# kaiwenShen/Do-You-Really-Need-to-Pay-2-20-Hedge-Fund-Strategy-Replication-via-Machine-Learning

Measured on AMD Instinct MI355X. Metric: seq/sec/node MTSS-WGAN-GP train (24x32 windows) at 1/2/4/8 GPUs; W-dist parity, higher is better.
Workload: dtype fp32; 1 GPU; global_batch=262144, batch_per_gpu=262144, seq_len=24, features=32, parallelism=dp1

## Files before the change

### do-you-really-need-to-pay-2-20-hedge-fund-strategy-replication-via-machine-learning_amd/csrc/bindings.cpp

```cpp
#include <torch/extension.h>
#include <torch/library.h>
#include <ATen/hip/impl/HIPGuardImplMasqueradingAsCUDA.h>
#include <ATen/hip/impl/HIPStreamMasqueradingAsCUDA.h>

#include "kernels.h"
#include "poison.h"

#include <atomic>
#include <cmath>
#include <cstdlib>
#include <cstring>

std::atomic<bool>& hfrep::poison_flag() {
  static std::atomic<bool> f{[] {
    const char* e = getenv("HFREP_POISON");
    return e && e[0] == '1';
  }()};
  return f;
}

namespace {

using at::Tensor;
using c10::optional;
// ... 162 lines not shown
  }
  Tensor ws = out_empty({(int64_t)hfrep::lstm_wgrad2_workspace_floats(M, K, Hd, N)}, x.options().dtype(at::kFloat));
  hfrep::launch_lstm_wgrad2(x.data_ptr(), hs.data_ptr(), dZ.data_ptr(), tangent ? xd->data_ptr() : nullptr,
                            tangent ? hds->data_ptr() : nullptr, tangent ? dZd->data_ptr() : nullptr,
                            gW.data_ptr<float>(), gU.data_ptr<float>(), gb.has_value() ? gb->data_ptr<float>() : nullptr,
                            M, K, Hd, N, Tn, ws.data_ptr<float>(), cur_stream(x));
}

Tensor act_fwd(Tensor x, int64_t act) {
  CHECK_GPU(x); GUARD(x);
  Tensor y = out_empty_like(x);
  hfrep::launch_act_fwd(dt_of(x), x.data_ptr(), y.data_ptr(), x.numel(), (int)act, cur_stream(x));
  return y;
}
Tensor act_bwd(Tensor dy, Tensor y, int64_t act) {
  CHECK_GPU(dy); CHECK_GPU(y); same_dt(dy, y);
  TORCH_CHECK(dy.numel() == y.numel(), "act_bwd: size");
  GUARD(dy);
  Tensor dx = out_empty_like(dy);
  hfrep::launch_act_bwd(dt_of(dy), dy.data_ptr(), y.data_ptr(), dx.data_ptr(), dy.numel(), (int)act, cur_stream(dy));
  return dx;
}
Tensor act_tangent_bwd(Tensor dyd, Tensor y, Tensor zd, int64_t act) {
  CHECK_GPU(dyd); CHECK_GPU(y); CHECK_GPU(zd); same_dt(dyd, y); same_dt(dyd, zd);
  TORCH_CHECK(dyd.numel() == y.numel() && y.numel() == zd.numel(), "act_tangent_bwd: size");
  GUARD(dyd);
  Tensor out = out_empty_like(dyd);
  hfrep::launch_act_tangent_bwd(dt_of(dyd), dyd.data_ptr(), y.data_ptr(), zd.data_ptr(), out.data_ptr(), dyd.numel(),
                                (int)act, cur_stream(dyd));
  return out;
}

void check_lstm_U(const Tensor& U, int64_t H) {
  CHECK_F32(U);
  TORCH_CHECK(U.dim() == 2 && U.size(0) == H && U.size(1) == 4 * H, "recurrent kernel must be (H, 4H)");
}

std::tuple<Tensor, Tensor, Tensor> lstm_fwd(Tensor zx, Tensor U, int64_t act, bool save) {
  CHECK_GPU(zx);
  TORCH_CHECK(zx.dim() == 3 && zx.size(2) % 4 == 0, "zx must be (B, T, 4H)");
  const int B = zx.size(0), Tn = zx.size(1), H = zx.size(2) / 4;
  check_lstm_U(U, H);
  GUARD(zx);
  Tensor hs = out_empty({B, Tn, H}, zx.options());
  Tensor gates = save ? out_empty({B, Tn, 4 * H}, zx.options()) : out_empty({0}, zx.options());
  Tensor cs = save ? out_empty({B, Tn, H}, zx.options()) : out_empty({0}, zx.options());
  const bool ok = hfrep::launch_lstm_fwd(dt_of(zx), zx.data_ptr(), U.data_ptr<float>(), hs.data_ptr(),
                                         save ? gates.data_ptr() : nullptr, save ? cs.data_ptr() : nullptr, B, Tn, H,
                                         (int)act, cur_stream(zx));
  TORCH_CHECK(ok, "lstm_fwd: hidden size ", H, " not instantiated (supported: 100, 64, 32)");
  return {hs, gates, cs};
}

Tensor lstm_bwd(Tensor dH, Tensor gates, Tensor cs, Tensor U, int64_t act) {
  CHECK_GPU(dH); CHECK_GPU(gates); CHECK_GPU(cs); same_dt(dH, gates); same_dt(dH, cs);
  const int B = gates.size(0), Tn = gates.size(1), H = gates.size(2) / 4;
  TORCH_CHECK(dH.sizes() == cs.sizes() && cs.size(2) == H, "lstm_bwd: shapes");
  check_lstm_U(U, H);
  GUARD(dH);
  Tensor dZ = out_empty_like(gates);
  const bool ok = hfrep::launch_lstm_bwd(dt_of(dH), dH.data_ptr(), gates.data_ptr(), cs.data_ptr(),
                                         U.data_ptr<float>(), dZ.data_ptr(), B, Tn, H, (int)act, cur_stream(dH));
  TORCH_CHECK(ok, "lstm_bwd: hidden size ", H, " not instantiated");
  return dZ;
}

std::tuple<Tensor, Tensor, Tensor> lstm_tfwd(Tensor dzx, Tensor gates, Tensor cs, Tensor U, int64_t act) {
  CHECK_GPU(dzx); CHECK_GPU(gates); CHECK_GPU(cs); same_dt(dzx, gates); same_dt(dzx, cs);
  TORCH_CHECK(dzx.sizes() == gates.sizes(), "lstm_tfwd: shapes");
  const int B = gates.size(0), Tn = gates.size(1), H = gates.size(2) / 4;
  check_lstm_U(U, H);
  GUARD(dzx);
  Tensor hds = out_empty({B, Tn, H}, dzx.options());
  Tensor zds = out_empty_like(gates);
  Tensor cds = out_empty({B, Tn, H}, dzx.options());
  const bool ok = hfrep::launch_lstm_tfwd(dt_of(dzx), dzx.data_ptr(), gates.data_ptr(), cs.data_ptr(),
                                          U.data_ptr<float>(), hds.data_ptr(), zds.data_ptr(), cds.data_ptr(), B, Tn,
                                          H, (int)act, cur_stream(dzx));
  TORCH_CHECK(ok, "lstm_tfwd: hidden size ", H, " not instantiated");
  return {hds, zds, cds};
}

std::tuple<Tensor, Tensor> lstm_tbwd(optional<Tensor> dH, Tensor dHd, Tensor gates, Tensor cs, Tensor zds, Tensor cds,
                                     Tensor U, int64_t act) {
  CHECK_GPU(dHd); CHECK_GPU(gates); CHECK_GPU(cs); CHECK_GPU(zds); CHECK_GPU(cds);
  same_dt(dHd, gates); same_dt(dHd, zds); same_dt(dHd, cds);
  if (dH.has_value()) { CHECK_GPU(*dH); same_dt(*dH, dHd); }
  const int B = gates.size(0), Tn = gates.size(1), H = gates.size(2) / 4;
  check_lstm_U(U, H);
  GUARD(dHd);
  Tensor dZ = out_empty_like(gates), dZd = out_empty_like(gates);
  const bool ok = hfrep::launch_lstm_tbwd(dt_of(dHd), ptr_or_null(dH), dHd.data_ptr(), gates.data_ptr(),
                                          cs.data_ptr(), zds.data_ptr(), cds.data_ptr(), U.data_ptr<float>(),
                                          dZ.data_ptr(), dZd.data_ptr(), B, Tn, H, (int)act, cur_stream(dHd));
  TORCH_CHECK(ok, "lstm_tbwd: hidden size ", H, " not instantiated");
  return {dZ, dZd};
}

bool lstmf_supported(int64_t H, int64_t K, int64_t act) { return hfrep::lstmf_supported((int)H, (int)K, (int)act); }
bool narrowf_supported(int64_t K, int64_t N) { return hfrep::narrowf_supported((int)K, (int)N); }
int64_t set_lstmf_fwd_impl(int64_t v) { return hfrep::set_lstmf_fwd_impl((int)v); }
int64_t set_lstmf_fwd100_impl(int64_t v) { return hfrep::set_lstmf_fwd100_impl((int)v); }
int64_t set_lstmf_bwd_impl(int64_t v) { return hfrep::set_lstmf_bwd_impl((int)v); }

std::tuple<Tensor, Tensor> lstmf_fwd(Tensor x, Tensor W, optional<Tensor> b, Tensor U, int64_t act, bool save) {
  CHECK_F32(x); CHECK_F32(W);
  TORCH_CHECK(x.dim() == 3, "x must be (B, T, K)");
  const int B = x.size(0), Tn = x.size(1), K = x.size(2), H = U.size(0);
  check_lstm_U(U, H);
  TORCH_CHECK(W.size(0) == K && W.size(1) == 4 * H, "W must be (K, 4H)");
  if (b.has_value()) { CHECK_F32(*b); TORCH_CHECK(b->numel() == 4 * H, "bias size"); }
  TORCH_CHECK(hfrep::lstmf_supported(H, K, (int)act), "lstmf_fwd: unsupported H/K/act");
  GUARD(x);
  Tensor hs = out_empty({B, Tn, H}, x.options());
  Tensor tape = at::empty({save ? (int64_t)hfrep::lstmf_tape_elems(B, Tn) : 0}, x.options());
  const bool ok = hfrep::launch_lstmf_fwd(x.data_ptr<float>(), W.data_ptr<float>(),
                                          b.has_value() ? b->data_ptr<float>() : nullptr, U.data_ptr<float>(),
                                          hs.data_ptr<float>(), save ? tape.data_ptr<float>() : nullptr, B, Tn, K, H,
                                          (int)act, cur_stream(x));
  TORCH_CHECK(ok, "lstmf_fwd: launch failed");
  return {hs, tape};
}

std::tuple<Tensor, Tensor> lstmf_tfwd(Tensor xd, Tensor W, Tensor U, Tensor tape, int64_t act) {
  CHECK_F32(xd); CHECK_F32(W); CHECK_F32(tape);
  TORCH_CHECK(xd.dim() == 3, "xd must be (B, T, K)");
  const int B = xd.size(0), Tn = xd.size(1), K = xd.size(2), H = U.size(0);
  check_lstm_U(U, H);
  TORCH_CHECK(W.size(0) == K && W.size(1) == 4 * H, "W must be (K, 4H)");
  TORCH_CHECK(tape.numel() == (int64_t)hfrep::lstmf_tape_elems(B, Tn), "lstmf_tfwd: tape size");
  TORCH_CHECK(hfrep::lstmf_supported(H, K, (int)act), "lstmf_tfwd: unsupported H/K/act");
  GUARD(xd);
  Tensor hds = out_empty({B, Tn, H}, xd.options());
  Tensor ttape = at::empty_like(tape);
  const bool ok = hfrep::launch_lstmf_tfwd(xd.data_ptr<float>(), W.data_ptr<float>(), U.data_ptr<float>(),
                                           tape.data_ptr<float>(), hds.data_ptr<float>(), ttape.data_ptr<float>(), B, Tn,
                                           K, H, (int)act, cur_stream(xd));
  TORCH_CHECK(ok, "lstmf_tfwd: launch failed");
  return {hds, ttape};
}

static void check_head(const optional<Tensor>& d, const optional<Tensor>& w, const Tensor& like, int64_t B, int64_t n) {
  if (d.has_value()) {
    CHECK_F32(*d);
    TORCH_CHECK(d->numel() == B && d->device() == like.device(), "head adjoint factor: B fp32 values");
  }
  if (w.has_value()) {
    CHECK_F32(*w);
    TORCH_CHECK(w->numel() == n && w->device() == like.device(), "head weight: Tn H fp32 values");
  }
}

bool lstmf_ahd_supported() { return hfrep::lstmf_ahd_supported(); }

Tensor lstmf_bwd(optional<Tensor> dH, Tensor tape, Tensor U, int64_t act, int64_t B, int64_t Tn, optional<Tensor> hd,
                 optional<Tensor> hw, optional<Tensor> ah_out) {
  CHECK_F32(tape);
  const int H = U.size(0);
  check_lstm_U(U, H);
  TORCH_CHECK(tape.numel() == (int64_t)hfrep::lstmf_tape_elems(B, Tn), "lstmf_bwd: tape size");
  if (dH.has_value()) { CHECK_F32(*dH); TORCH_CHECK(dH->numel() == B * Tn * H, "lstmf_bwd: dH shape"); }
  TORCH_CHECK(hd.has_value() == hw.has_value() && !(hd.has_value() && dH.has_value()),
              "lstmf_bwd: dH or the head factors (hd, hw)");
  check_head(hd, hw, tape, B, Tn * H);
  if (ah_out.has_value()) {
    CHECK_F32(*ah_out);
    TORCH_CHECK(ah_out->numel() == B * Tn * H && ah_out->is_contiguous() && ah_out->device() == tape.device(),
                "lstmf_bwd: ah_out must be a contiguous (B, T, H) fp32 tensor on the tape's device");
    TORCH_CHECK(hfrep::lstmf_ahd_supported(), "lstmf_bwd: ah_out needs the split-recurrent BPTT (lstmf_ahd_supported)");
  }
  GUARD(tape);
  Tensor dZ = out_empty({B, Tn, 4 * H}, tape.options());
  Tensor dHm;
  if (hd.has_value() && !hfrep::lstmf_head_supported()) {
    dHm = out_empty({B, Tn * H}, tape.options());
    hfrep::launch_skinny_dgrad(hfrep::DT_F32, hd->data_ptr<float>(), hw->data_ptr<float>(), dHm.data_ptr(), B,
                               (int)(Tn * H), 1, cur_stream(tape));
  }
  const bool head = hd.has_value() && !dHm.defined();
  const float* dhp = dHm.defined() ? dHm.data_ptr<float>() : dH.has_value() ? dH->data_ptr<float>() : nullptr;
  const bool ok = hfrep::launch_lstmf_bwd(dhp, tape.data_ptr<float>(), U.data_ptr<float>(), dZ.data_ptr<float>(), B, Tn,
                                          H, (int)act, cur_stream(tape), head ? hd->data_ptr<float>() : nullptr,
                                          head ? hw->data_ptr<float>() : nullptr,
                                          ah_out.has_value() ? ah_out->data_ptr<float>() : nullptr);
  TORCH_CHECK(ok, "lstmf_bwd: unsupported H / act");
  return dZ;
}

Tensor lstmf_tbwd1(optional<Tensor> dH, Tensor aH, Tensor tape, Tensor ttape, Tensor U, int64_t act, int64_t B,
                   int64_t Tn, optional<Tensor> hd, optional<Tensor> hw) {
  CHECK_F32(tape); CHECK_F32(ttape); CHECK_F32(aH);
  const int H = U.size(0);
  check_lstm_U(U, H);
  TORCH_CHECK(tape.numel() == (int64_t)hfrep::lstmf_tape_elems(B, Tn) && ttape.numel() == tape.numel(), "tape size");
  TORCH_CHECK(aH.numel() == B * Tn * H && aH.is_contiguous() && aH.device() == tape.device(),
              "lstmf_tbwd1: aH must be a contiguous (B, T, H) fp32 tensor on the tape's device");
  if (dH.has_value()) {
    CHECK_F32(*dH);
    TORCH_CHECK(dH->numel() == B * Tn * H && dH->is_contiguous() && dH->device() == tape.device(),
                "lstmf_tbwd1: adjoint shape");
  }
  const bool head = hw.has_value();
  TORCH_CHECK(!head || !dH.has_value(), "lstmf_tbwd1: the adjoint dH or head factors, not both");
  TORCH_CHECK(head || !hd.has_value(), "lstmf_tbwd1: hd needs hw");
  check_head(hd, hw, tape, B, Tn * H);
  GUARD(tape);
  Tensor dZ = out_empty({B, Tn, 4 * H}, tape.options());
  const bool ok = hfrep::launch_lstmf_tbwd1(dH.has_value() ? dH->data_ptr<float>() : nullptr, aH.data_ptr<float>(),
                                            tape.data_ptr<float>(), ttape.data_ptr<float>(), U.data_ptr<float>(),
                                            dZ.data_ptr<float>(), B, Tn, H, (int)act, cur_stream(tape),
                                            head && hd.has_value() ? hd->data_ptr<float>() : nullptr,
                                            head ? hw->data_ptr<float>() : nullptr);
  TORCH_CHECK(ok, "lstmf_tbwd1: unsupported H / act");
  return dZ;
}

std::tuple<Tensor, Tensor> lstmf_tbwd(optional<Tensor> dH, optional<Tensor> dHd, Tensor tape, Tensor ttape, Tensor U,
                                      int64_t act, int64_t B, int64_t Tn, optional<Tensor> hd, optional<Tensor> hdd,
                                      optional<Tensor> hw) {
  CHECK_F32(tape); CHECK_F32(ttape);
  const int H = U.size(0);
  check_lstm_U(U, H);
  TORCH_CHECK(tape.numel() == (int64_t)hfrep::lstmf_tape_elems(B, Tn) && ttape.numel() == tape.numel(), "tape size");
  for (const auto* d : {&dH, &dHd})
    if (d->has_value()) { CHECK_F32(**d); TORCH_CHECK((*d)->numel() == B * Tn * H, "lstmf_tbwd: adjoint shape"); }
  const bool head = hw.has_value();
  TORCH_CHECK(!head || (!dH.has_value() && !dHd.has_value()), "lstmf_tbwd: adjoints (dH, dHd) or head factors, not both");
  check_head(hd, hw, tape, B, Tn * H);
  check_head(hdd, {}, tape, B, Tn * H);
  GUARD(tape);
  Tensor dZ = out_empty({B, Tn, 4 * H}, tape.options()), dZd = out_empty({B, Tn, 4 * H}, tape.options());
  const bool ok = hfrep::launch_lstmf_tbwd(dH.has_value() ? dH->data_ptr<float>() : nullptr,
                                           dHd.has_value() ? dHd->data_ptr<float>() : nullptr, tape.data_ptr<float>(),
                                           ttape.data_ptr<float>(), U.data_ptr<float>(), dZ.data_ptr<float>(),
                                           dZd.data_ptr<float>(), B, Tn, H, (int)act, cur_stream(tape),
                                           head && hd.has_value() ? hd->data_ptr<float>() : nullptr,
                                           head && hdd.has_value() ? hdd->data_ptr<float>() : nullptr,
                                           head ? hw->data_ptr<float>() : nullptr);
  TORCH_CHECK(ok, "lstmf_tbwd: unsupported H / act");
  return {dZ, dZd};
}

Tensor lstmf_dgrad(Tensor dz, Tensor W, int64_t impl) {
  CHECK_F32(dz); CHECK_F32(W);
  TORCH_CHECK(dz.dim() == 2 && dz.is_contiguous() && W.dim() == 2 && W.is_contiguous() && W.size(1) == dz.size(1),
              "lstmf_dgrad: dz (M, N) and W (KO, N), contiguous");
  TORCH_CHECK(hfrep::lstmf_dgrad_supported(dz.size(1), W.size(0)), "lstmf_dgrad: N must be 400 and KO <= 112");
  GUARD(dz);
  Tensor x = out_empty({dz.size(0), W.size(0)}, dz.options());
  if (dz.size(0) == 0) return x;
  const bool ok = hfrep::launch_lstmf_dgrad(dz.data_ptr<float>(), W.data_ptr<float>(), x.data_ptr<float>(), dz.size(0),
                                            dz.size(1), W.size(0), cur_stream(dz), (int)impl);
  TORCH_CHECK(ok, "lstmf_dgrad: launch failed");
  return x;
}

void check_lstm2(const Tensor& x, const Tensor& U, int64_t H) {
  TORCH_CHECK(x.scalar_type() == at::kBFloat16, "lstm2 kernels are bf16-only");
  check_lstm_U(U, H);
  TORCH_CHECK(hfrep::lstm2_supported((int)H, (int)x.size(2)), "lstm2: unsupported H/K (H must be 100, K <= 128)");
}

std::tuple<Tensor, Tensor> lstm2_fwd(Tensor x, Tensor W, optional<Tensor> b, Tensor U, int64_t act, bool save) {
  CHECK_GPU(x); CHECK_F32(W);
  TORCH_CHECK(x.dim() == 3, "x must be (B, T, K)");
  const int B = x.size(0), Tn = x.size(1), K = x.size(2), H = U.size(0);
  check_lstm2(x, U, H);
  TORCH_CHECK(W.size(0) == K && W.size(1) == 4 * H, "W must be (K, 4H)");
  if (b.has_value()) { CHECK_F32(*b); TORCH_CHECK(b->numel() == 4 * H, "bias size"); }
  GUARD(x);
  Tensor hs = out_empty({B, Tn, H}, x.options());
  Tensor tape = at::empty({save ? (int64_t)hfrep::lstm2_tape_elems(B, Tn) : 0}, x.options());
  hfrep::launch_lstm2_fwd(x.data_ptr(), W.data_ptr<float>(), b.has_value() ? b->data_ptr<float>() : nullptr,
                          U.data_ptr<float>(), hs.data_ptr(), save ? tape.data_ptr() : nullptr, B, Tn, K, H, (int)act,
                          cur_stream(x));
  return {hs, tape};
}


static int check_dx_W(const optional<Tensor>& W, int H) {
  if (!W.has_value()) return 0;
  CHECK_F32(*W);
  TORCH_CHECK(W->dim() == 2 && W->size(1) == 4 * H && W->size(0) >= 1 && W->size(0) <= 112,
              "fused dX: W must be (K <= 112, 4H)");
  return (int)W->size(0);
}

static void check_head(const optional<Tensor>& d, const Tensor& w, const Tensor& like, int64_t B, int64_t Tn, int64_t H) {
  if (!d.has_value()) return;
  CHECK_GPU(*d); same_dt(*d, like);
  TORCH_CHECK(d->numel() == B && d->is_contiguous(), "head adjoint: d must be (B, 1) contiguous");
  CHECK_F32(w);
  TORCH_CHECK(w.numel() == Tn * H && w.is_contiguous(), "head adjoint: w must hold T * H floats");
}

std::tuple<Tensor, Tensor> lstm2_bwd(optional<Tensor> dH_, Tensor tape, Tensor U, int64_t act, optional<Tensor> W,
                                     bool need_dz, optional<Tensor> head_d, optional<Tensor> head_w) {
  CHECK_GPU(tape);
  const int H = U.size(0);
  TORCH_CHECK(dH_.has_value() != (head_d.has_value() && head_w.has_value()), "lstm2_bwd: dH xor (head_d, head_w)");
  const int B = dH_ ? dH_->size(0) : head_d->size(0);
  const int Tn = dH_ ? dH_->size(1) : head_w->numel() / H;
  check_lstm_U(U, H);
  if (dH_) { CHECK_GPU(*dH_); same_dt(*dH_, tape); TORCH_CHECK(dH_->size(2) == H, "dH shape"); }
  else check_head(head_d, *head_w, tape, B, Tn, H);
  TORCH_CHECK(tape.numel() == (int64_t)hfrep::lstm2_tape_elems(B, Tn), "lstm2_bwd: tape size");
  const int K = check_dx_W(W, H);
  GUARD(tape);
  TORCH_CHECK(need_dz || K, "lstm2_bwd: nothing to compute (need_dz=False without W)");
  const bool gen = !dH_;
  Tensor dZ = out_empty({need_dz ? B : 0, Tn, 4 * H}, tape.options());
  Tensor dX = out_empty({K ? B : 0, Tn, K}, tape.options());
  hfrep::launch_lstm2_bwd(gen ? nullptr : dH_->data_ptr(), tape.data_ptr(), U.data_ptr<float>(),
                          need_dz ? dZ.data_ptr() : nullptr, K ? W->data_ptr<float>() : nullptr,
                          K ? dX.data_ptr() : nullptr, K, B, Tn, H, (int)act, cur_stream(tape),
                          gen ? head_d->data_ptr() : nullptr, gen ? head_w->data_ptr<float>() : nullptr);
  return {dZ, dX};
}

std::tuple<Tensor, Tensor> lstm2_tfwd(Tensor xd, Tensor W, Tensor U, Tensor tape, int64_t act) {
  CHECK_GPU(xd); CHECK_F32(W); CHECK_GPU(tape); same_dt(xd, tape);
  const int B = xd.size(0), Tn = xd.size(1), K = xd.size(2), H = U.size(0);
  check_lstm2(xd, U, H);
  TORCH_CHECK(W.size(0) == K && W.size(1) == 4 * H, "W must be (K, 4H)");
  TORCH_CHECK(tape.numel() == (int64_t)hfrep::lstm2_tape_elems(B, Tn), "lstm2_tfwd: tape size");
  GUARD(xd);
  Tensor hds = out_empty({B, Tn, H}, xd.options());
  Tensor ttape = at::empty_like(tape);
  hfrep::launch_lstm2_tfwd(xd.data_ptr(), W.data_ptr<float>(), U.data_ptr<float>(), tape.data_ptr(), hds.data_ptr(),
                           ttape.data_ptr(), B, Tn, K, H, (int)act, cur_stream(xd));
  return {hds, ttape};
}

std::tuple<Tensor, Tensor, Tensor, Tensor> lstm2_tbwd(optional<Tensor> dH, optional<Tensor> dHd_, Tensor tape,
                                                      Tensor ttape, Tensor U, int64_t act, optional<Tensor> W,
                                                      optional<Tensor> head_d, optional<Tensor> head_dd,
                                                      optional<Tensor> head_w) {
  CHECK_GPU(tape); CHECK_GPU(ttape); same_dt(tape, ttape);
  const int H = U.size(0);
  const bool head = head_w.has_value();
  TORCH_CHECK(head ? (!dH && !dHd_ && (head_d || head_dd)) : (dHd_.has_value() && !head_d && !head_dd),
              "lstm2_tbwd: (dH?, dHd) tensors xor (head_d?, head_dd?, head_w)");
  const int B = head ? (head_d ? head_d->size(0) : head_dd->size(0)) : dHd_->size(0);
  const int Tn = head ? head_w->numel() / H : dHd_->size(1);
  check_lstm_U(U, H);
  if (!head) {
    CHECK_GPU(*dHd_); same_dt(*dHd_, tape);
    if (dH.has_value()) { CHECK_GPU(*dH); same_dt(*dH, *dHd_); TORCH_CHECK(dH->sizes() == dHd_->sizes(), "dH shape"); }
  } else {
    check_head(head_d, *head_w, tape, B, Tn, H);
    check_head(head_dd, *head_w, tape, B, Tn, H);
  }
  TORCH_CHECK(tape.numel() == (int64_t)hfrep::lstm2_tape_elems(B, Tn) && ttape.numel() == tape.numel(), "tape size");
  GUARD(tape);
  const int K = check_dx_W(W, H);
  const bool gen = head;
  Tensor dZ = out_empty({B, Tn, 4 * H}, tape.options()), dZd = out_empty({B, Tn, 4 * H}, tape.options());
  Tensor dX = out_empty({K ? B : 0, Tn, K}, tape.options()), dXd = out_empty({K ? B : 0, Tn, K}, tape.options());
  hfrep::launch_lstm2_tbwd(gen ? nullptr : ptr_or_null(dH), gen ? nullptr : dHd_->data_ptr(), tape.data_ptr(),
                           ttape.data_ptr(), U.data_ptr<float>(), dZ.data_ptr(), dZd.data_ptr(),
                           K ? W->data_ptr<float>() : nullptr, K ? dX.data_ptr() : nullptr, K ? dXd.data_ptr() : nullptr,
                           K, B, Tn, H, (int)act, cur_stream(tape), gen ? ptr_or_null(head_d) : nullptr,
                           gen ? ptr_or_null(head_dd) : nullptr, gen ? head_w->data_ptr<float>() : nullptr);
  return {dZ, dZd, dX, dXd};
}
// ... 400 lines not shown
  CHECK_F32(x); CHECK_F32(ref_sorted);
  TORCH_CHECK(x.dim() == 2, "ks_stat: x must be (n, F)");
  const int64_t n = x.size(0), F = x.size(1);
  TORCH_CHECK(n >= 1 && n <= (int64_t(1) << 24), "ks_stat: 1 <= n <= 2^24, got n = ", n);
  TORCH_CHECK(F >= 1 && F <= 1024, "ks_stat: 1 <= F <= 1024, got F = ", F);
  TORCH_CHECK(ref_sorted.device() == x.device() && ref_sorted.dim() == 2 && ref_sorted.size(0) == F &&
                  ref_sorted.size(1) == n,
              "ks_stat: ref_sorted must be (F, n) = (", F, ", ", n, ") fp32 on x's device");
  GUARD(x);
  const auto f64 = x.options().dtype(at::kDouble);
  Tensor out = out_empty({F}, f64);
  Tensor ws = out_empty({F, n}, x.options());
  Tensor ws2 = out_empty({n > 16384 ? F : 0, n}, x.options());
  Tensor slab = out_empty({F, 2, (int64_t)hfrep::ks_blocks((int)n)}, f64);
  hfrep::launch_ks_stat(x.data_ptr<float>(), ref_sorted.data_ptr<float>(), reinterpret_cast<uint32_t*>(ws.data_ptr()),
                        reinterpret_cast<uint32_t*>(ws2.data_ptr()), slab.data_ptr<double>(), out.data_ptr<double>(), (int)n, (int)F, cur_stream(x));
  return out;
}

Tensor acf_mean(Tensor x, int64_t nlags) {
  CHECK_F32(x);
  TORCH_CHECK(x.dim() == 3 && x.size(0) >= 1 && x.size(1) >= 1 && x.size(2) >= 1, "acf_mean: x must be (N, T, F)");
  const int64_t N = x.size(0), T = x.size(1), F = x.size(2);
  TORCH_CHECK(N <= INT32_MAX && nlags >= 0 && nlags <= 4096 && T <= 65536 && F <= 65536 &&
                  hfrep::acf_supported((int)T, (int)F, (int)nlags),
              "acf_mean: the (T, F) window and the (nlags + 1) F accumulators must fit 160 KB of LDS, got T = ", T,
              ", F = ", F, ", nlags = ", nlags);
  GUARD(x);
  const auto f64 = x.options().dtype(at::kDouble);
  Tensor out = out_empty({F, nlags + 1}, f64);
  Tensor slab = out_empty({(int64_t)hfrep::acf_blocks((int)N), (nlags + 1) * F}, f64);
  hfrep::launch_acf_mean(x.data_ptr<float>(), slab.data_ptr<double>(), out.data_ptr<double>(), (int)N, (int)T, (int)F,
                         (int)nlags, cur_stream(x));
  return out;
}

Tensor nb_divergences(Tensor real, Tensor fake, Tensor theta, Tensor var, Tensor log_prior) {
  CHECK_F32(real); CHECK_F32(fake);
  TORCH_CHECK(real.dim() == 3 && real.size(0) >= 1 && real.sizes() == fake.sizes() && fake.device() == real.device(),
              "nb_divergences: real and fake must be (N, T, F) on one device");
  const int64_t N = real.size(0), T = real.size(1), F = real.size(2);
  TORCH_CHECK(N <= INT32_MAX && T <= 168 && F <= 64 && hfrep::nb_supported((int)T, (int)F),
              "nb_divergences: F <= 64 and T <= 168, got T = ", T,
              ", F = ", F);
  for (const Tensor* t : {&theta, &var, &log_prior})
    TORCH_CHECK(t->is_cuda() && t->device() == real.device() && t->scalar_type() == at::kDouble && t->is_contiguous(),
                "nb_divergences: theta, var and log_prior must be contiguous float64 tensors on real's device");
  TORCH_CHECK(theta.dim() == 2 && theta.size(0) == F && theta.size(1) == T && var.sizes() == theta.sizes() &&
                  log_prior.dim() == 1 && log_prior.size(0) == F,
              "nb_divergences: theta, var (F, T) and log_prior (F,)");
  GUARD(real);
  const auto f64 = real.options().dtype(at::kDouble);
  Tensor out = out_empty({4}, f64);
  Tensor slab = out_empty({(int64_t)hfrep::nb_slab_rows((int)N), 4}, f64);
  hfrep::launch_nb_divergences(real.data_ptr<float>(), fake.data_ptr<float>(), theta.data_ptr<double>(),
                               var.data_ptr<double>(), log_prior.data_ptr<double>(), slab.data_ptr<double>(),
                               out.data_ptr<double>(), (int)N, (int)T, (int)F, cur_stream(real));
  return out;
}

Tensor lp_cols(Tensor a, Tensor b) {
  CHECK_F32(a); CHECK_F32(b);
  TORCH_CHECK(a.dim() == 2 && a.sizes() == b.sizes() && a.device() == b.device(),
              "lp_cols: a and b must be (n, F) on one device");
  const int64_t n = a.size(0), F = a.size(1);
  TORCH_CHECK(n >= 1 && n <= INT32_MAX && F >= 1 && F <= (1 << 20), "lp_cols: 1 <= n < 2^31, 1 <= F <= 2^20");
  GUARD(a);
  const auto f64 = a.options().dtype(at::kDouble);
  Tensor out = out_empty({3, F}, f64);
  Tensor slab = out_empty({(int64_t)hfrep::lp_blocks(n), 3, F}, f64);
  hfrep::launch_lp_cols(a.data_ptr<float>(), b.data_ptr<float>(), slab.data_ptr<double>(), out.data_ptr<double>(), n,
                        (int)F, cur_stream(a));
  return out;
}

Tensor p2p_buffer(int64_t cap, int64_t device) {
  TORCH_CHECK(cap > 0, "p2p_buffer: cap must be positive");
  bool fine = false;
  void* p = hfrep::p2p_alloc(cap, (int)device, &fine);
  auto opts = at::TensorOptions().dtype(at::kByte).device(at::Device(at::kCUDA, (int)device));
  return torch::from_blob(p, {(int64_t)hfrep::p2p_buffer_bytes(cap)}, [](void* q) { hfrep::p2p_free(q); }, opts);
}

std::vector<int64_t> p2p_handle(Tensor buf) {
  TORCH_CHECK(buf.is_cuda() && buf.scalar_type() == at::kByte, "p2p_handle: a p2p_buffer tensor");
  uint8_t h[64];
  hfrep::p2p_ipc_handle(buf.data_ptr(), h);
  return std::vector<int64_t>(h, h + 64);
}

int64_t p2p_open(std::vector<int64_t> handle, int64_t device) {
  TORCH_CHECK(handle.size() == 64, "p2p_open: a 64-byte IPC handle");
  uint8_t h[64];
  for (int i = 0; i < 64; ++i) h[i] = (uint8_t)handle[i];
  return (int64_t)reinterpret_cast<intptr_t>(hfrep::p2p_ipc_open(h, (int)device));
}

void p2p_close(int64_t ptr) { hfrep::p2p_ipc_close(reinterpret_cast<void*>((intptr_t)ptr)); }

void p2p_allreduce_(Tensor x, Tensor buf, std::vector<int64_t> peers, int64_t rank, int64_t cap, double scale,
                    double timeout_s) {
  CHECK_F32(x);
  TORCH_CHECK(buf.is_cuda() && buf.scalar_type() == at::kByte && buf.device() == x.device(),
              "p2p_allreduce_: buf must be this device's p2p_buffer");
  const int world = (int)peers.size();
  TORCH_CHECK(world >= 1 && world <= hfrep::kP2PMaxRanks && rank >= 0 && rank < world, "p2p_allreduce_: 1 <= world <= 8");
  TORCH_CHECK(x.numel() <= cap && buf.numel() >= (int64_t)hfrep::p2p_buffer_bytes(cap), "p2p_allreduce_: x exceeds cap");
  TORCH_CHECK(peers[rank] == (int64_t)reinterpret_cast<intptr_t>(buf.data_ptr()), "p2p_allreduce_: peers[rank] must be buf");
  hfrep::P2PPeers pp{};
  for (int r = 0; r < world; ++r) pp.base[r] = reinterpret_cast<char*>((intptr_t)peers[r]);
  TORCH_CHECK(timeout_s > 0, "p2p_allreduce_: timeout_s must be positive");
  GUARD(x);
  static thread_local int s_dev = -1;
  static thread_local double s_sec = -1;
  static thread_local uint64_t s_ticks = 0;
  if (s_dev != x.get_device() || s_sec != timeout_s) {
    s_ticks = hfrep::p2p_timeout_ticks(timeout_s, x.get_device());
    s_dev = x.get_device();
    s_sec = timeout_s;
  }
  hfrep::launch_p2p_allreduce(x.data_ptr<float>(), x.numel(), pp, (int)rank, world, cap, (float)scale, s_ticks,
                              cur_stream(x));
}

int64_t p2p_error(Tensor buf) {
  TORCH_CHECK(buf.is_cuda() && buf.scalar_type() == at::kByte, "p2p_error: a p2p_buffer tensor");
  GUARD(buf);
  return hfrep::p2p_read_error(buf.data_ptr());
}

}

TORCH_LIBRARY(hfrep, m) {
  m.def("linear(Tensor x, Tensor W, Tensor? b, int act, Tensor(a!)? out=None) -> Tensor");
  m.def("linear_dgrad(Tensor dz, Tensor W) -> Tensor");
  m.def("linear_wgrad_(Tensor x, Tensor dz, Tensor(a!) gW, Tensor(b!)? gb, int shiftT=0) -> ()");
  m.def("lstm_wgrad_(Tensor x, Tensor hs, Tensor dZ, Tensor(a!) gW, Tensor(b!) gU, Tensor(c!)? gb, Tensor? xd=None, Tensor? hds=None, Tensor? dZd=None, int impl=0) -> ()");
  m.def("act_fwd(Tensor x, int act) -> Tensor");
  m.def("act_bwd(Tensor dy, Tensor y, int act) -> Tensor");
  m.def("act_tangent_bwd(Tensor dyd, Tensor y, Tensor zd, int act) -> Tensor");
  m.def("lstm_fwd(Tensor zx, Tensor U, int act, bool save) -> (Tensor, Tensor, Tensor)");
  m.def("lstm_bwd(Tensor dH, Tensor gates, Tensor cs, Tensor U, int act) -> Tensor");
  m.def("lstm_tfwd(Tensor dzx, Tensor gates, Tensor cs, Tensor U, int act) -> (Tensor, Tensor, Tensor)");
  m.def("lstm_tbwd(Tensor? dH, Tensor dHd, Tensor gates, Tensor cs, Tensor zds, Tensor cds, Tensor U, int act) -> (Tensor, Tensor)");
  m.def("lstmf_supported(int H, int K, int act) -> bool", &lstmf_supported);
  m.def("narrowf_supported(int K, int N) -> bool", &narrowf_supported);
  m.def("set_lstmf_fwd_impl(int v) -> int", &set_lstmf_fwd_impl);
  m.def("set_lstmf_fwd100_impl(int v) -> int", &set_lstmf_fwd100_impl);
  m.def("set_lstmf_bwd_impl(int v) -> int", &set_lstmf_bwd_impl);
  m.def("lstmf_fwd(Tensor x, Tensor W, Tensor? b, Tensor U, int act, bool save) -> (Tensor, Tensor)");
  m.def("linear_head_cs(Tensor x, Tensor W, Tensor? b, int split, float wa, float wb, Tensor(a!) gW, Tensor(b!)? gb) -> Tensor");
  m.def("linear_head_cs_supported(int K) -> bool", &linear_head_cs_supported);
  m.def("lstmf_bwd(Tensor? dH, Tensor tape, Tensor U, int act, int B, int T, Tensor? hd=None, Tensor? hw=None, "
        "Tensor(a!)? ah_out=None) -> Tensor");
  m.def("lstmf_ahd_supported() -> bool", &lstmf_ahd_supported);
  m.def("lstmf_tbwd1(Tensor? dH, Tensor aH, Tensor tape, Tensor ttape, Tensor U, int act, int B, int T, Tensor? hd=None, "
        "Tensor? hw=None) -> Tensor");
  m.def("lstmf_tbwd(Tensor? dH, Tensor? dHd, Tensor tape, Tensor ttape, Tensor U, int act, int B, int T, Tensor? hd=None, "
        "Tensor? hdd=None, Tensor? hw=None) -> (Tensor, Tensor)");
  m.def("lstmf_tfwd(Tensor xd, Tensor W, Tensor U, Tensor tape, int act) -> (Tensor, Tensor)");
  m.def("lstmf_dgrad(Tensor dz, Tensor W, int impl=0) -> Tensor");
  m.def("lstm2_fwd(Tensor x, Tensor W, Tensor? b, Tensor U, int act, bool save) -> (Tensor, Tensor)");
  m.def("lstm2_bwd(Tensor? dH, Tensor tape, Tensor U, int act, Tensor? W=None, bool need_dz=True, Tensor? head_d=None, "
        "Tensor? head_w=None) -> (Tensor, Tensor)");
  m.def("lstm2_tfwd(Tensor xd, Tensor W, Tensor U, Tensor tape, int act) -> (Tensor, Tensor)");
  m.def("lstm2_tbwd(Tensor? dH, Tensor? dHd, Tensor tape, Tensor ttape, Tensor U, int act, Tensor? W=None, "
        "Tensor? head_d=None, Tensor? head_dd=None, Tensor? head_w=None) -> (Tensor, Tensor, Tensor, Tensor)");
  m.def("set_debug_poison(bool on) -> bool", &set_debug_poison);
  m.def("layernorm_fwd(Tensor x, Tensor gamma, Tensor beta, float eps, bool save=True, float pre_lrelu=-1.0) -> "
        "(Tensor, Tensor, Tensor)");
  m.def("layernorm_bwd_(Tensor dy, Tensor xhat, Tensor rstd, Tensor gamma, Tensor(a!)? ggamma, Tensor(b!)? gbeta) -> Tensor");
  m.def("layernorm_tfwd(Tensor xd, Tensor xhat, Tensor rstd, Tensor gamma) -> Tensor");
  m.def("layernorm_tbwd_(Tensor? dy, Tensor dyd, Tensor xd, Tensor xhat, Tensor rstd, Tensor gamma, "
        "Tensor(a!) ggamma, Tensor(b!) gbeta, bool need_dx) -> (Tensor, Tensor)");
  m.def("gp_coef(Tensor g, float weight) -> (Tensor, Tensor)");
  m.def("gp_coef_pack(Tensor g, float weight, Tensor w) -> (Tensor, Tensor)");
  m.def("gp_pack(Tensor pen, float weight, Tensor w) -> Tensor");
  m.def("gan_loss(Tensor p, int split, float la, float lb, int kind) -> (Tensor, Tensor)");
  m.def("im2col_causal(Tensor x, int k, int dil) -> Tensor");
  m.def("col2im_causal(Tensor dcols, int k, int dil, int C) -> Tensor");
  m.def("interpolate(Tensor real, Tensor fake, Tensor alpha) -> Tensor");
  m.def("philox_fill_(Tensor(a!) out, int seed, Tensor(b!) ctr, int dist) -> ()");
  m.def("sample_windows(Tensor data, int batch, int seed, Tensor(a!) ctr, ScalarType out_dtype, Tensor(b!)? dst=None) -> Tensor");
  m.def("ae_fit_supported(int A, int k, int batch) -> bool", &ae_fit_supported);
  m.def("ae_fit(Tensor[] Xt, Tensor[] Xv, Tensor[] order, Tensor(a!)[] We, Tensor(b!)[] Wd, Tensor(c!)[] mWe, "
        "Tensor(d!)[] vWe, Tensor(e!)[] mWd, Tensor(f!)[] vWd, Tensor(g!)[] step, Tensor(h!)[] m_cache, int[] patience, "
        "float lr, float b1, float b2, float eps, int batch, bool bf16) -> (Tensor, Tensor)");
  m.def("ae_window_table(Tensor x, Tensor ends, bool refit) -> (Tensor, Tensor, Tensor)");
  m.def("ae_recon_metrics(Tensor[] x, Tensor[] ends, Tensor[] scale, Tensor[] mn, Tensor[] sstot, Tensor[] We, Tensor[] Wd, "
        "Tensor work, bool bf16) -> (Tensor, Tensor)");
  m.def("rmsprop_(Tensor(a!) p, Tensor g, Tensor(b!) ms, float lr, float rho, float eps, float clip, float gscale) -> ()");
  m.def("adam_(Tensor(a!) p, Tensor g, Tensor(b!) m, Tensor(c!) v, Tensor step, float lr, float b1, float b2, float eps, float clip, float gscale) -> ()");
  m.def("nadam_(Tensor(a!) p, Tensor g, Tensor(b!) m, Tensor(c!) v, Tensor step, Tensor m_cache, float lr, float b1, float b2, float eps, float gscale) -> ()");
  m.def("step_advance_(Tensor(a!) step, Tensor(b!)? m_cache, float b1) -> ()");
  m.def("clip_(Tensor(a!) p, float c) -> ()");
  m.def("wdist_sorted(Tensor x, Tensor ref_sorted) -> Tensor");
  m.def("ks_stat(Tensor x, Tensor ref_sorted) -> Tensor");
  m.def("acf_mean(Tensor x, int nlags) -> Tensor");
  m.def("nb_divergences(Tensor real, Tensor fake, Tensor theta, Tensor var, Tensor log_prior) -> Tensor");
  m.def("lp_cols(Tensor a, Tensor b) -> Tensor");
  m.def("p2p_buffer(int cap, int device) -> Tensor", &p2p_buffer);
  m.def("p2p_handle(Tensor buf) -> int[]");
  m.def("p2p_open(int[] handle, int device) -> int", &p2p_open);
  m.def("p2p_close(int ptr) -> ()", &p2p_close);
  m.def("p2p_allreduce_(Tensor(a!) x, Tensor buf, int[] peers, int rank, int cap, float scale, float timeout_s) -> ()");
  m.def("p2p_error(Tensor buf) -> int");
}

TORCH_LIBRARY_IMPL(hfrep, CUDA, m) {
  m.impl("linear", &linear);
  m.impl("p2p_handle", &p2p_handle);
  m.impl("p2p_allreduce_", &p2p_allreduce_);
  m.impl("p2p_error", &p2p_error);
  m.impl("linear_dgrad", &linear_dgrad);
  m.impl("linear_wgrad_", &linear_wgrad_);
  m.impl("lstm_wgrad_", &lstm_wgrad_);
  m.impl("act_fwd", &act_fwd);
  m.impl("act_bwd", &act_bwd);
  m.impl("act_tangent_bwd", &act_tangent_bwd);
  m.impl("lstm_fwd", &lstm_fwd);
  m.impl("lstmf_fwd", &lstmf_fwd);
  m.impl("lstmf_tfwd", &lstmf_tfwd);
  m.impl("linear_head_cs", &linear_head_cs);
  m.impl("lstmf_bwd", &lstmf_bwd);
  m.impl("lstmf_tbwd", &lstmf_tbwd);
  m.impl("lstmf_tbwd1", &lstmf_tbwd1);
  m.impl("lstmf_dgrad", &lstmf_dgrad);
  m.impl("lstm_bwd", &lstm_bwd);
  m.impl("lstm_tfwd", &lstm_tfwd);
  m.impl("lstm_tbwd", &lstm_tbwd);
  m.impl("lstm2_fwd", &lstm2_fwd);
  m.impl("lstm2_bwd", &lstm2_bwd);
  m.impl("lstm2_tfwd", &lstm2_tfwd);
  m.impl("lstm2_tbwd", &lstm2_tbwd);
  m.impl("layernorm_fwd", &layernorm_fwd);
  m.impl("layernorm_bwd_", &layernorm_bwd_);
  m.impl("layernorm_tfwd", &layernorm_tfwd);
  m.impl("layernorm_tbwd_", &layernorm_tbwd_);
  m.impl("gp_coef", &gp_coef);
  m.impl("gp_coef_pack", &gp_coef_pack);
  m.impl("gp_pack", &gp_pack);
  m.impl("gan_loss", &gan_loss);
  m.impl("im2col_causal", &im2col_causal);
  m.impl("col2im_causal", &col2im_causal);
  m.impl("interpolate", &interpolate);
  m.impl("philox_fill_", &philox_fill_);
  m.impl("sample_windows", &sample_windows);
  m.impl("ae_fit", &ae_fit);
  m.impl("ae_window_table", &ae_window_table);
  m.impl("ae_recon_metrics", &ae_recon_metrics);
  m.impl("rmsprop_", &rmsprop_);
  m.impl("adam_", &adam_);
  m.impl("nadam_", &nadam_);
  m.impl("step_advance_", &step_advance_);
  m.impl("clip_", &clip_);
  m.impl("wdist_sorted", &wdist_sorted);
  m.impl("ks_stat", &ks_stat);
  m.impl("acf_mean", &acf_mean);
  m.impl("nb_divergences", &nb_divergences);
  m.impl("lp_cols", &lp_cols);
}
```

### do-you-really-need-to-pay-2-20-hedge-fund-strategy-replication-via-machine-learning_amd/csrc/kernels.h

```cpp
#pragma once
#include <hip/hip_runtime.h>
#include <stdint.h>

namespace hfrep {

enum DType : int { DT_F32 = 0, DT_BF16 = 1 };

bool launch_lstm_fwd(int dt, const void* zx, const float* U, void* hs, void* gates, void* cs, int B, int Tn, int H,
                     int act, hipStream_t s);
bool launch_lstm_bwd(int dt, const void* dH, const void* gates, const void* cs, const float* U, void* dZ, int B,
                     int Tn, int H, int act, hipStream_t s);
bool launch_lstm_tfwd(int dt, const void* dzx, const void* gates, const void* cs, const float* U, void* hds,
                      void* zds, void* cds, int B, int Tn, int H, int act, hipStream_t s);
bool launch_lstm_tbwd(int dt, const void* dH, const void* dHd, const void* gates, const void* cs, const void* zds,
                      const void* cds, const float* U, void* dZ, void* dZd, int B, int Tn, int H, int act,
                      hipStream_t s);

size_t lstm2_tape_elems(int B, int Tn);
bool lstm2_supported(int H, int K);
void launch_lstm2_fwd(const void* x, const float* W, const float* b, const float* U, void* hs, void* tape, int B, int Tn,
                      int K, int H, int act, hipStream_t s);
void launch_lstm2_tfwd(const void* xd, const float* W, const float* U, const void* tape, void* hds, void* ttape, int B,
                       int Tn, int K, int H, int act, hipStream_t s);
void launch_lstm2_bwd(const void* dH, const void* tape, const float* U, void* dZ, const float* W, void* dX, int K,
                      int B, int Tn, int H, int act, hipStream_t s, const void* head_d = nullptr,
                      const float* hw = nullptr);
void launch_lstm2_tbwd(const void* dH, const void* dHd, const void* tape, const void* ttape, const float* U, void* dZ,
                       void* dZd, const float* W, void* dX, void* dXd, int K, int B, int Tn, int H, int act,
                       hipStream_t s, const void* head_d = nullptr, const void* head_dd = nullptr,
                       const float* hw = nullptr);

bool lstmf_supported(int H, int K, int act);
size_t lstmf_tape_elems(int B, int Tn);
bool launch_lstmf_fwd(const float* x, const float* W, const float* b, const float* U, float* hs, float* tape, int B,
                      int Tn, int K, int H, int act, hipStream_t s);
bool launch_lstmf_tfwd(const float* xd, const float* W, const float* U, const float* tape, float* hds, float* ttape,
                       int B, int Tn, int K, int H, int act, hipStream_t s);
bool launch_lstmf_bwd(const float* dH, const float* tape, const float* U, float* dZ, int B, int Tn, int H, int act,
                      hipStream_t s, const float* hd = nullptr, const float* hw = nullptr, float* aH = nullptr);
bool lstmf_head_supported();
bool lstmf_ahd_supported();
bool launch_lstmf_tbwd1(const float* dH, const float* aH, const float* tape, const float* ttape, const float* U, float* dZ,
                        int B, int Tn, int H, int act, hipStream_t s, const float* hd = nullptr,
                        const float* hw = nullptr);
bool launch_lstmf_tbwd(const float* dH, const float* dHd, const float* tape, const float* ttape, const float* U, float* dZ,
                       float* dZd, int B, int Tn, int H, int act, hipStream_t s, const float* hd = nullptr,
                       const float* hdd = nullptr, const float* hw = nullptr);
int set_lstmf_fwd_impl(int v);
int set_lstmf_fwd100_impl(int v);
int set_lstmf_bwd_impl(int v);

bool lstmf_wgrad_supported(int K, int H, int N);
size_t lstmf_wgrad_workspace_floats(int M, int K, int impl = 0);
bool launch_lstmf_wgrad(const float* X, const float* Hs, const float* D, const float* Xd, const float* Hds, const float* Dd,
                        float* gW, float* gU, float* gb, int M, int K, int Tn, float* ws, hipStream_t s, int impl = 0);
bool lstmf_dgrad_supported(int N, int KO);
bool launch_lstmf_dgrad(const float* D, const float* W, float* X, int M, int N, int KO, hipStream_t s, int impl = 0);

bool ae_fit_supported(int A, int k, int batch);
struct AeFitJob {
  const float* Xt;
  const float* Xv;
  const int* order;
  float *We, *Wd, *mWe, *vWe, *mWd, *vWd, *step, *m_cache;
  double* hist;
  int* nep;
  int nt, nv, epochs, patience, k, pad_;
};
void launch_ae_fit(bool bf16, const AeFitJob* jobs, int njobs, int batch, float lr, float b1, float b2, float eps, int A,
                   hipStream_t s);

void launch_ae_window_table(const double* X, const int* ends, double* scale, double* mn, double* sstot, int A, int n,
                            int W, bool refit, hipStream_t s);
struct AeEvalJob {
  const double* X;
  const int* ends;
  const double *scale, *mn, *sstot;
  const float *We, *Wd;
  double *r2, *rmse;
  int n, W, k, pad_;
};
void launch_ae_recon_metrics(bool bf16, const AeEvalJob* jobs, int njobs, const int* work, int nwork, int A,
                             hipStream_t s);

void launch_linear(int dt, const void* A, const float* W, const float* bias, void* C, int M, int N, int K,
                   int w_trans, int act, hipStream_t s);
bool fp32_exact_mode();
size_t wgrad_workspace_floats(int M, int K, int N);
void launch_wgrad(int dt, const void* X, const void* D, float* gW, float* gb, int M, int K, int N, int shiftT,
                  float* ws, hipStream_t s);

size_t lstm_wgrad2_workspace_floats(int M, int K, int Hd, int N);
void launch_lstm_wgrad2(const void* X0, const void* H0, const void* D0, const void* X1, const void* H1, const void* D1,
                        float* gW, float* gU, float* gb, int M, int K, int Hd, int N, int Tn, float* ws, hipStream_t s);
void launch_lstm_wgrad2_reduce(const float* ws, float* gW, float* gU, float* gb, int splits, int K, int Hd, int N,
                               hipStream_t s, int Ks = 0);
void launch_linear2(const void* A, const float* W, const float* bias, void* C, int M, int N, int K, int w_trans, int act,
                    hipStream_t s);

bool lstm_wgrad3_supported(int M, int K, int Hd, int N);
size_t lstm_wgrad3_workspace_floats(int K, int Hd, int N);
bool launch_lstm_wgrad3(const void* X0, const void* H0, const void* D0, const void* X1, const void* H1, const void* D1,
                        float* gW, float* gU, float* gb, int M, int K, int Hd, int N, int Tn, float* ws, hipStream_t s);

bool skinny_supported(int K, int N);
bool narrow_supported(int K, int N);
void launch_narrow_fwd(const void* x, const float* W, const float* b, void* y, int M, int K, int N, int act,
                       hipStream_t s);
bool narrowf_supported(int K, int N);
bool widef_supported(int K, int N);
void launch_widef(const float* x, const float* B, int sk, int sn, const float* b, float* y, int M, int K, int N,
                  int act, hipStream_t s);
void launch_narrowf(const float* x, const float* B, int sk, int sn, const float* b, float* y, int M, int K, int N,
                    int act, hipStream_t s);
void launch_skinny_fwd(int dt, const void* x, const float* W, const float* b, void* y, int M, int K, int N, int act,
                       hipStream_t s);
size_t skinny_wgrad_workspace_floats(int M, int K, int N);
void launch_skinny_wgrad(int dt, const void* x, const void* d, float* gW, float* gb, int M, int K, int N, float* ws,
                         hipStream_t s);
void launch_skinny_dgrad(int dt, const void* d, const float* W, void* dx, int M, int K, int N, hipStream_t s);
bool skinny_fwd_cs_supported(int K);
size_t skinny_fwd_cs_workspace_floats(int M, int K);
void launch_skinny_fwd_cs(int dt, const void* x, const float* W, const float* b, void* y, int M, int K, int split,
                          float wa, float wb, float* gW, float* gb, float* ws, hipStream_t s);
void launch_split_reduce(const float* slab, float* a, float* b, int splits, int na, int nb, hipStream_t s);

int device_cu_count();
void launch_im2col_causal(int dt, const void* x, void* cols, int B, int Tn, int C, int k, int dil, hipStream_t s);
void launch_col2im_causal(int dt, const void* dcols, void* dx, int B, int Tn, int C, int k, int dil, hipStream_t s);
void launch_act_fwd(int dt, const void* x, void* y, int64_t n, int act, hipStream_t s);
void launch_act_bwd(int dt, const void* dy, const void* y, void* dx, int64_t n, int act, hipStream_t s);
void launch_act_tangent_bwd(int dt, const void* dyd, const void* y, const void* zd, void* out, int64_t n, int act,
                            hipStream_t s);
void launch_layernorm_fwd(int dt, const void* x, const float* gamma, const float* beta, void* y, void* xhat,
                          float* rstd, int64_t rows, int D, float eps, float pre_alpha, hipStream_t s);
int layernorm_bwd_splits(int64_t rows);
void launch_layernorm_bwd(int dt, const void* dy, const void* xhat, const float* rstd, const float* gamma,
                          void* dx, float* ggamma, float* gbeta, float* ws, int64_t rows, int D, hipStream_t s);
void launch_layernorm_tfwd(int dt, const void* xd, const void* xhat, const float* rstd, const float* gamma, void* yd,
                           int64_t rows, int D, hipStream_t s);
void launch_layernorm_tbwd(int dt, const void* dy, const void* dyd, const void* xd, const void* xhat,
                           const float* rstd, const float* gamma, void* dx, void* dxd, float* ggamma, float* gbeta,
                           float* ws, int64_t rows, int D, hipStream_t s);
void launch_gan_loss(int dt, const void* p, int64_t n, int64_t split, float la, float lb, int kind, void* grad,
                     float* partial, float* out, hipStream_t s);
int gan_loss_partials();
void launch_gp_pack(const float* pen, const float* w, float weight, float* pack, hipStream_t s);
void launch_gp_coef(int dt, const void* g, void* v, float* pen, float* rowpen, int B, int64_t D, float weight,
                    hipStream_t s, const float* w = nullptr, float* pack = nullptr);
void launch_interpolate(int dt, const void* real, const void* fake, const float* alpha, void* out, int B,
                        int64_t D, hipStream_t s);
void launch_philox_fill(int dt, void* out, int64_t n, uint64_t seed, int64_t* ctr, int dist, hipStream_t s);
void launch_sample_windows(int dt, const float* data, int64_t N, int64_t D, void* out, int B, uint64_t seed,
                           int64_t* ctr, hipStream_t s);
void launch_cast(int dt_in, const void* in, int dt_out, void* out, int64_t n, hipStream_t s);

void launch_rmsprop(float* p, const float* g, float* ms, int64_t n, float lr, float rho, float eps, float clip,
                    float gscale, hipStream_t s);
void launch_adam(float* p, const float* g, float* m, float* v, int64_t n, const float* step, float lr, float b1,
                 float b2, float eps, float clip, float gscale, hipStream_t s);
void launch_nadam(float* p, const float* g, float* m, float* v, int64_t n, const float* step, const float* m_cache,
                  float lr, float b1, float b2, float eps, float gscale, hipStream_t s);
void launch_step_advance(float* step, float* m_cache, float b1, hipStream_t s);
void launch_clip(float* p, int64_t n, float c, hipStream_t s);

int wdist_blocks(int n);
void launch_wdist_sorted(int dt, const void* x, const float* ref_sorted, uint32_t* ws, double* slab, double* out, int n,
                         int F, hipStream_t s);

int ks_blocks(int n);
void launch_ks_stat(const float* x, const float* ref_sorted, uint32_t* ws, uint32_t* ws2, double* slab, double* out,
                    int n, int F, hipStream_t s);
bool acf_supported(int T, int F, int nlags);
int acf_blocks(int N);
void launch_acf_mean(const float* x, double* slab, double* out, int N, int T, int F, int nlags, hipStream_t s);
bool nb_supported(int T, int F);
int nb_slab_rows(int N);
void launch_nb_divergences(const float* real, const float* fake, const double* theta, const double* var,
                           const double* log_prior, double* slab, double* out, int N, int T, int F, hipStream_t s);
int lp_blocks(int64_t n);
void launch_lp_cols(const float* a, const float* b, double* slab, double* out, int64_t n, int F, hipStream_t s);

constexpr int kP2PMaxRanks = 8, kP2PMaxBlocks = 256;
constexpr int kP2PCtr = 0, kP2PDone = 128, kP2PErr = 256, kP2PFlags = 4096, kP2PData = 16384;
struct P2PPeers { char* base[kP2PMaxRanks]; };
size_t p2p_buffer_bytes(int64_t cap);
void* p2p_alloc(int64_t cap, int device, bool* fine_grained);
void p2p_free(void* p);
void p2p_ipc_handle(void* p, uint8_t out[64]);
void* p2p_ipc_open(const uint8_t h[64], int device);
void p2p_ipc_close(void* p);
int p2p_read_error(void* own);
uint64_t p2p_timeout_ticks(double seconds, int device);
int p2p_blocks(int64_t n);
void launch_p2p_allreduce(float* x, int64_t n, const P2PPeers& peers, int rank, int world, int64_t cap, float scale,
                          uint64_t timeout_ticks, hipStream_t s);

// ... 2 lines not shown
```

### do-you-really-need-to-pay-2-20-hedge-fund-strategy-replication-via-machine-learning_amd/csrc/lstm_f32.hip

```cpp
#include "lstmf_dev.h"

#include <atomic>
#include <cstdlib>
#include <type_traits>
#include <stdexcept>

namespace hfrep {

namespace {

__device__ __forceinline__ rsrc_t ftile_rsrc(const float* base, int row0, int B, int Tn, int W) {
  row0 = __builtin_amdgcn_readfirstlane(row0);
  const int nr = base ? max(0, min(32, B - row0)) : 0;
  return make_rsrc(base + (nr ? (size_t)row0 * Tn * W : 0), nr * Tn * W * 4);
}

template <int K>
struct FGeo {
  static_assert(K >= 1 && K <= 112, "fp32 LSTM: K <= 112");
  static constexpr int KS = (K + 3) / 4;
  static constexpr int KQ = KS <= 12 ? 12 : 28;
  static constexpr int LR = KS <= 12 ? 56 : 120;
  static constexpr int NJ = (KS + 3) / 4;
};
template <int K>
constexpr int f_nwr() { return FGeo<K>::KS <= 12 ? FGeo<K>::KS : 12; }
template <int K>
constexpr int f_nwl() { return FGeo<K>::KS - f_nwr<K>(); }

__device__ __forceinline__ float qswap2(float v) {
  return __builtin_bit_cast(float, __builtin_amdgcn_mov_dpp(__builtin_bit_cast(int, v), 0x4E, 0xF, 0xF, true));
}
__device__ __forceinline__ float qswap1(float v) {
  return __builtin_bit_cast(float, __builtin_amdgcn_mov_dpp(__builtin_bit_cast(int, v), 0xB1, 0xF, 0xF, true));
}
__device__ __forceinline__ void quad_transpose(float (&a)[4], int q) {
  const float p0 = qswap2(a[0]), p1 = qswap2(a[1]), p2 = qswap2(a[2]), p3 = qswap2(a[3]);
  const bool lo = q < 2;
  const float b0 = lo ? a[0] : p2, b1 = lo ? a[1] : p3, b2 = lo ? p0 : a[2], b3 = lo ? p1 : a[3];
  const float r0 = qswap1(b0), r1 = qswap1(b1), r2 = qswap1(b2), r3 = qswap1(b3);
  const bool ev = !(q & 1);
  a[0] = ev ? b0 : r1;
  a[1] = ev ? r0 : b1;
  a[2] = ev ? b2 : r3;
  a[3] = ev ? r2 : b3;
}

template <int K>
struct FXPart {
  static constexpr bool VEC = K % 4 == 0;
  static constexpr int PER = VEC ? K / 4 : K;
  static constexpr int NJ = (32 * PER + 255) / 256;
  float v[VEC ? 4 * NJ : NJ];
  int goff[NJ], lpos[NJ];
  __device__ __forceinline__ void set(int Tn, int tid) {
    using GX = FGeo<K>;
#pragma unroll
    for (int j = 0; j < NJ; ++j) {
      const int e = tid + 256 * j, r = e / PER, c = e - r * PER;
      const bool ok = r < 32;
      if constexpr (VEC) {
        goff[j] = ok ? (r * Tn * K + 4 * c) * 4 : kOOB;
        lpos[j] = ok ? r * GX::LR + c : -1;
      } else {
        goff[j] = ok ? (r * Tn * K + c) * 4 : kOOB;
        lpos[j] = ok ? r * GX::LR + (c & 3) * GX::KQ + (c >> 2) : -1;
      }
    }
  }
  __device__ __forceinline__ void load(rsrc_t rx, int Tn, int t, bool on) {
#pragma unroll
    for (int j = 0; j < NJ; ++j) {
      const int vo = on ? goff[j] : kOOB;
      if constexpr (VEC) {
        const f32x4 d = __builtin_bit_cast(f32x4, __builtin_amdgcn_raw_buffer_load_b128(rx, vo, t * K * 4, 0));
        v[4 * j] = d[0]; v[4 * j + 1] = d[1]; v[4 * j + 2] = d[2]; v[4 * j + 3] = d[3];
      } else {
        v[j] = ld1(rx, vo, t * K * 4);
      }
    }
  }
  __device__ __forceinline__ void to_lds(float* xb, float* trash) const {
    using GX = FGeo<K>;
#pragma unroll
    for (int j = 0; j < NJ; ++j) {
      float* d = lpos[j] >= 0 ? xb + lpos[j] : trash;
      if constexpr (VEC) {
        const int s = lpos[j] >= 0 ? GX::KQ : 0;
        d[0] = v[4 * j]; d[s] = v[4 * j + 1]; d[2 * s] = v[4 * j + 2]; d[3 * s] = v[4 * j + 3];
      } else {
        d[0] = v[j];
      }
    }
  }
};

constexpr int FT_MN = 2 * FNT, FT_SLOT = 64 * 5, FT_STEP = 4 * FT_MN * FT_SLOT;
__device__ __forceinline__ rsrc_t ftape_rsrc(const float* tape, int rb, int nrb, int Tn) {
  rb = __builtin_amdgcn_readfirstlane(rb);
  const bool on = tape && rb < nrb;
  return make_rsrc(tape + (on ? (size_t)rb * Tn * FT_STEP : 0), on ? Tn * FT_STEP * 4 : 0);
}
__device__ __forceinline__ int ftape_lane(int w, int lane) { return (w * FT_MN * FT_SLOT) * 4 + lane * 16; }
__device__ __forceinline__ int ftape_cell(int w, int lane) { return (w * FT_MN * FT_SLOT + 256 + lane) * 4; }
__device__ __forceinline__ constexpr int ftape_slot(int m, int n) { return (m * FNT + n) * FT_SLOT * 4; }

}

template <int ACT, int KX, bool TAPE, bool TAN>
__global__ void __launch_bounds__(256, 1)
lstmf_fwd_kernel(const float* __restrict__ x, const float* __restrict__ W, const float* __restrict__ bias,
                 const float* __restrict__ U, const float* __restrict__ ptape, float* __restrict__ hs,
                 float* __restrict__ tape, int B, int Tn) {
  using GX = FGeo<KX>;
  using GH = FGeo<FH>;
  constexpr int NWR = f_nwr<KX>(), NWL = f_nwl<KX>();
  extern __shared__ __attribute__((aligned(16))) float fsm[];
  float* xb = fsm;
  float* hb = xb + 2 * 32 * GX::LR;
  float* wl = hb + 2 * 32 * GH::LR;
  float* trash = wl + NWL * 4 * FNT * 64;
  const int tid = threadIdx.x, lane = tid & 63;
  const int w = __builtin_amdgcn_readfirstlane(tid >> 6);
  const int q = lane & 3, g = lane >> 4, j4 = (lane & 15) >> 2;
  const int ub = FUW * w + j4;
  const int nrb = (B + 31) / 32;

  for (int i = tid; i < 2 * 32 * (GX::LR + GH::LR); i += 256) fsm[i] = 0.f;

  constexpr float GSC = ACT == ACT_TANH ? -2.f * kLog2e : ACT == ACT_SIGMOID ? -kLog2e : 1.f;
  const float sc = TAN ? 1.f : (q == 2 ? GSC : -kLog2e);
  float uf[GH::KS][FNT];
  float wf[NWR][FNT];
  float bq[FNT];
#pragma unroll
  for (int n = 0; n < FNT; ++n) {
    const int u = ub + 4 * n;
    const bool ok = u < FH;
    const int cl = q * FH + (ok ? u : FH - 1);
#pragma unroll
    for (int ks = 0; ks < GH::KS; ++ks) {
      const float v = U[(4 * ks + g) * FG + cl];
      uf[ks][n] = ok ? v * sc : 0.f;
      asm volatile("" : "+a"(uf[ks][n]));
    }
#pragma unroll
    for (int ks = 0; ks < GX::KS; ++ks) {
      const int k = 4 * ks + g;
      const float v = W[min(k, KX - 1) * FG + cl];
      const float wv = (ok && k < KX) ? v * sc : 0.f;
      if (ks < NWR) {
        wf[ks < NWR ? ks : 0][n] = wv;
        if (ks >= 8) asm volatile("" : "+a"(wf[ks < NWR ? ks : 0][n]));
      }
      else wl[(((ks - NWR) * 4 + w) * FNT + n) * 64 + lane] = wv;
    }
    const float bv = bias ? bias[cl] : 0.f;
    bq[n] = (!TAN && ok) ? bv * sc : 0.f;
  }
  const bool glin = !TAN && ACT == ACT_LINEAR && q == 2;
  const float am = (ACT == ACT_TANH && q == 2) ? 2.f : 1.f, bm = (ACT == ACT_TANH && q == 2) ? -1.f : 0.f;
  const int ax = (lane & 15) * GX::LR + g * GX::KQ, ah = (lane & 15) * GH::LR + g * GH::KQ;
  const int hw = (4 * g + q) * GH::LR + j4 * GH::KQ + 7 * w;

  for (int rb = blockIdx.x; rb < nrb; rb += gridDim.x) {
    const int row0 = rb * 32;
    const rsrc_t rx = ftile_rsrc(x, row0, B, Tn, KX);
    const rsrc_t rh = ftile_rsrc(hs, row0, B, Tn, FH);
    const rsrc_t rt = ftape_rsrc(TAPE ? tape : nullptr, rb, nrb, Tn);
    const rsrc_t rp = ftape_rsrc(TAN ? ptape : nullptr, rb, nrb, Tn);
    int vp1[2];
#pragma unroll
    for (int m = 0; m < 2; ++m) vp1[m] = ((16 * m + 4 * g + q) * Tn * FH + ub) * 4;
    const int tl = ftape_lane(w, lane), tcl = ftape_cell(w, lane);
    float cprev[TAN ? 2 : 1][FNT];
    if constexpr (TAN) {
#pragma unroll
      for (int m = 0; m < 2; ++m)
#pragma unroll
        for (int n = 0; n < FNT; ++n) cprev[m][n] = 0.f;
    }
    float cst[2][FNT];
#pragma unroll
    for (int m = 0; m < 2; ++m)
#pragma unroll
      for (int n = 0; n < FNT; ++n) cst[m][n] = 0.f;
    FXPart<KX> xp;
    xp.set(Tn, tid);
    xp.load(rx, Tn, 0, true);
    for (int i = tid; i < 32 * GH::LR; i += 256) hb[i] = 0.f;
    xp.to_lds(xb, trash);
    __syncthreads();
    for (int t = 0; t < Tn; ++t) {
      const float* xcur = xb + (t & 1) * 32 * GX::LR;
      const float* hcur = hb + (t & 1) * 32 * GH::LR;
      float* hnext = hb + ((t + 1) & 1) * 32 * GH::LR;
      xp.load(rx, Tn, t + 1, t + 1 < Tn);
#pragma unroll
      for (int m = 0; m < 2; ++m) {
        f32x4 pg[TAN ? FNT : 1];
        float pc[TAN ? FNT : 1];
        const int p1 = vp1[m] + t * FH * 4, tb = t * FT_STEP * 4;
        if constexpr (TAN) {
#pragma unroll
          for (int n = 0; n < FNT; ++n) {
            const bool tok = !(w == 3 && n >= 4);
            pg[n] = ld4(rp, tok ? tl + tb + ftape_slot(m, n) : kOOB);
            pc[n] = ld1(rp, tok ? tcl + tb + ftape_slot(m, n) : kOOB, 0);
          }
        }
        f32x4 acc[FNT];
#pragma unroll
        for (int n = 0; n < FNT; ++n) acc[n] = f32x4{0.f, 0.f, 0.f, 0.f};
#pragma unroll
        for (int j = 0; j < GX::NJ; ++j) {
          const f32x4 a4 = *reinterpret_cast<const f32x4*>(xcur + ax + 16 * m * GX::LR + 4 * j);
#pragma unroll
          for (int s = 0; s < 4; ++s) {
            const int ks = 4 * j + s;
            if (ks >= GX::KS) break;
#pragma unroll
            for (int n = 0; n < FNT; ++n) {
              const float bw = ks < NWR ? wf[ks < NWR ? ks : 0][n] : wl[(((ks - NWR) * 4 + w) * FNT + n) * 64 + lane];
              acc[n] = mma4(a4[s], bw, acc[n]);
            }
          }
          __builtin_amdgcn_sched_barrier(0);
        }
#pragma unroll
        for (int j = 0; j < GH::NJ; ++j) {
          const f32x4 a4 = *reinterpret_cast<const f32x4*>(hcur + ah + 16 * m * GH::LR + 4 * j);
#pragma unroll
          for (int s = 0; s < 4; ++s) {
            const int ks = 4 * j + s;
            if (ks >= GH::KS) break;
#pragma unroll
            for (int n = 0; n < FNT; ++n) acc[n] = mma4(a4[s], uf[ks][n], acc[n]);
          }
          __builtin_amdgcn_sched_barrier(0);
        }
#pragma unroll
        for (int n = 0; n < FNT; ++n) {
          const bool tok = !(w == 3 && n >= 4);
          const int v1 = tok ? p1 + 16 * n : kOOB;
          float hv;
          if constexpr (!TAN) {
            float y[4];
#pragma unroll
            for (int i = 0; i < 4; ++i) {
              const float s = acc[n][i] + bq[n];
              const float e = am * __builtin_amdgcn_rcpf(1.f + __builtin_amdgcn_exp2f(s)) + bm;
              y[i] = glin ? s : e;
            }
            quad_transpose(y, q);
            const float cn = y[1] * cst[m][n] + y[0] * y[2];
            float ca;
            if constexpr (ACT == ACT_TANH) ca = 2.f * __builtin_amdgcn_rcpf(1.f + __builtin_amdgcn_exp2f(GSC * cn)) - 1.f;
            else if constexpr (ACT == ACT_SIGMOID) ca = __builtin_amdgcn_rcpf(1.f + __builtin_amdgcn_exp2f(GSC * cn));
// ... 263 lines not shown
        }
      for (int i = tid; i < 32 * BZ_LR; i += 512) zt[i] = 0.f;
      for (int i = tid; i < 32 * BH_LR; i += 512) ht[i] = 0.f;
      __syncthreads();
      auto half_b = [&](auto M_, int t) {
        constexpr int m = decltype(M_)::value;
#pragma unroll
        for (int n = 0; n < FNT; ++n) {
          const bool tok = unit_ok(w, n);
          f32x4 z4;
          bptt_cell<ACT>(z4, dc[m][n], tg[m][n], tc[m][n], tcp[m][n], tdh[m][n], ht[hr + 16 * m * BH_LR + 4 * n], tok,
                         zt + zw + 16 * m * BZ_LR + 4 * n, trash);
          tc[m][n] = tcp[m][n];
          const int tp = t > 0 ? t - 1 : 0;
          bwdf_tape_load(tg[m][n], tcp[m][n], tdh[m][n], rt, rdh, tl + tp * FT_STEP * 4 + ftape_slot(m, n),
                         tcl + (tp - 1) * FT_STEP * 4 + ftape_slot(m, n), vp1[m] + tp * FH * 4 + 16 * n,
                         tok && t > 0, tp > 0);
        }
      };
      for (int t = Tn - 1; t >= 0; --t) {
        if (t < Tn - 1) st.half<1, false>(zt, rz, Tn, t + 1, nr);
        half_b(I0{}, t);
        lds_barrier();
        st.half<0, false>(zt, rz, Tn, t, nr);
        half_b(I1{}, t);
        lds_barrier();
      }
      st.half<1, false>(zt, rz, Tn, 0, nr);
      __syncthreads();
    }
  }
}

constexpr int kTanCellGroup = 2;
template <int ACT, bool HEAD = false>
__global__ void __launch_bounds__(512, 1)
lstmf_tbwdp_kernel(const float* __restrict__ dH, const float* __restrict__ dHd, const float* __restrict__ tape,
                   const float* __restrict__ ttape, const float* __restrict__ U, float* __restrict__ dZ,
                   float* __restrict__ dZd, int B, int Tn, const float* __restrict__ hd, const float* __restrict__ hdd,
                   const float* __restrict__ hw) {
  extern __shared__ __attribute__((aligned(16))) float fsm[];
  float* zt = fsm;
  float* zdt = zt + 32 * BZ_LR;
  float* ht = zdt + 32 * BZ_LR;
  float* hdt = ht + 32 * BH_LR;
  float* trash = hdt + 32 * BH_LR;
  const int tid = threadIdx.x, lane = tid & 63;
  const int wv = __builtin_amdgcn_readfirstlane(tid >> 6);
  const int w = wv & 3;
  const int q = lane & 3, g = lane >> 4, j4 = (lane & 15) >> 2, c16 = lane & 15;
  const int nrb = (B + 31) / 32;
  if (wv < 4) {
    float ut[2][FH];
    rev_ut_load(ut, U, w, c16, g);
    auto half_a = [&](auto M_) {
      constexpr int M = decltype(M_)::value;
      rev_half_a<M, 2>(zt, ht, ut, w, c16, g);
      rev_half_a<M, 2>(zdt, hdt, ut, w, c16, g);
    };
    const RevStore st(tid, Tn);
    for (int rb = blockIdx.x; rb < nrb; rb += gridDim.x) {
      const int row0 = rb * 32;
      const rsrc_t rz = ftile_rsrc(dZ, row0, B, Tn, FG), rzd = ftile_rsrc(dZd, row0, B, Tn, FG);
      const int nr = min(32, B - row0);
      auto store_half = [&](auto M_, int ts) {
        constexpr int M = decltype(M_)::value;
        st.half<M, true>(zt, rz, Tn, ts, nr);
        st.half<M, true>(zdt, rzd, Tn, ts, nr);
      };
      for (int i = tid; i < 2 * 32 * (BZ_LR + BH_LR); i += 512) zt[i] = 0.f;
      __syncthreads();
      for (int t = Tn - 1; t >= 0; --t) {
        if (t < Tn - 1) store_half(I1{}, t + 1);
        half_a(I1{});
        lds_barrier();
        store_half(I0{}, t);
        half_a(I0{});
        lds_barrier();
      }
      store_half(I1{}, 0);
      __syncthreads();
    }
  } else {
    const int ub = FUW * w + j4;
    const int hr = (4 * g + q) * BH_LR + ub, zw = (4 * g + q) * BZ_LR + ub;
    const int tl = ftape_lane(w, lane), tcl = ftape_cell(w, lane);
    for (int rb = blockIdx.x; rb < nrb; rb += gridDim.x) {
      const int row0 = rb * 32;
      const rsrc_t rdh = ftile_rsrc(dH, row0, B, Tn, FH), rdhd = ftile_rsrc(dHd, row0, B, Tn, FH);
      const rsrc_t rt = ftape_rsrc(tape, rb, nrb, Tn), rtt = ftape_rsrc(ttape, rb, nrb, Tn);
      int vp1[2];
#pragma unroll
      for (int m = 0; m < 2; ++m) vp1[m] = ((16 * m + 4 * g + q) * Tn * FH + ub) * 4;
      float hdv[2], hddv[2];
      head_rows<HEAD>(hdv, hd, hd != nullptr, row0, B, g, q);
      head_rows<HEAD>(hddv, hdd, hdd != nullptr, row0, B, g, q);
      const rsrc_t rhw = head_rsrc<HEAD>(hw, Tn);
      const int hvo = ub * 4;
      float tc[2][FNT], tcd[2][FNT], acn[2][FNT], acdn[2][FNT];
      f32x4 tg[FNT], tz[FNT];
      float tcp[FNT], tcdp[FNT], tdh[FNT], tdhd[FNT];
      auto load_half = [&](auto M_, int tt, bool on) {
        constexpr int m = decltype(M_)::value;
#pragma unroll
        for (int n = 0; n < FNT; ++n) {
          const bool tok = on && unit_ok(w, n);
          const float wn = tan_step_load<HEAD>(tg[n], tz[n], tcp[n], tcdp[n], tdh[n], rt, rtt, rdh, rhw, tl, tcl, vp1[m],
                                               hvo, hdv[m], m, n, tt, tok);
          if constexpr (HEAD) tdhd[n] = hddv[m] * wn;
          else tdhd[n] = ld1(rdhd, tok ? vp1[m] : kOOB, tt * FH * 4 + 16 * n);
        }
      };
#pragma unroll
      for (int m = 0; m < 2; ++m)
#pragma unroll
        for (int n = 0; n < FNT; ++n) {
          const bool tok = unit_ok(w, n);
          const int oc = tcl + (Tn - 1) * FT_STEP * 4 + ftape_slot(m, n);
          acn[m][n] = 0.f;
          acdn[m][n] = 0.f;
          tc[m][n] = ld1(rt, tok ? oc : kOOB, 0);
          tcd[m][n] = ld1(rtt, tok ? oc : kOOB, 0);
        }
      load_half(I0{}, Tn - 1, true);
      for (int i = tid; i < 2 * 32 * (BZ_LR + BH_LR); i += 512) zt[i] = 0.f;
      __syncthreads();
      auto half_b = [&](auto M_) {
        constexpr int m = decltype(M_)::value;
#pragma unroll
        for (int n = 0; n < FNT; ++n) {
          const int hi = hr + 16 * m * BH_LR + 4 * n, zo = zw + 16 * m * BZ_LR + 4 * n;
          tan_cell<ACT, true>(acn[m][n], acdn[m][n], tg[n], tz[n], tc[m][n], tcd[m][n], tcp[n], tcdp[n], tdh[n], ht + hi,
                              tdhd[n], hdt + hi, unit_ok(w, n), zt, zdt, zo, trash);
          tc[m][n] = tcp[n];
          tcd[m][n] = tcdp[n];
          if ((n + 1) % kTanCellGroup == 0 || n == FNT - 1) __builtin_amdgcn_sched_barrier(0);
        }
      };
      for (int t = Tn - 1; t >= 0; --t) {
        half_b(I0{});
        __builtin_amdgcn_sched_barrier(0);
        load_half(I1{}, t, true);
        lds_barrier();
        half_b(I1{});
        __builtin_amdgcn_sched_barrier(0);
        load_half(I0{}, t > 0 ? t - 1 : 0, t > 0);
        lds_barrier();
      }
      __syncthreads();
    }
  }
}

template <int ACT, bool HEAD = false>
__global__ void __launch_bounds__(512, 1)
lstmf_tbwd1_kernel(const float* __restrict__ dH, const float* __restrict__ aH, const float* __restrict__ tape,
                   const float* __restrict__ ttape, const float* __restrict__ U, float* __restrict__ dZ, int B, int Tn,
                   const float* __restrict__ hd, const float* __restrict__ hw) {
  extern __shared__ __attribute__((aligned(16))) float fsm[];
  float* zt = fsm;
  float* ht = zt + 32 * BZ_LR;
  float* trash = ht + 32 * BH_LR;
  const int tid = threadIdx.x, lane = tid & 63;
  const int wv = __builtin_amdgcn_readfirstlane(tid >> 6);
  const int w = wv & 3;
  const int q = lane & 3, g = lane >> 4, j4 = (lane & 15) >> 2, c16 = lane & 15;
  const int nrb = (B + 31) / 32;
  if (wv < 4) {
    float ut[2][FH];
    rev_ut_load(ut, U, w, c16, g);
    const RevStore st(tid, Tn);
    for (int rb = blockIdx.x; rb < nrb; rb += gridDim.x) {
      const int row0 = rb * 32;
      const rsrc_t rz = ftile_rsrc(dZ, row0, B, Tn, FG);
      const int nr = min(32, B - row0);
      for (int i = tid; i < 32 * (BZ_LR + BH_LR); i += 512) zt[i] = 0.f;
      __syncthreads();
      for (int t = Tn - 1; t >= 0; --t) {
        if (t < Tn - 1) st.half<1, true>(zt, rz, Tn, t + 1, nr);
        rev_half_a<1, 2>(zt, ht, ut, w, c16, g);
        lds_barrier();
        st.half<0, true>(zt, rz, Tn, t, nr);
        rev_half_a<0, 2>(zt, ht, ut, w, c16, g);
        lds_barrier();
      }
      st.half<1, true>(zt, rz, Tn, 0, nr);
      __syncthreads();
    }
  } else {
    const int ub = FUW * w + j4;
    const int hr = (4 * g + q) * BH_LR + ub, zw = (4 * g + q) * BZ_LR + ub;
    const int tl = ftape_lane(w, lane), tcl = ftape_cell(w, lane);
    for (int rb = blockIdx.x; rb < nrb; rb += gridDim.x) {
      const int row0 = rb * 32;
      const rsrc_t rdh = ftile_rsrc(dH, row0, B, Tn, FH), rah = ftile_rsrc(aH, row0, B, Tn, FH);
      const rsrc_t rt = ftape_rsrc(tape, rb, nrb, Tn), rtt = ftape_rsrc(ttape, rb, nrb, Tn);
      int vp1[2];
#pragma unroll
      for (int m = 0; m < 2; ++m) vp1[m] = ((16 * m + 4 * g + q) * Tn * FH + ub) * 4;
      float hdv[2];
      head_rows<HEAD>(hdv, hd, hd != nullptr, row0, B, g, q);
      const rsrc_t rhw = head_rsrc<HEAD>(hw, Tn);
      const int hvo = ub * 4;
      float tc[2][FNT], tcd[2][FNT], acn[2][FNT], acdn[2][FNT];
      f32x4 tg[FNT], tz[FNT];
      float tcp[FNT], tcdp[FNT], tdh[FNT], tah[FNT];
      auto load_cell = [&](auto M_, int n, int tt, bool on) {
        constexpr int m = decltype(M_)::value;
        const bool tok = on && unit_ok(w, n);
        tan_step_load<HEAD>(tg[n], tz[n], tcp[n], tcdp[n], tdh[n], rt, rtt, rdh, rhw, tl, tcl, vp1[m], hvo, hdv[m], m, n, tt,
                            tok);
        tah[n] = ld1(rah, tok ? vp1[m] : kOOB, tt * FH * 4 + 16 * n);
      };
      auto load_half = [&](auto M_, int tt, bool on) {
#pragma unroll
        for (int n = 0; n < FNT; ++n) load_cell(M_, n, tt, on);
      };
#pragma unroll
      for (int m = 0; m < 2; ++m)
#pragma unroll
        for (int n = 0; n < FNT; ++n) {
          const bool tok = unit_ok(w, n);
          const int oc = tcl + (Tn - 1) * FT_STEP * 4 + ftape_slot(m, n);
          acn[m][n] = 0.f;
          acdn[m][n] = 0.f;
          tc[m][n] = ld1(rt, tok ? oc : kOOB, 0);
          tcd[m][n] = ld1(rtt, tok ? oc : kOOB, 0);
        }
      load_half(I0{}, Tn - 1, true);
      for (int i = tid; i < 32 * (BZ_LR + BH_LR); i += 512) zt[i] = 0.f;
      __syncthreads();
      auto half_b = [&](auto M_, auto MN_, int tn, bool non) {
        constexpr int m = decltype(M_)::value;
#pragma unroll
        for (int n = 0; n < FNT; ++n) {
          const bool tok = unit_ok(w, n);
          const float i_ = tg[n][0], f_ = tg[n][1], g_ = tg[n][2], o_ = tg[n][3];
          const float zdi = tz[n][0], zdf = tz[n][1], zdg = tz[n][2], zdo = tz[n][3];
          const float c = tc[m][n], cd = tcd[m][n], cp = tcp[n], cdp = tcdp[n];
          const float si = i_ * (1.f - i_), sf = f_ * (1.f - f_), so = o_ * (1.f - o_), sg = act_dy(ACT, g_);
          const float idot = si * zdi, fdot = sf * zdf, gdot = sg * zdg, odot = so * zdo;
          const float ca = act_f(ACT, c), d1 = act_dy(ACT, ca), d2 = act_d2y(ACT, ca);
          const float a_h = tdh[n] + ht[hr + 16 * m * BH_LR + 4 * n], a_hd = tah[n];
          const float a_od = a_hd * ca;
          const float a_o = a_h * ca + a_hd * d1 * cd;
          const float a_cd = acdn[m][n] + a_hd * o_ * d1;
          const float a_c = acn[m][n] + a_h * o_ * d1 + a_hd * (odot * d1 + o_ * d2 * cd);
          const float a_fd = a_cd * cp, a_id = a_cd * g_, a_gd = a_cd * i_;
          const float a_f = a_c * cp + a_cd * cdp;
          const float a_i = a_c * g_ + a_cd * gdot;
          const float a_g = a_c * i_ + a_cd * idot;
          acn[m][n] = tok ? a_c * f_ + a_cd * fdot : 0.f;
          acdn[m][n] = tok ? a_cd * f_ : 0.f;
          const float s2i = si * (1.f - 2.f * i_), s2f = sf * (1.f - 2.f * f_), s2o = so * (1.f - 2.f * o_);
          const float s2g = act_d2y(ACT, g_);
          float z4[4];
          z4[0] = a_i * si + a_id * s2i * zdi;
          z4[1] = a_f * sf + a_fd * s2f * zdf;
          z4[2] = a_g * sg + a_gd * s2g * zdg;
          z4[3] = a_o * so + a_od * s2o * zdo;
          float* zp = tok ? zt + zw + 16 * m * BZ_LR + 4 * n : trash;
#pragma unroll
          for (int k = 0; k < 4; ++k) zp[k * BZ_KQ] = z4[k];
          tc[m][n] = cp;
          tcd[m][n] = cdp;
          load_cell(MN_, n, tn, non);
          if ((n + 1) % kTanCellGroup == 0 || n == FNT - 1) __builtin_amdgcn_sched_barrier(0);
        }
      };
      for (int t = Tn - 1; t >= 0; --t) {
        half_b(I0{}, I1{}, t, true);
        lds_barrier();
        half_b(I1{}, I0{}, t > 0 ? t - 1 : 0, t > 0);
        lds_barrier();
      }
      __syncthreads();
    }
  }
}

constexpr int FS_HR = 112;
constexpr int FS_HPL = 32 * FS_HR * 2;
constexpr int FS_HB = 3 * FS_HPL + 32 * 4 * 4;

template <int ACT, int KX, bool TAPE, bool TAN>
__global__ void __launch_bounds__(256, 1)
lstmf_fwds_kernel(const float* __restrict__ x, const float* __restrict__ W, const float* __restrict__ bias,
                  const float* __restrict__ U, const float* __restrict__ ptape, float* __restrict__ hs,
                  float* __restrict__ tape, int B, int Tn) {
  using GX = FGeo<KX>;
  static_assert(GX::KS <= 12, "split forward: K <= 48 (W^T in registers)");
  constexpr int NW = GX::KS;
  extern __shared__ __attribute__((aligned(16))) float fsm[];
  float* xb = fsm;
  float* trash = xb + 2 * 32 * GX::LR;
  lds_char* trashc = (lds_char*)trash;
  lds_char* hb = (lds_char*)(trash + 4);
  const int tid = threadIdx.x, lane = tid & 63;
  const int w = __builtin_amdgcn_readfirstlane(tid >> 6);
  const int q = lane & 3, g = lane >> 4, j4 = (lane & 15) >> 2;
  const int ub = FUW * w + j4;
  const int nrb = (B + 31) / 32;

  for (int i = tid; i < 2 * 32 * GX::LR; i += 256) xb[i] = 0.f;

  constexpr float GSC = ACT == ACT_TANH ? -2.f * kLog2e : ACT == ACT_SIGMOID ? -kLog2e : 1.f;
  const float sc = TAN ? 1.f : (q == 2 ? GSC : -kLog2e);
  bf16x8 up[3][FNT][3];
  float ut[FNT], wf[NW][FNT], bq[FNT];
#pragma unroll
  for (int n = 0; n < FNT; ++n) {
    const int u = ub + 4 * n;
    const bool ok = u < FH;
    const int cl = q * FH + (ok ? u : FH - 1);
#pragma unroll
    for (int ks = 0; ks < 3; ++ks) {
      uint32_t hh[8], mm[8], ll[8];
#pragma unroll
      for (int j = 0; j < 8; ++j) {
        const int k = 32 * ks + 8 * g + j;
        const float v = ok ? U[k * FG + cl] * sc : 0.f;
        const uint32_t h = trunc_hi(v);
        const float r1 = v - __builtin_bit_cast(float, h);
        const uint32_t m = trunc_hi(r1);
        const float r2 = r1 - __builtin_bit_cast(float, m);
        hh[j] = h; mm[j] = m; ll[j] = __builtin_bit_cast(uint32_t, r2);
      }
      uint4 ph, pm, pl;
      ph.x = __builtin_amdgcn_perm(hh[1], hh[0], 0x07060302u); ph.y = __builtin_amdgcn_perm(hh[3], hh[2], 0x07060302u);
      ph.z = __builtin_amdgcn_perm(hh[5], hh[4], 0x07060302u); ph.w = __builtin_amdgcn_perm(hh[7], hh[6], 0x07060302u);
      pm.x = __builtin_amdgcn_perm(mm[1], mm[0], 0x07060302u); pm.y = __builtin_amdgcn_perm(mm[3], mm[2], 0x07060302u);
      pm.z = __builtin_amdgcn_perm(mm[5], mm[4], 0x07060302u); pm.w = __builtin_amdgcn_perm(mm[7], mm[6], 0x07060302u);
      pl.x = __builtin_amdgcn_perm(ll[1], ll[0], 0x07060302u); pl.y = __builtin_amdgcn_perm(ll[3], ll[2], 0x07060302u);
      pl.z = __builtin_amdgcn_perm(ll[5], ll[4], 0x07060302u); pl.w = __builtin_amdgcn_perm(ll[7], ll[6], 0x07060302u);
      up[ks][n][0] = __builtin_bit_cast(bf16x8, ph);
      up[ks][n][1] = __builtin_bit_cast(bf16x8, pm);
      up[ks][n][2] = __builtin_bit_cast(bf16x8, pl);
#pragma unroll
      for (int p = 0; p < 3; ++p) asm volatile("" : "+a"(up[ks][n][p]));
    }
    ut[n] = ok ? U[(96 + g) * FG + cl] * sc : 0.f;
#pragma unroll
    for (int ks = 0; ks < NW; ++ks) {
      const int k = 4 * ks + g;
      const float v = W[min(k, KX - 1) * FG + cl];
      wf[ks][n] = (ok && k < KX) ? v * sc : 0.f;
    }
    const float bv = bias ? bias[cl] : 0.f;
    bq[n] = (!TAN && ok) ? bv * sc : 0.f;
  }
  const bool glin = !TAN && ACT == ACT_LINEAR && q == 2;
  const float am = (ACT == ACT_TANH && q == 2) ? 2.f : 1.f, bm = (ACT == ACT_TANH && q == 2) ? -1.f : 0.f;
  const int ax = (lane & 15) * GX::LR + g * GX::KQ;
  const int ahp = ((lane & 15) * FS_HR + 8 * g) * 2, aht = 3 * FS_HPL + ((lane & 15) * 4 + g) * 4;

  for (int rb = blockIdx.x; rb < nrb; rb += gridDim.x) {
    const int row0 = rb * 32;
    const rsrc_t rx = ftile_rsrc(x, row0, B, Tn, KX);
    const rsrc_t rh = ftile_rsrc(hs, row0, B, Tn, FH);
    const rsrc_t rt = ftape_rsrc(TAPE ? tape : nullptr, rb, nrb, Tn);
    const rsrc_t rp = ftape_rsrc(TAN ? ptape : nullptr, rb, nrb, Tn);
    int vp1[2];
#pragma unroll
    for (int m = 0; m < 2; ++m) vp1[m] = ((16 * m + 4 * g + q) * Tn * FH + ub) * 4;
    const int tl = ftape_lane(w, lane), tcl = ftape_cell(w, lane);
// ... 489 lines not shown
      for (int m = 0; m < 2; ++m)
#pragma unroll
        for (int n = 0; n < NT; ++n) cprev[m][n] = 0.f;
    }
    float cst[2][NT];
#pragma unroll
    for (int m = 0; m < 2; ++m)
#pragma unroll
      for (int n = 0; n < NT; ++n) cst[m][n] = 0.f;
    if constexpr (!BIG) {
      xp.set(Tn, xtid);
      if (!xld) {
#pragma unroll
        for (int j = 0; j < FXPart<KX>::NJ; ++j) { xp.goff[j] = kOOB; xp.lpos[j] = -1; }
      }
      xp.load(rx, Tn, 0, true);
    }
    for (int i = tid; i < 32 * GH::LR; i += 512) hb[i] = 0.f;
    if constexpr (!BIG) xp.to_lds(xb, trash);
    __syncthreads();
    for (int t = 0; t < Tn; ++t) {
      const float* xcur = xb + (t & 1) * 32 * GX::LR;
      const float* hcur = hb + (t & 1) * 32 * GH::LR;
      float* hnext = hb + ((t + 1) & 1) * 32 * GH::LR;
      if constexpr (!BIG) xp.load(rx, Tn, t + 1, t + 1 < Tn);
      auto half = [&](auto M_) {
        constexpr int m = decltype(M_)::value;
        constexpr int NH = (BIG && m == ROLE - 1) ? 4 : 3;
        f32x4 pg[TAN ? NH : 1];
        float pc[TAN ? NH : 1];
        const int p1 = vp0 + (16 * m * Tn + t) * FH * 4;
        const int tb = t * FT_STEP * 4 + ftape_slot(m, 0);
        if constexpr (TAN) {
#pragma unroll
          for (int n = 0; n < NH; ++n) {
            pg[n] = ld4(rp, lane * 16 + (tb + tsl[n]));
            pc[n] = ld1(rp, (256 + lane) * 4 + (tb + tsl[n]), 0);
          }
        }
        f32x4 acc[NH];
#pragma unroll
        for (int n = 0; n < NH; ++n) acc[n] = f32x4{0.f, 0.f, 0.f, 0.f};
        f32x4 w4[NH];
#pragma unroll
        for (int j = 0; j < GX::NJ; ++j) {
          const f32x4 a4 = *reinterpret_cast<const f32x4*>(xcur + ax + 16 * m * GX::LR + 4 * j);
#pragma unroll
          for (int s = 0; s < 4; ++s) {
            const int ks = 4 * j + s;
            if (ks >= GX::KS) break;
            if (ks >= NWR && (ks - NWR) % 4 == 0) {
#pragma unroll
              for (int n = 0; n < NH; ++n) w4[n] = wlw[(wrel(n) + (ks - NWR) / 4) * 64];
            }
#pragma unroll
            for (int n = 0; n < NH; ++n) {
              const float bw = ks < NWR ? wf[ks < NWR ? ks : 0][n] : w4[n][(ks >= NWR ? ks - NWR : 0) & 3];
              acc[n] = mma4(a4[s], bw, acc[n]);
            }
          }
          __builtin_amdgcn_sched_barrier(0);
        }
#pragma unroll
        for (int j = 0; j < GH::NJ; ++j) {
          const f32x4 a4 = *reinterpret_cast<const f32x4*>(hcur + ah + 16 * m * GH::LR + 4 * j);
#pragma unroll
          for (int s = 0; s < 4; ++s) {
            const int ks = 4 * j + s;
            if (ks >= GH::KS) break;
#pragma unroll
            for (int n = 0; n < NH; ++n) acc[n] = mma4(a4[s], uf[ks][n], acc[n]);
          }
          __builtin_amdgcn_sched_barrier(0);
        }
#pragma unroll
        for (int n = 0; n < NH; ++n) {
          const int v1 = p1 + 16 * f2_rel<ROLE>(n);
          const int tg = lane * 16 + (tb + tsl[n]), tc = (256 + lane) * 4 + (tb + tsl[n]);
          const f32x4 zs = acc[n];
          float hv;
          if constexpr (!TAN) {
            float y[4];
#pragma unroll
            for (int e4 = 0; e4 < 4; ++e4) {
              const float s_ = zs[e4] + bq[n];
              const float r_ = __builtin_amdgcn_rcpf(1.f + __builtin_amdgcn_exp2f(s_));
              float e = r_;
              if constexpr (ACT == ACT_TANH) e = __builtin_fmaf(am, r_, bm);
              y[e4] = glin ? s_ : e;
            }
            quad_transpose(y, q);
            const float cn = __builtin_fmaf(y[1], cst[m][n], y[0] * y[2]);
            float ca;
            if constexpr (ACT == ACT_TANH) ca = __builtin_fmaf(__builtin_amdgcn_rcpf(1.f + __builtin_amdgcn_exp2f(GSC * cn)), 2.f, -1.f);
            else if constexpr (ACT == ACT_SIGMOID) ca = __builtin_amdgcn_rcpf(1.f + __builtin_amdgcn_exp2f(GSC * cn));
            else ca = cn;
            hv = y[3] * ca;
            cst[m][n] = cn;
            if constexpr (TAPE) {
              st4(f32x4{y[0], y[1], y[2], y[3]}, rt, tg);
              st1(cn, rt, tc, 0);
            }
          } else {
            float zd[4] = {zs[0], zs[1], zs[2], zs[3]};
            quad_transpose(zd, q);
            const f32x4 y = pg[n];
            const float idot = y[0] * (1.f - y[0]) * zd[0], fdot = y[1] * (1.f - y[1]) * zd[1];
            const float dg = ACT == ACT_TANH ? __builtin_fmaf(-y[2], y[2], 1.f) : ACT == ACT_SIGMOID ? y[2] * (1.f - y[2]) : 1.f;
            const float gdot = dg * zd[2], odot = y[3] * (1.f - y[3]) * zd[3];
            const float c = pc[n];
            const float ca = act_f(ACT, c);
            const float dc = ACT == ACT_TANH ? __builtin_fmaf(-ca, ca, 1.f) : ACT == ACT_SIGMOID ? ca * (1.f - ca) : 1.f;
            const float yd = y[3] * dc;
            const float fc = __builtin_fmaf(fdot, cprev[m][n], y[1] * cst[m][n]);
            float cdn = __builtin_fmaf(y[0], gdot, __builtin_fmaf(idot, y[2], fc));
            if (m == 0 && (t0 + f2_rel<ROLE>(n)) % FNT == 4) {
              if constexpr (ACT == ACT_LINEAR) cdn = f2_rnd(y[0] * gdot) + (f2_rnd(idot * y[2]) + (f2_rnd(fdot * cprev[m][n]) + f2_rnd(y[1] * cst[m][n])));
              else cdn = __builtin_fmaf(y[0], gdot, f2_rnd(idot * y[2]) + fc);
            }
            hv = __builtin_fmaf(odot, ca, yd * cdn);
            cst[m][n] = cdn;
            cprev[m][n] = c;
            st4(f32x4{zd[0], zd[1], zd[2], zd[3]}, rt, tg);
            st1(cdn, rt, tc, 0);
          }
          hnext[hw + 16 * m * GH::LR + f2_rel<ROLE>(n)] = hv;
          st1(hv, rh, v1, 0);
        }
      };
      half(I0{});
      half(I1{});
      if constexpr (!BIG) xp.to_lds(xb + ((t + 1) & 1) * 32 * GX::LR, trash);
      lds_barrier();
    }
  }
}

template <int ACT, int KX, bool TAPE, bool TAN>
__global__ void __launch_bounds__(512, 1)
lstmf_fwd2_kernel(const float* __restrict__ x, const float* __restrict__ W, const float* __restrict__ bias,
                  const float* __restrict__ U, const float* __restrict__ ptape, float* __restrict__ hs,
                  float* __restrict__ tape, int B, int Tn) {
  static_assert(KX == 100, "the eight-wave exact forward is the K = 100 layer's");
  extern __shared__ __attribute__((aligned(16))) float fsm[];
  const int v = __builtin_amdgcn_readfirstlane(threadIdx.x >> 6);
  if (v == 0) fwd2_run<ACT, TAPE, TAN, 1>(x, W, bias, U, ptape, hs, tape, B, Tn, fsm, v);
  else if (v == 1) fwd2_run<ACT, TAPE, TAN, 2>(x, W, bias, U, ptape, hs, tape, B, Tn, fsm, v);
  else fwd2_run<ACT, TAPE, TAN, 0>(x, W, bias, U, ptape, hs, tape, B, Tn, fsm, v);
}

constexpr int BS_LZ = 432;
constexpr int BS_PL = 32 * BS_LZ * 2;

template <int ACT, bool HEAD = false, bool AHD = false>
__global__ void __launch_bounds__(256, 1)
lstmf_bwds_kernel(const float* __restrict__ dH, const float* __restrict__ tape, const float* __restrict__ U,
                  float* __restrict__ dZ, int B, int Tn, const float* __restrict__ hd, const float* __restrict__ hw,
                  float* __restrict__ aH) {
  extern __shared__ __attribute__((aligned(16))) float fsm[];
  float* zt = fsm;
  float* ht = zt + 32 * BZ_LR;
  float* trash = ht + 32 * BH_LR;
  lds_char* trashp = (lds_char*)(trash + 4 * BZ_KQ);
  lds_char* zp = (lds_char*)(trash + 4 * BZ_KQ + 4);
  const int tid = threadIdx.x, lane = tid & 63;
  const int w = __builtin_amdgcn_readfirstlane(tid >> 6);
  const int q = lane & 3, g = lane >> 4, j4 = (lane & 15) >> 2, c16 = lane & 15;
  const int nrb = (B + 31) / 32;
  bf16x8 up[2][DS_KS][3];
#pragma unroll
  for (int e = 0; e < 2; ++e) {
    const int col = 16 * (2 * w + e) + c16;
    const bool ok = col < FH;
#pragma unroll
    for (int ks = 0; ks < DS_KS; ++ks) {
      f32x4 v[2];
#pragma unroll
      for (int j = 0; j < 8; ++j) {
        const int k = min(32 * ks + 8 * g + j, FG - 1);
        const float x = U[(ok ? col : 0) * FG + (k & 3) * FH + (k >> 2)];
        v[j >> 2][j & 3] = (ok && 32 * ks + 8 * g + j < FG) ? x : 0.f;
      }
      uint32_t p0[3][2], p1[3][2];
      split3(v[0], p0);
      split3(v[1], p1);
#pragma unroll
      for (int p = 0; p < 3; ++p) {
        up[e][ks][p] = __builtin_bit_cast(bf16x8, make_uint4(p0[p][0], p0[p][1], p1[p][0], p1[p][1]));
        if (e == 1 || ks < 8) asm volatile("" : "+a"(up[e][ks][p]));
      }
    }
  }
  const int ub = FUW * w + j4;
  const int hr = (4 * g + q) * BH_LR + ub, zw = (4 * g + q) * BZ_LR + ub;
  const int zpw = ((4 * g + q) * BS_LZ + 4 * ub) * 2;
  const int ao = (c16 * BS_LZ + 8 * g) * 2;
  const RevStore st(tid, Tn);
  const int tl = ftape_lane(w, lane), tcl = ftape_cell(w, lane);
  for (int rb = blockIdx.x; rb < nrb; rb += gridDim.x) {
    const int row0 = rb * 32;
    const rsrc_t rdh = ftile_rsrc(dH, row0, B, Tn, FH), rt = ftape_rsrc(tape, rb, nrb, Tn);
    const rsrc_t rz = ftile_rsrc(dZ, row0, B, Tn, FG);
    const rsrc_t rah = ftile_rsrc(AHD ? aH : nullptr, row0, B, Tn, FH);
    const int nr = min(32, B - row0);
    int vp1[2];
#pragma unroll
    for (int m = 0; m < 2; ++m) vp1[m] = ((16 * m + 4 * g + q) * Tn * FH + ub) * 4;
    float hdv[2];
    head_rows<HEAD>(hdv, hd, true, row0, B, g, q);
    const rsrc_t rhw = head_rsrc<HEAD>(hw, Tn);
    const int hvo = ub * 4;
    float dc[2][FNT], tc[2][FNT];
    f32x4 tg[FNT];
    float tcp[FNT], tdh[FNT];
    const int T1 = Tn - 1;
#pragma unroll
    for (int n = 0; n < FNT; ++n) {
      const bool tok = unit_ok(w, n);
#pragma unroll
      for (int m = 0; m < 2; ++m) {
        dc[m][n] = 0.f;
        tc[m][n] = ld1(rt, tok ? tcl + T1 * FT_STEP * 4 + ftape_slot(m, n) : kOOB, 0);
      }
      bwdf_tape_load_u<HEAD>(tg[n], tcp[n], tdh[n], rt, rdh, tl, tcl, vp1[0], T1 * FT_STEP * 4 + ftape_slot(0, n),
                             max(T1 - 1, 0) * FT_STEP * 4 + ftape_slot(0, n), T1 * FH * 4 + 16 * n, tok, T1 > 0, hdv[0],
                             rhw, hvo);
    }
    for (int i = tid; i < 3 * BS_PL / 16; i += 256)
      reinterpret_cast<__attribute__((address_space(3))) u32x4_t*>(zp)[i] = u32x4_t{0, 0, 0, 0};
    for (int i = tid; i < 32 * BH_LR; i += 256) ht[i] = 0.f;
    __syncthreads();
    auto cell = [&](auto M_, int n, float hrec, int t) {
      constexpr int m = decltype(M_)::value;
      const bool tok = unit_ok(w, n);
      f32x4 z4;
      const float dht = bptt_cell<ACT>(z4, dc[m][n], tg[n], tc[m][n], tcp[n], tdh[n], hrec, tok,
                                       zt + zw + 16 * m * BZ_LR + 4 * n, trash);
      uint32_t p[3][2];
      split3(z4, p);
      planes_store(p, tok ? zp + zpw + 16 * m * BS_LZ * 2 + 32 * n : trashp, tok ? BS_PL : 0);
      tc[m][n] = tcp[n];
      if constexpr (m == 0) {
        bwdf_tape_load_u<HEAD>(tg[n], tcp[n], tdh[n], rt, rdh, tl, tcl, vp1[1], t * FT_STEP * 4 + ftape_slot(1, n),
                               max(t - 1, 0) * FT_STEP * 4 + ftape_slot(1, n), t * FH * 4 + 16 * n, tok, t > 0, hdv[1],
                               rhw, hvo);
      } else {
        const int tp = t > 0 ? t - 1 : 0;
        bwdf_tape_load_u<HEAD>(tg[n], tcp[n], tdh[n], rt, rdh, tl, tcl, vp1[0], tp * FT_STEP * 4 + ftape_slot(0, n),
                               max(tp - 1, 0) * FT_STEP * 4 + ftape_slot(0, n), tp * FH * 4 + 16 * n, tok && t > 0,
                               tp > 0, hdv[0], rhw, hvo);
      }
      if constexpr (AHD) st1(dht, rah, tok ? vp1[m] : kOOB, t * FH * 4 + 16 * n);
    };
    auto phase = [&](auto MA_, int t) {
      constexpr int MA = decltype(MA_)::value;
      if constexpr (MA == 1) {
        if (t < T1) st.half<1, false>(zt, rz, Tn, t + 1, nr);
      } else {
        st.half<0, false>(zt, rz, Tn, t, nr);
      }
      float hv[FNT];
#pragma unroll
      for (int n = 0; n < FNT; ++n) hv[n] = ht[hr + 16 * (1 - MA) * BH_LR + 4 * n];
      __builtin_amdgcn_sched_barrier(0);
      f32x4 acc[2] = {f32x4{0.f, 0.f, 0.f, 0.f}, f32x4{0.f, 0.f, 0.f, 0.f}};
      const lds_char* ar = zp + ao + 16 * MA * BS_LZ * 2;
      bf16x8 af[2][3];
#pragma unroll
      for (int p = 0; p < 3; ++p) af[0][p] = *reinterpret_cast<const __attribute__((address_space(3))) bf16x8*>(ar + p * BS_PL);
#pragma unroll
      for (int ks = 0; ks < DS_KS; ++ks) {
        if (ks + 1 < DS_KS) {
#pragma unroll
          for (int p = 0; p < 3; ++p)
            af[(ks + 1) & 1][p] = *reinterpret_cast<const __attribute__((address_space(3))) bf16x8*>(ar + p * BS_PL + 64 * (ks + 1));
        }
        const bf16x8(&a)[3] = af[ks & 1];
#pragma unroll
        for (int e = 0; e < 2; ++e) acc[e] = mma_split6(a, up[e][ks], acc[e]);
        if (ks < FNT) cell(std::integral_constant<int, 1 - MA>{}, ks, hv[ks], t);
      }
#pragma unroll
      for (int ks = 0; ks < DS_KS; ++ks) {
        __builtin_amdgcn_sched_group_barrier(0x100, 3, 0);
#pragma unroll
        for (int i = 0; i < 12; ++i) {
          __builtin_amdgcn_sched_group_barrier(0x008, 1, 0);
          __builtin_amdgcn_sched_group_barrier(0x002, 3, 0);
        }
      }
      __builtin_amdgcn_sched_barrier(0);
#pragma unroll
      for (int e = 0; e < 2; ++e) {
        const bool ok = 2 * w + e < 7;
        float* hd = ok ? ht + (16 * MA + 4 * g) * BH_LR + 16 * (2 * w + e) + c16 : trash;
        const int hs = ok ? BH_LR : 0;
#pragma unroll
        for (int i = 0; i < 4; ++i) hd[i * hs] = acc[e][i];
      }
      lds_barrier();
    };
    for (int t = T1; t >= 0; --t) {
      phase(I1{}, t);
      phase(I0{}, t);
    }
    st.half<1, false>(zt, rz, Tn, 0, nr);
    __syncthreads();
  }
}


struct RevStoreW {
  int lo[2], go[2];
  __device__ __forceinline__ RevStoreW(int lane, int Tn) {
#pragma unroll
    for (int j = 0; j < 2; ++j) {
      const bool ok = lane + 64 * j < 100;
      const int ch = ok ? lane + 64 * j : lane, qq = ch / 25, c = ch - 25 * qq;
      lo[j] = qq * BZ_KQ + 4 * c;
      go[j] = ok ? (qq * FH + 4 * c) * 4 : kOOB;
    }
  }
  template <int M>
  __device__ __forceinline__ void half(const float* tile, rsrc_t rz, int Tn, int ts, int nr) const {
#pragma unroll
    for (int r = 16 * M; r < 16 * M + 16; ++r) {
#pragma unroll
      for (int j = 0; j < 2; ++j) {
        const f32x4 v = *reinterpret_cast<const f32x4*>(tile + lo[j] + r * BZ_LR);
        st16(v, rz, r < nr, go[j], (r * Tn + ts) * FG * 4);
      }
    }
  }
};

#ifndef HFREP_BWDS2_NAF
#define HFREP_BWDS2_NAF 1
#endif
template <int ACT, bool HEAD, int NG, bool TILE, bool ST>
__device__ __forceinline__ void bwds2_run(const float* __restrict__ dH, const float* __restrict__ tape,
                                          const float* __restrict__ U, float* __restrict__ dZ, int B, int Tn,
                                          const float* __restrict__ hd, const float* __restrict__ hw, float* fsm,
                                          int v) {
  float* zt = fsm;
  float* ht = zt + 32 * BZ_LR;
  float* trash = ht + 32 * BH_LR;
  lds_char* zp = (lds_char*)(trash + 4 * BZ_KQ + 4);
  const int tid = threadIdx.x, lane = tid & 63;
  const int q = lane & 3, g = lane >> 4, j4 = (lane & 15) >> 2, c16 = lane & 15;
  const int nrb = (B + 31) / 32;
  const int g0 = 3 * v;
  bf16x8 up[TILE ? DS_KS : 1][3];
  if constexpr (TILE) {
    const int col = 16 * v + c16;
    const bool ok = col < FH;
#pragma unroll
    for (int ks = 0; ks < DS_KS; ++ks) {
      f32x4 uv[2];
#pragma unroll
      for (int j = 0; j < 8; ++j) {
        const int k = min(32 * ks + 8 * g + j, FG - 1);
        const float x = U[(ok ? col : 0) * FG + (k & 3) * FH + (k >> 2)];
        uv[j >> 2][j & 3] = (ok && 32 * ks + 8 * g + j < FG) ? x : 0.f;
      }
      uint32_t p0[3][2], p1[3][2];
      split3(uv[0], p0);
      split3(uv[1], p1);
#pragma unroll
      for (int p = 0; p < 3; ++p) {
        up[ks][p] = __builtin_bit_cast(bf16x8, make_uint4(p0[p][0], p0[p][1], p1[p][0], p1[p][1]));
        asm volatile("" : "+v"(up[ks][p]));
      }
    }
  }
  const int ub = 4 * g0 + j4;
  const int hr = (4 * g + q) * BH_LR + ub, zw = (4 * g + q) * BZ_LR + ub;
  const int zpw = ((4 * g + q) * BS_LZ + 4 * ub) * 2;
  const int ao = (c16 * BS_LZ + 8 * g) * 2;
  const RevStoreW st(lane, Tn);
  const int tl = lane * 16, tcl = (256 + lane) * 4;
  int tsl[NG];
#pragma unroll
  for (int k = 0; k < NG; ++k) tsl[k] = ftape_lane((g0 + k) / FNT, 0) + ftape_slot(0, (g0 + k) % FNT);
  for (int rb = blockIdx.x; rb < nrb; rb += gridDim.x) {
    const int row0 = rb * 32;
    const rsrc_t rdh = ftile_rsrc(dH, row0, B, Tn, FH), rt = ftape_rsrc(tape, rb, nrb, Tn);
    const rsrc_t rz = ftile_rsrc(dZ, row0, B, Tn, FG);
    const int nr = min(32, B - row0);
    int vp1[2];
#pragma unroll
    for (int m = 0; m < 2; ++m) vp1[m] = ((16 * m + 4 * g + q) * Tn * FH + ub) * 4;
    float hdv[2];
    head_rows<HEAD>(hdv, hd, true, row0, B, g, q);
    const rsrc_t rhw = head_rsrc<HEAD>(hw, Tn);
    const int hvo = ub * 4;
    float dc[2][NG], tc[2][NG];
    f32x4 tg[NG];
    float tcp[NG], tdh[NG];
    const int T1 = Tn - 1;
#pragma unroll
    for (int k = 0; k < NG; ++k) {
#pragma unroll
      for (int m = 0; m < 2; ++m) {
        dc[m][k] = 0.f;
        tc[m][k] = ld1(rt, tcl, T1 * FT_STEP * 4 + m * ftape_slot(1, 0) + tsl[k]);
      }
      bwdf_tape_load_u<HEAD>(tg[k], tcp[k], tdh[k], rt, rdh, tl, tcl, vp1[0], T1 * FT_STEP * 4 + tsl[k],
                             max(T1 - 1, 0) * FT_STEP * 4 + tsl[k], T1 * FH * 4 + 16 * k, true, T1 > 0, hdv[0], rhw, hvo);
    }
    for (int i = tid; i < 3 * BS_PL / 16; i += 512)
      reinterpret_cast<__attribute__((address_space(3))) u32x4_t*>(zp)[i] = u32x4_t{0, 0, 0, 0};
    for (int i = tid; i < 32 * BH_LR; i += 512) ht[i] = 0.f;
    __syncthreads();
    auto cell = [&](auto M_, int k, float hrec, int t) {
      constexpr int m = decltype(M_)::value;
      f32x4 z4;
      bptt_cell<ACT>(z4, dc[m][k], tg[k], tc[m][k], tcp[k], tdh[k], hrec, true, zt + zw + 16 * m * BZ_LR + 4 * k, trash);
      uint32_t p[3][2];
      split3(z4, p);
      planes_store(p, zp + zpw + 16 * m * BS_LZ * 2 + 32 * k, BS_PL);
      tc[m][k] = tcp[k];
      const int sl = (1 - m) * ftape_slot(1, 0) + tsl[k];
      if constexpr (m == 0) {
        bwdf_tape_load_u<HEAD>(tg[k], tcp[k], tdh[k], rt, rdh, tl, tcl, vp1[1], t * FT_STEP * 4 + sl,
                               max(t - 1, 0) * FT_STEP * 4 + sl, t * FH * 4 + 16 * k, true, t > 0, hdv[1], rhw, hvo);
      } else {
        const int tp = t > 0 ? t - 1 : 0;
        bwdf_tape_load_u<HEAD>(tg[k], tcp[k], tdh[k], rt, rdh, tl, tcl, vp1[0], tp * FT_STEP * 4 + sl,
                               max(tp - 1, 0) * FT_STEP * 4 + sl, tp * FH * 4 + 16 * k, t > 0, tp > 0, hdv[0], rhw, hvo);
      }
    };
    auto phase = [&](auto MA_, int t) {
      constexpr int MA = decltype(MA_)::value;
      if constexpr (ST) {
        if constexpr (MA == 1) {
          if (t < T1) st.half<1>(zt, rz, Tn, t + 1, nr);
        } else {
          st.half<0>(zt, rz, Tn, t, nr);
        }
      }
      float hv[NG];
#pragma unroll
      for (int k = 0; k < NG; ++k) hv[k] = ht[hr + 16 * (1 - MA) * BH_LR + 4 * k];
      if constexpr (TILE) {
        __builtin_amdgcn_sched_barrier(0);
        f32x4 acc = f32x4{0.f, 0.f, 0.f, 0.f};
        const lds_char* ar = zp + ao + 16 * MA * BS_LZ * 2;
        constexpr int NAF = HFREP_BWDS2_NAF;
        bf16x8 af[NAF][3];
        if constexpr (NAF == 2) {
#pragma unroll
          for (int p = 0; p < 3; ++p) af[0][p] = *reinterpret_cast<const __attribute__((address_space(3))) bf16x8*>(ar + p * BS_PL);
        }
#pragma unroll
        for (int ks = 0; ks < DS_KS; ++ks) {
          const int kr = NAF == 2 ? ks + 1 : ks;
          if (kr < DS_KS) {
#pragma unroll
            for (int p = 0; p < 3; ++p)
              af[kr % NAF][p] = *reinterpret_cast<const __attribute__((address_space(3))) bf16x8*>(ar + p * BS_PL + 64 * kr);
          }
          acc = mma_split6(af[ks % NAF], up[ks], acc);
          if (ks < NG) cell(std::integral_constant<int, 1 - MA>{}, ks, hv[ks], t);
        }
#pragma unroll
        for (int ks = 0; ks < DS_KS; ++ks) {
          __builtin_amdgcn_sched_group_barrier(0x100, 3, 0);
#pragma unroll
          for (int i = 0; i < 6; ++i) {
            __builtin_amdgcn_sched_group_barrier(0x008, 1, 0);
            __builtin_amdgcn_sched_group_barrier(0x002, 3, 0);
          }
        }
        __builtin_amdgcn_sched_barrier(0);
        float* hp = ht + (16 * MA + 4 * g) * BH_LR + 16 * v + c16;
#pragma unroll
        for (int i = 0; i < 4; ++i) hp[i * BH_LR] = acc[i];
      } else {
#pragma unroll
        for (int k = 0; k < NG; ++k) cell(std::integral_constant<int, 1 - MA>{}, k, hv[k], t);
      }
      lds_barrier();
    };
    for (int t = T1; t >= 0; --t) {
      phase(I1{}, t);
      phase(I0{}, t);
    }
    if constexpr (ST) st.half<1>(zt, rz, Tn, 0, nr);
    __syncthreads();
  }
}

template <int ACT, bool HEAD = false>
__global__ void __launch_bounds__(512, 1)
lstmf_bwds2_kernel(const float* __restrict__ dH, const float* __restrict__ tape, const float* __restrict__ U,
                   float* __restrict__ dZ, int B, int Tn, const float* __restrict__ hd, const float* __restrict__ hw) {
  extern __shared__ __attribute__((aligned(16))) float fsm[];
  const int v = __builtin_amdgcn_readfirstlane(threadIdx.x >> 6);
  if (v < 7) bwds2_run<ACT, HEAD, 3, true, false>(dH, tape, U, dZ, B, Tn, hd, hw, fsm, v);
  else bwds2_run<ACT, HEAD, 4, false, true>(dH, tape, U, dZ, B, Tn, hd, hw, fsm, v);
}

namespace {
template <int KX>
constexpr size_t fwdf_smem() {
  return (size_t)(2 * 32 * FGeo<KX>::LR + 2 * 32 * FGeo<FH>::LR + f_nwl<KX>() * 4 * FNT * 64 + 4) * 4;
}
static_assert(fwdf_smem<100>() <= F_LDS_MAX, "fp32 forward LDS");

template <int KX>
constexpr size_t fwds_smem() {
  return (size_t)(2 * 32 * FGeo<KX>::LR) * 4 + 2 * FS_HB + 16;
}
static_assert(fwds2_smem<32>() <= F_LDS_MAX, "two-wave split forward LDS");
static_assert(fwd2_smem() <= F_LDS_MAX, "eight-wave exact forward LDS");
static std::atomic<int>& fwdf_impl() {
  static std::atomic<int> v{fp32_exact() ? 1 : 3};
  return v;
}
static int fwdf_version() { return fwdf_impl().load(std::memory_order_relaxed); }
static std::atomic<int>& fwdf100_impl() {
  static std::atomic<int> v{2};
  return v;
}
template <int ACT, int KX, bool TAPE, bool TAN>
void fwd2_launch(const float* x, const float* W, const float* b, const float* U, const float* pt, float* hs, float* tp,
                 int B, int Tn, hipStream_t s) {
  const int nrb = (B + 31) / 32, cus = device_cu_count();
  auto k = lstmf_fwd2_kernel<ACT, KX, TAPE, TAN>;
  allow_lds(reinterpret_cast<const void*>(k));
  hipLaunchKernelGGL(k, dim3(nrb < cus ? nrb : cus), dim3(512), fwd2_smem(), s, x, W, b, U, pt, hs, tp, B, Tn);
}
template <int ACT, int KX, bool TAPE, bool TAN, int SKEW>
void fwds2_launch(const float* x, const float* W, const float* b, const float* U, const float* pt, float* hs, float* tp,
                  int B, int Tn, hipStream_t s) {
  const int nrb = (B + 31) / 32, cus = device_cu_count();
  auto k = lstmf_fwds2_kernel<ACT, KX, TAPE, TAN, SKEW>;
  allow_lds(reinterpret_cast<const void*>(k));
  hipLaunchKernelGGL(k, dim3(nrb < cus ? nrb : cus), dim3(512), fwds2_smem<KX>(), s, x, W, b, U, pt, hs, tp, B, Tn);
}
template <int ACT, int KX, bool TAPE, bool TAN>
void fwdf_launch(const float* x, const float* W, const float* b, const float* U, const float* pt, float* hs, float* tp,
                 int B, int Tn, hipStream_t s) {
  const int nrb = (B + 31) / 32, cus = device_cu_count();
  if constexpr (KX == 100) {
    if (fwdf100_impl().load(std::memory_order_relaxed) == 2)
      return fwd2_launch<ACT, KX, TAPE, TAN>(x, W, b, U, pt, hs, tp, B, Tn, s);
  }
  if constexpr (KX == 32) {
    const int ver = fwdf_version();
    if (ver == 3) return fwds2_launch<ACT, KX, TAPE, TAN, HFREP_FWDS2_SKEW>(x, W, b, U, pt, hs, tp, B, Tn, s);
#ifdef HFREP_FWDS2_AB
    if constexpr (ACT == ACT_TANH) {
      if (ver == 30) return fwds2_launch<ACT, KX, TAPE, TAN, 0>(x, W, b, U, pt, hs, tp, B, Tn, s);
      if (ver == 31) return fwds2_launch<ACT, KX, TAPE, TAN, 1>(x, W, b, U, pt, hs, tp, B, Tn, s);
      if (ver == 32) return fwds2_launch<ACT, KX, TAPE, TAN, 2>(x, W, b, U, pt, hs, tp, B, Tn, s);
      if (ver == 33) return fwds2_launch<ACT, KX, TAPE, TAN, 3>(x, W, b, U, pt, hs, tp, B, Tn, s);
    }
#endif
  }
  if constexpr (FGeo<KX>::KS <= 8 || (FGeo<KX>::KS <= 12 && !TAN)) {
    if (fwdf_version() >= 2) {
      auto k = lstmf_fwds_kernel<ACT, KX, TAPE, TAN>;
      allow_lds(reinterpret_cast<const void*>(k));
      hipLaunchKernelGGL(k, dim3(nrb < cus ? nrb : cus), dim3(256), fwds_smem<KX>(), s, x, W, b, U, pt, hs, tp, B, Tn);
      return;
    }
  }
  auto k = lstmf_fwd_kernel<ACT, KX, TAPE, TAN>;
  allow_lds(reinterpret_cast<const void*>(k));
  hipLaunchKernelGGL(k, dim3(nrb < cus ? nrb : cus), dim3(256), fwdf_smem<KX>(), s, x, W, b, U, pt, hs, tp, B, Tn);
}
template <int KX, bool TAPE, bool TAN>
void fwdf_act(int act, const float* x, const float* W, const float* b, const float* U, const float* pt, float* hs,
              float* tp, int B, int Tn, hipStream_t s) {
  switch (act) {
    case ACT_LINEAR: fwdf_launch<ACT_LINEAR, KX, TAPE, TAN>(x, W, b, U, pt, hs, tp, B, Tn, s); break;
    case ACT_SIGMOID: fwdf_launch<ACT_SIGMOID, KX, TAPE, TAN>(x, W, b, U, pt, hs, tp, B, Tn, s); break;
    default: fwdf_launch<ACT_TANH, KX, TAPE, TAN>(x, W, b, U, pt, hs, tp, B, Tn, s); break;
  }
}
template <bool TAPE, bool TAN>
bool fwdf_k(int K, int act, const float* x, const float* W, const float* b, const float* U, const float* pt, float* hs,
            float* tp, int B, int Tn, hipStream_t s) {
  switch (K) {
    case 32: fwdf_act<32, TAPE, TAN>(act, x, W, b, U, pt, hs, tp, B, Tn, s); return true;
    case 35: fwdf_act<35, TAPE, TAN>(act, x, W, b, U, pt, hs, tp, B, Tn, s); return true;
    case 36: fwdf_act<36, TAPE, TAN>(act, x, W, b, U, pt, hs, tp, B, Tn, s); return true;
    case 100: fwdf_act<100, TAPE, TAN>(act, x, W, b, U, pt, hs, tp, B, Tn, s); return true;
    default: return false;
  }
}
}

int set_lstmf_fwd_impl(int v) { return fwdf_impl().exchange(v); }
int set_lstmf_fwd100_impl(int v) { return fwdf100_impl().exchange(v); }

bool lstmf_supported(int H, int K, int act) {
  return H == FH && (K == 32 || K == 35 || K == 36 || K == 100) && (act == ACT_LINEAR || act == ACT_SIGMOID || act == ACT_TANH);
}

bool launch_lstmf_fwd(const float* x, const float* W, const float* b, const float* U, float* hs, float* tape, int B,
                      int Tn, int K, int H, int act, hipStream_t s) {
  if (!lstmf_supported(H, K, act) || B <= 0 || Tn <= 0) return false;
  if (tape) return fwdf_k<true, false>(K, act, x, W, b, U, nullptr, hs, tape, B, Tn, s);
  return fwdf_k<false, false>(K, act, x, W, b, U, nullptr, hs, nullptr, B, Tn, s);
}

bool launch_lstmf_tfwd(const float* xd, const float* W, const float* U, const float* tape, float* hds, float* ttape,
                       int B, int Tn, int K, int H, int act, hipStream_t s) {
  if (!lstmf_supported(H, K, act) || B <= 0 || Tn <= 0) return false;
  return fwdf_k<true, true>(K, act, xd, W, nullptr, U, tape, hds, ttape, B, Tn, s);
}

static std::atomic<int>& bwdf_impl() {
  static std::atomic<int> v{fp32_exact() ? 2 : 4};
  return v;
}
template <int ACT>
void bwdf_launch(const float* dH, const float* tape, const float* U, float* dZ, int B, int Tn, hipStream_t s,
                 const float* hd, const float* hw, float* aH) {
  const int ver = bwdf_impl().load(std::memory_order_relaxed);
  const int nrb = (B + 31) / 32, cus = device_cu_count();
  const size_t sm = (size_t)(32 * BZ_LR + 32 * BH_LR + 4 * BZ_KQ) * 4;
  if (ver == 4 && !aH) {
    auto go = [&](auto k) {
      allow_lds(reinterpret_cast<const void*>(k));
      hipLaunchKernelGGL(k, dim3(nrb < cus ? nrb : cus), dim3(512), sm + 16 + 3 * BS_PL, s, dH, tape, U, dZ, B, Tn, hd,
                         hw);
    };
    if (hd) go(lstmf_bwds2_kernel<ACT, true>);
    else go(lstmf_bwds2_kernel<ACT, false>);
    return;
  }
  if (ver != 2) {
    auto go = [&](auto k) {
      allow_lds(reinterpret_cast<const void*>(k));
      hipLaunchKernelGGL(k, dim3(nrb < cus ? nrb : cus), dim3(256), sm + 16 + 3 * BS_PL, s, dH, tape, U, dZ, B, Tn, hd,
                         hw, aH);
    };
    if (aH) {
      if (hd) go(lstmf_bwds_kernel<ACT, true, true>);
      else go(lstmf_bwds_kernel<ACT, false, true>);
    } else {
      if (hd) go(lstmf_bwds_kernel<ACT, true>);
      else go(lstmf_bwds_kernel<ACT, false>);
    }
    return;
  }
  if (aH) throw std::runtime_error("lstmf_bwd: the exact-fp32 BPTT does not store the h adjoints (lstmf_ahd_supported)");
  if (hd) throw std::runtime_error("lstmf_bwd: the exact-fp32 BPTT takes a materialised dH (lstmf_head_supported)");
  auto k = lstmf_bwdp_kernel<ACT>;
  allow_lds(reinterpret_cast<const void*>(k));
  hipLaunchKernelGGL(k, dim3(nrb < cus ? nrb : cus), dim3(512), sm, s, dH, tape, U, dZ, B, Tn);
}
static_assert((32 * BZ_LR + 32 * BH_LR + 4 * BZ_KQ) * 4 + 16 + 3 * BS_PL <= F_LDS_MAX, "split BPTT LDS");
int set_lstmf_bwd_impl(int v) { return bwdf_impl().exchange(v); }
bool lstmf_head_supported() { return bwdf_impl().load(std::memory_order_relaxed) != 2; }
bool lstmf_ahd_supported() { return bwdf_impl().load(std::memory_order_relaxed) != 2; }
bool launch_lstmf_bwd(const float* dH, const float* tape, const float* U, float* dZ, int B, int Tn, int H, int act,
                      hipStream_t s, const float* hd, const float* hw, float* aH) {
  if (H != FH || B <= 0 || Tn <= 0) return false;
  switch (act) {
    case ACT_LINEAR: bwdf_launch<ACT_LINEAR>(dH, tape, U, dZ, B, Tn, s, hd, hw, aH); return true;
    case ACT_SIGMOID: bwdf_launch<ACT_SIGMOID>(dH, tape, U, dZ, B, Tn, s, hd, hw, aH); return true;
    case ACT_TANH: bwdf_launch<ACT_TANH>(dH, tape, U, dZ, B, Tn, s, hd, hw, aH); return true;
    default: return false;
  }
}

template <int ACT>
void tbwdf_launch(const float* dH, const float* dHd, const float* tape, const float* ttape, const float* U, float* dZ,
                  float* dZd, int B, int Tn, hipStream_t s, const float* hd, const float* hdd, const float* hw) {
  const int cus = device_cu_count();
  const size_t sm = (size_t)(2 * 32 * BZ_LR + 2 * 32 * BH_LR + 4 * BZ_KQ) * 4;
  const int nrb = (B + 31) / 32;
  auto go = [&](auto k) {
    allow_lds(reinterpret_cast<const void*>(k));
    hipLaunchKernelGGL(k, dim3(nrb < cus ? nrb : cus), dim3(512), sm, s, dH, dHd, tape, ttape, U, dZ, dZd, B, Tn, hd, hdd,
                       hw);
  };
  if (hw) go(lstmf_tbwdp_kernel<ACT, true>);
  else go(lstmf_tbwdp_kernel<ACT, false>);
}
bool launch_lstmf_tbwd(const float* dH, const float* dHd, const float* tape, const float* ttape, const float* U, float* dZ,
                       float* dZd, int B, int Tn, int H, int act, hipStream_t s, const float* hd, const float* hdd,
                       const float* hw) {
  if (H != FH || B <= 0 || Tn <= 0) return false;
  switch (act) {
    case ACT_LINEAR: tbwdf_launch<ACT_LINEAR>(dH, dHd, tape, ttape, U, dZ, dZd, B, Tn, s, hd, hdd, hw); return true;
    case ACT_SIGMOID: tbwdf_launch<ACT_SIGMOID>(dH, dHd, tape, ttape, U, dZ, dZd, B, Tn, s, hd, hdd, hw); return true;
    case ACT_TANH: tbwdf_launch<ACT_TANH>(dH, dHd, tape, ttape, U, dZ, dZd, B, Tn, s, hd, hdd, hw); return true;
    default: return false;
  }
}
template <int ACT>
void tbwd1f_launch(const float* dH, const float* aH, const float* tape, const float* ttape, const float* U, float* dZ,
                   int B, int Tn, hipStream_t s, const float* hd, const float* hw) {
  const int cus = device_cu_count();
  const size_t sm = (size_t)(32 * BZ_LR + 32 * BH_LR + 4 * BZ_KQ) * 4;
  const int nrb = (B + 31) / 32;
  auto go = [&](auto k) {
    allow_lds(reinterpret_cast<const void*>(k));
    hipLaunchKernelGGL(k, dim3(nrb < cus ? nrb : cus), dim3(512), sm, s, dH, aH, tape, ttape, U, dZ, B, Tn, hd, hw);
  };
  if (hw) go(lstmf_tbwd1_kernel<ACT, true>);
  else go(lstmf_tbwd1_kernel<ACT, false>);
}
bool launch_lstmf_tbwd1(const float* dH, const float* aH, const float* tape, const float* ttape, const float* U, float* dZ,
                        int B, int Tn, int H, int act, hipStream_t s, const float* hd, const float* hw) {
  if (H != FH || B <= 0 || Tn <= 0 || !aH) return false;
  switch (act) {
    case ACT_LINEAR: tbwd1f_launch<ACT_LINEAR>(dH, aH, tape, ttape, U, dZ, B, Tn, s, hd, hw); return true;
    case ACT_SIGMOID: tbwd1f_launch<ACT_SIGMOID>(dH, aH, tape, ttape, U, dZ, B, Tn, s, hd, hw); return true;
    case ACT_TANH: tbwd1f_launch<ACT_TANH>(dH, aH, tape, ttape, U, dZ, B, Tn, s, hd, hw); return true;
    default: return false;
  }
}
size_t lstmf_tape_elems(int B, int Tn) { return (size_t)((B + 31) / 32) * Tn * FT_STEP; }

}
```

### do-you-really-need-to-pay-2-20-hedge-fund-strategy-replication-via-machine-learning_amd/models/layers.py

```python
from __future__ import annotations

import math
from dataclasses import dataclass

import numpy as np
import torch

from ..ops import functional as Fn
from ..ops import reference as R


def glorot_uniform(shape, gen, fan_in=None, fan_out=None):
    if fan_in is None:
        fan_in, fan_out = shape[0], shape[-1]
    lim = math.sqrt(6.0 / (fan_in + fan_out))
    return (torch.rand(shape, generator=gen, dtype=torch.float64) * 2 - 1) * lim


def orthogonal(shape, gen, gain=1.0):
    rows = int(np.prod(shape[:-1]))
    cols = shape[-1]
    a = torch.randn(max(rows, cols), min(rows, cols), generator=gen, dtype=torch.float64)
    q, r = torch.linalg.qr(a)
    q = q * torch.sign(torch.diagonal(r))
    if rows < cols:
        q = q.t()
    return (gain * q).reshape(shape)


@dataclass
class ParamSpec:
    name: str
    shape: tuple
    init: str
    keras: str = ""
    offset: int = 0


class Layer:

    kind = "layer"
    index = 0

    def __init__(self):
        self.model = None
        self.specs: list[ParamSpec] = []
        self.name = ""

    def build(self, in_shape):
        raise NotImplementedError

    def p(self, name):
        return self.model.view(self, name)

    def g(self, name):
        return self.model.gview(self, name)

    def forward(self, x):
        raise NotImplementedError

    def efwd(self, x, save: bool):
        raise NotImplementedError

    def ebwd(self, ctx, dy, need_dx: bool, wgrad: bool = True):
        raise NotImplementedError

    def etfwd(self, ctx, xd):
        raise NotImplementedError

    def etbwd(self, ctx, tctx, dy, dyd, need_dx: bool, need_dxd: bool = True):
        raise NotImplementedError

    def w(self, name):
        return self.p(name)


class Dense(Layer):
    kind = "dense"

    def __init__(self, units: int, activation=None, use_bias: bool = True):
        super().__init__()
        self.units, self.act, self.use_bias = units, activation, use_bias
        self.act_code = R.act_code(activation)

    def build(self, in_shape):
        fin = in_shape[-1]
        self.specs = [ParamSpec("kernel", (fin, self.units), "glorot")]
        if self.use_bias:
            self.specs.append(ParamSpec("bias", (self.units,), "zeros"))
        return tuple(in_shape[:-1]) + (self.units,)

    def forward(self, x):
        return R.dense(x, self.w("kernel"), self.w("bias") if self.use_bias else None, self.act)

    def efwd(self, x, save, out=None, compute=True, wgrad_rows=None):
        if not compute:
            assert self.act_code == 0, "only a linear Dense output can be left uncomputed"
            y = torch.empty(tuple(x.shape[:-1]) + (self.units,), dtype=x.dtype, device=x.device)
            return y, ({"x": x, "y": y} if save else None)
        b = self.p("bias") if self.use_bias else None
        if (wgrad_rows is not None and save and out is None and self.units == 1 and self.act_code == 0
                and Fn.head_cs_ok(x, self.p("kernel"))):
            split, wa, wb = wgrad_rows
            y = Fn.linear_head_cs(x, self.p("kernel"), b, split, wa, wb, self.g("kernel"),
                                  self.g("bias") if self.use_bias else None)
            return y, {"x": x, "y": y, "wgrad_done": True}
        y = Fn.linear(x, self.p("kernel"), b, self.act_code, out=out)
        return y, ({"x": x, "y": y} if save else None)

    def _dgrad(self, dz):
        if self.units == 1 and dz.dim() == 2 and Fn.outer_adjoint_ok(dz):
            return Fn.OuterAdjoint(dz, self.p("kernel"))
        return Fn.linear_dgrad(dz, self.p("kernel"))

    def ebwd(self, ctx, dy, need_dx, wgrad=True):
        dz = Fn.act_backward(dy, ctx["y"], self.act_code)
        if wgrad and not ctx.get("wgrad_done"):
            Fn.run_wgrad(Fn.linear_wgrad_, ctx["x"], dz, self.g("kernel"), self.g("bias") if self.use_bias else None)
        return self._dgrad(dz) if need_dx else None

    def etfwd(self, ctx, xd, compute=True):
        if not compute:
            assert self.act_code == 0, "only a linear Dense output can be left uncomputed"
            zd = torch.empty(tuple(xd.shape[:-1]) + (self.units,), dtype=xd.dtype, device=xd.device)
            return zd, {"xd": xd, "zd": zd}
        zd = Fn.linear(xd, self.p("kernel"), None, 0)
        yd = Fn.act_backward(zd, ctx["y"], self.act_code)
        return yd, {"xd": xd, "zd": zd}

    def etbwd(self, ctx, tctx, dy, dyd, need_dx, need_dxd=True):
        dzd = Fn.act_backward(dyd, ctx["y"], self.act_code)
        zero_dz = dy is None and self.act_code in (0, 3, 4)
        if not zero_dz:
            dz = Fn.act_tangent_backward(dy, dyd, ctx["y"], tctx["zd"], self.act_code)
            Fn.run_wgrad(Fn.linear_wgrad_, ctx["x"], dz, self.g("kernel"), self.g("bias") if self.use_bias else None)
        Fn.run_wgrad(Fn.linear_wgrad_, tctx["xd"], dzd, self.g("kernel"), None)
        if not need_dx:
            return None, None
        return (None if zero_dz else self._dgrad(dz)), (self._dgrad(dzd) if need_dxd else None)


class LSTM(Layer):
    kind = "lstm"
    accepts_outer = True

    def __init__(self, units: int, activation="tanh", return_sequences: bool = True):
        super().__init__()
        assert return_sequences, "the reference uses return_sequences=True everywhere"
        self.units, self.act = units, activation
        self.act_code = R.act_code(activation)

    def build(self, in_shape):
        fin = in_shape[-1]
        H = self.units
        self.specs = [
            ParamSpec("kernel", (fin, 4 * H), "glorot"),
            ParamSpec("recurrent_kernel", (H, 4 * H), "orthogonal"),
            ParamSpec("bias", (4 * H,), "lstm_bias"),
        ]
        return tuple(in_shape[:-1]) + (H,)

    def forward(self, x):
        return R.lstm(x, self.w("kernel"), self.w("recurrent_kernel"), self.w("bias"), act=self.act)

    def efwd(self, x, save):
        hs, tape = Fn.lstm_layer_fwd(x, self.p("kernel"), self.p("bias"), self.p("recurrent_kernel"), self.act_code,
                                     save)
        return hs, ({"x": x, "hs": hs, "tape": tape} if save else None)

    def ebwd(self, ctx, dy, need_dx, wgrad=True, keep=None):
        U = self.p("recurrent_kernel")
        dx = None
        if keep is not None:
            got = Fn.lstm_layer_bwd_keep(dy, ctx["tape"], U, self.act_code, W=self.p("kernel") if need_dx else None)
            if got is not None:
                dZ, dx, keep["ahd"] = got
                keep["dZ"] = dZ
                keep["dy"] = None
                if wgrad:
                    Fn.run_wgrad(Fn.lstm_wgrad_, ctx["x"], ctx["hs"], dZ, self.g("kernel"), self.g("recurrent_kernel"),
                                 self.g("bias"))
                return dx
        if need_dx:
            dZ, dx = Fn.lstm_layer_bwd(dy, ctx["tape"], U, self.act_code, W=self.p("kernel"), need_dz=wgrad)
        else:
            dZ = Fn.lstm_layer_bwd(dy, ctx["tape"], U, self.act_code)
        if wgrad:
            Fn.run_wgrad(Fn.lstm_wgrad_, ctx["x"], ctx["hs"], dZ, self.g("kernel"), self.g("recurrent_kernel"), self.g("bias"))
        return dx

    def etfwd(self, ctx, xd):
        hds, ttape = Fn.lstm_layer_tfwd(xd, self.p("kernel"), ctx["tape"], self.p("recurrent_kernel"), self.act_code)
        return hds, {"xd": xd, "hds": hds, "ttape": ttape}

    def etbwd(self, ctx, tctx, dy, dyd, need_dx, need_dxd=True, brec=None):
        U = self.p("recurrent_kernel")
        dx = dxd = None
        if brec is not None and "ahd" in brec:
            dZd, ahd = brec.pop("dZ"), brec.pop("ahd")
            dZ = Fn.lstm_layer_tbwd1(dy, ahd, ctx["tape"], tctx["ttape"], U, self.act_code)
            del ahd
            if need_dx:
                dx = Fn.linear_dgrad(dZ, self.p("kernel"))
        elif need_dx:
            dZ, dZd, dx, dxd = Fn.lstm_layer_tbwd(dy, dyd, ctx["tape"], tctx["ttape"], U, self.act_code,
                                                  W=self.p("kernel"), need_dxd=need_dxd)
        else:
            dZ, dZd = Fn.lstm_layer_tbwd(dy, dyd, ctx["tape"], tctx["ttape"], U, self.act_code)
        Fn.run_wgrad(Fn.lstm_wgrad_, ctx["x"], ctx["hs"], dZ, self.g("kernel"), self.g("recurrent_kernel"), self.g("bias"),
                       tctx["xd"], tctx["hds"], dZd)
        return dx, dxd


class LayerNormalization(Layer):
    kind = "layer_normalization"

    def __init__(self, epsilon: float = R.LN_EPS):
        super().__init__()
        self.eps = epsilon

    def build(self, in_shape):
        d = in_shape[-1]
        self.specs = [ParamSpec("gamma", (d,), "ones"), ParamSpec("beta", (d,), "zeros")]
        return tuple(in_shape)

    def forward(self, x):
        return R.layer_norm(x, self.w("gamma"), self.w("beta"), self.eps)

    def efwd(self, x, save):
        y, xhat, rstd = Fn.layer_norm_fwd(x, self.p("gamma"), self.p("beta"), self.eps, save=save)
        return y, ({"x": x, "xhat": xhat, "rstd": rstd} if save else None)

    def ebwd(self, ctx, dy, need_dx, wgrad=True):
        gg, gb = (self.g("gamma"), self.g("beta")) if wgrad else (None, None)
        dx = Fn.layer_norm_bwd_(dy, ctx["xhat"], ctx["rstd"], self.p("gamma"), gg, gb)
        return dx if need_dx else None

    def etfwd(self, ctx, xd):
        return Fn.layer_norm_tfwd(xd, ctx["xhat"], ctx["rstd"], self.p("gamma")), {"xd": xd}

    def etbwd(self, ctx, tctx, dy, dyd, need_dx, need_dxd=True):
        return Fn.layer_norm_tbwd_(dy, dyd, tctx["xd"], ctx["xhat"], ctx["rstd"], self.p("gamma"), self.g("gamma"),
                                   self.g("beta"), need_dx)


class LeakyReLU(Layer):
    kind = "leaky_re_lu"

    def __init__(self, alpha: float = R.LRELU_ALPHA):
        super().__init__()
        self.alpha = alpha

    def build(self, in_shape):
        return tuple(in_shape)

    def forward(self, x):
        return R.leaky_relu(x, self.alpha)

    def efwd(self, x, save):
        y = Fn.act_forward(x, 3)
        return y, ({"y": y} if save else None)

    def ebwd(self, ctx, dy, need_dx, wgrad=True):
        return Fn.act_backward(dy, ctx["y"], 3) if need_dx else None

    def etfwd(self, ctx, xd):
        return Fn.act_backward(xd, ctx["y"], 3), {}

    def etbwd(self, ctx, tctx, dy, dyd, need_dx, need_dxd=True):
        if not need_dx:
            return None, None
        dx = Fn.act_backward(dy, ctx["y"], 3) if dy is not None else None
        return dx, (Fn.act_backward(dyd, ctx["y"], 3) if need_dxd else None)


class Flatten(Layer):
    kind = "flatten"
    accepts_outer = True

    def build(self, in_shape):
        self.in_shape = tuple(in_shape)
        return (int(np.prod(in_shape)),)

    def forward(self, x):
        return x.reshape(x.shape[0], -1)

    def efwd(self, x, save):
        return x.reshape(x.shape[0], -1), ({"shape": x.shape} if save else None)

    def ebwd(self, ctx, dy, need_dx, wgrad=True):
        return dy.reshape(ctx["shape"]) if need_dx else None

    def etfwd(self, ctx, xd):
        return xd.reshape(xd.shape[0], -1), {}

    def etbwd(self, ctx, tctx, dy, dyd, need_dx, need_dxd=True):
        if not need_dx:
            return None, None
        return (dy.reshape(ctx["shape"]) if dy is not None else None), dyd.reshape(ctx["shape"])


class Conv1D(Layer):

    kind = "conv1d"

    def __init__(self, filters: int, kernel_size: int, activation=None, dilation: int = 1):
        super().__init__()
        self.filters, self.k, self.act, self.dil = filters, kernel_size, activation, dilation
        self.act_code = R.act_code(activation)

    def build(self, in_shape):
        T, cin = in_shape[-2], in_shape[-1]
        self.cin = cin
        self.specs = [ParamSpec("kernel", (self.k, cin, self.filters), "glorot_conv"),
                      ParamSpec("bias", (self.filters,), "zeros")]
        return (T, self.filters)

    def forward(self, x):
        return R.conv1d_causal(x, self.w("kernel"), self.w("bias"), self.act, self.dil)

    def _unfold(self, x):
        return Fn.im2col_causal(x, self.k, self.dil)

    def efwd(self, x, save):
        cols = self._unfold(x)
        y = Fn.linear(cols, self.p("kernel").reshape(-1, self.filters), self.p("bias"), self.act_code)
        return y, ({"x": x, "cols": cols, "y": y} if save else None)
# ... 247 lines not shown
```

### do-you-really-need-to-pay-2-20-hedge-fund-strategy-replication-via-machine-learning_amd/ops/functional.py

```python
from __future__ import annotations

import contextlib

import torch

from . import _native
from . import reference as R


def _nat(t: torch.Tensor) -> bool:
    return _native.use_native_for(t)


def _ops():
    return _native.native()


def _2d(x: torch.Tensor) -> torch.Tensor:
    return x.reshape(-1, x.shape[-1])


class _WgradDefer:
    stream = None
    keep: list = []


@contextlib.contextmanager
def wgrad_on(stream):
    if stream is None or _WgradDefer.stream is not None:
        yield
        return
    cur = torch.cuda.current_stream(stream.device)
    _WgradDefer.stream, _WgradDefer.keep = stream, []
    try:
        yield
    finally:
        _WgradDefer.stream = None
        cur.wait_stream(stream)
        _WgradDefer.keep = []


def run_wgrad(fn, *args, **kw):
    s = _WgradDefer.stream
    if s is None:
        return fn(*args, **kw)
    s.wait_stream(torch.cuda.current_stream(s.device))
    with torch.cuda.stream(s):
        fn(*args, **kw)
    _WgradDefer.keep.append((args, kw))




def linear(x: torch.Tensor, W: torch.Tensor, b: torch.Tensor | None, act: int,
           out: torch.Tensor | None = None) -> torch.Tensor:
    if _nat(x):
        y = _ops().linear(_2d(x.contiguous()), W, b, int(act), out)
        return y.reshape(*x.shape[:-1], W.shape[1])
    y = torch.matmul(x, W.to(x.dtype))
    if b is not None:
        y = y + b.to(x.dtype)
    y = R.apply_act(y, act)
    return y if out is None else out.copy_(y)




def linear_dgrad(dz: torch.Tensor, W: torch.Tensor) -> torch.Tensor:
    if (dz.dtype == torch.float32 and W.dtype == torch.float32 and dz.shape[-1] == 400
            and W.shape[0] <= 112 and _nat(dz)):
        return _ops().lstmf_dgrad(_2d(dz.contiguous()), W.contiguous()).reshape(*dz.shape[:-1], W.shape[0])
    if _nat(dz):
        return _ops().linear_dgrad(_2d(dz.contiguous()), W).reshape(*dz.shape[:-1], W.shape[0])
    return torch.matmul(dz, W.t().to(dz.dtype))


def linear_wgrad_(x: torch.Tensor, dz: torch.Tensor, gW: torch.Tensor, gb: torch.Tensor | None,
                  shift_T: int = 0) -> None:
    if _nat(dz):
        _ops().linear_wgrad_(_2d(x.contiguous()), _2d(dz.contiguous()), gW, gb, int(shift_T))
        return
    if shift_T:
        x = R.shift_prev(x)
    x2, d2 = _2d(x).to(gW.dtype), _2d(dz).to(gW.dtype)
    gW.add_(x2.t() @ d2)
    if gb is not None:
        gb.add_(d2.sum(0))


def act_forward(x: torch.Tensor, act: int) -> torch.Tensor:
    if _nat(x):
        return _ops().act_fwd(x.contiguous(), int(act))
    return R.apply_act(x, act)


def act_backward(dy: torch.Tensor, y: torch.Tensor, act: int) -> torch.Tensor:
    if act == 0:
        return dy
    if _nat(dy):
        return _ops().act_bwd(dy.contiguous(), y.contiguous(), int(act))
    return dy * R.act_dy(y, act)


def act_tangent_backward(dy, dyd, y, zd, act: int):
    first = act_backward(dy, y, act) if dy is not None else None
    if act in (0, 3, 4):
        return first if first is not None else torch.zeros_like(dyd)
    if _nat(dyd):
        sec = _ops().act_tangent_bwd(dyd.contiguous(), y.contiguous(), zd.contiguous(), int(act))
    else:
        sec = dyd * R.act_d2y(y, act) * zd
    return sec if first is None else first + sec


def lstm_seq_fwd(zx, U, act: int, save: bool):
    if _nat(zx):
        hs, gates, cs = _ops().lstm_fwd(zx.contiguous(), U, int(act), bool(save))
        return hs, (gates if save else None), (cs if save else None)
    return R.lstm_seq_fwd(zx, U.to(zx.dtype), act, save)


def lstm_seq_bwd(dh_seq, gates, cs, U, act: int):
    if _nat(dh_seq):
        return _ops().lstm_bwd(dh_seq.contiguous(), gates, cs, U, int(act))
    return R.lstm_seq_bwd(dh_seq, gates, cs, U.to(dh_seq.dtype), act)


def lstm_seq_tfwd(dzx, gates, cs, U, act: int):
    if _nat(dzx):
        return tuple(_ops().lstm_tfwd(dzx.contiguous(), gates, cs, U, int(act)))
    return R.lstm_seq_tfwd(dzx, gates, cs, U.to(dzx.dtype), act)


def lstm_seq_tbwd(dh_seq, dhd_seq, gates, cs, zds, cds, U, act: int):
    if _nat(dhd_seq):
        return tuple(_ops().lstm_tbwd(dh_seq.contiguous(), dhd_seq.contiguous(), gates, cs, zds, cds, U, int(act)))
    return R.lstm_seq_tbwd(dh_seq, dhd_seq, gates, cs, zds, cds, U.to(dhd_seq.dtype), act)


def shift_prev(h_seq: torch.Tensor) -> torch.Tensor:
    if _nat(h_seq):
        return _ops().shift_prev(h_seq.contiguous())
    return R.shift_prev(h_seq)


def layer_norm_fwd(x, gamma, beta, eps: float, save: bool = True):
    if _nat(x):
        y, xhat, rstd = _ops().layernorm_fwd(x.contiguous(), gamma, beta, float(eps), bool(save))
        return y, xhat, rstd
    return R.layer_norm_fwd(x, gamma.to(x.dtype), beta.to(x.dtype), eps)


def lrelu_layer_norm_fwd(x, gamma, beta, eps: float, alpha: float, save: bool = True):
    if _nat(x):
        return _ops().layernorm_fwd(x.contiguous(), gamma, beta, float(eps), bool(save), float(alpha))
# ... 78 lines not shown

def gp_coef_pack(g: torch.Tensor, weight: float, w: torch.Tensor):
    if _nat(g) and w.dtype == torch.float32:
        return _ops().gp_coef_pack(g.contiguous(), float(weight), w.contiguous())
    pen, v = gp_coef(g, weight)
    w = w.to(torch.float64 if g.dtype == torch.float64 else torch.float32)
    pen = pen.to(w.dtype)
    return torch.stack([w[0] + w[1] + weight * pen, w[0], w[1], pen]), v


def gp_pack(pen: torch.Tensor, weight: float, w: torch.Tensor) -> torch.Tensor:
    if _nat(pen) and pen.dtype == torch.float32 and w.dtype == torch.float32:
        return _ops().gp_pack(pen.reshape(1).contiguous(), float(weight), w.contiguous())
    w = w.to(pen.dtype)
    return torch.stack([w[0] + w[1] + weight * pen.reshape(()), w[0], w[1], pen.reshape(())])


def wdist(x: torch.Tensor, ref_sorted: torch.Tensor) -> torch.Tensor:
    if _nat(x):
        return _ops().wdist_sorted(x, ref_sorted)
    return R.wdist_sorted(x, ref_sorted)


def wdist_ref(real: torch.Tensor) -> torch.Tensor:
    return torch.sort(real.to(torch.float32).t().contiguous(), dim=1).values.contiguous()


KS_MAX_ROWS = 1 << 24


def ks_stat(x: torch.Tensor, ref_sorted: torch.Tensor) -> torch.Tensor:
    if _nat(x):
        return _ops().ks_stat(x, ref_sorted)
    return R.ks_stat(x, ref_sorted)


def acf_mean(x: torch.Tensor, nlags: int = 17) -> torch.Tensor:
    if _nat(x):
        return _ops().acf_mean(x, int(nlags))
    return R.acf_mean(x, int(nlags))


def acf_mean_supported(T: int, F: int, nlags: int) -> bool:
    return 0 <= nlags <= 4096 and 4 * T * F + 8 * (nlags + 3) * F <= 160 * 1024


def nb_divergences(real: torch.Tensor, fake: torch.Tensor, theta: torch.Tensor, var: torch.Tensor,
                   log_prior: torch.Tensor) -> torch.Tensor:
    if _nat(real):
        return _ops().nb_divergences(real, fake, theta, var, log_prior)
    return R.nb_divergences(real, fake, theta, var, log_prior)


def nb_divergences_supported(T: int, F: int) -> bool:
    return 1 <= F <= 64 and 1 <= T <= 168


def lp_cols(a: torch.Tensor, b: torch.Tensor) -> torch.Tensor:
    if _nat(a):
        return _ops().lp_cols(a, b)
    return R.lp_cols(a, b)


def interpolate(real: torch.Tensor, fake: torch.Tensor, alpha: torch.Tensor) -> torch.Tensor:
    if _nat(real):
        return _ops().interpolate(real.contiguous(), fake.contiguous(), alpha.contiguous())
    a = alpha.reshape(-1, *([1] * (real.dim() - 1))).to(real.dtype)
    return a * real + (1 - a) * fake


def _use_lstm2(x: torch.Tensor, U: torch.Tensor) -> bool:
    return (x.dtype == torch.bfloat16 and U.shape[0] == 100 and x.shape[-1] <= 128 and _nat(x)
            and not _native.fallback_allowed())


def _lstm2_dx_fused(W) -> bool:
    return W is not None and W.shape[0] <= 112


def _use_lstmf(x: torch.Tensor, U: torch.Tensor, act: int) -> bool:
    return (x.dtype == torch.float32 and _nat(x) and not _native.fallback_allowed()
            and bool(_ops().lstmf_supported(int(U.shape[0]), int(x.shape[-1]), int(act))))


class FTape:

    __slots__ = ("t", "B", "T")

    def __init__(self, t: torch.Tensor, B: int, T: int):
        self.t, self.B, self.T = t, int(B), int(T)


def lstm_layer_fwd(x, W, b, U, act: int, save: bool):
    if _use_lstm2(x, U):
        hs, tape = _ops().lstm2_fwd(x.contiguous(), W, b, U, int(act), bool(save))
        return hs, (tape if save else None)
    if _use_lstmf(x, U, act):
        hs, tape = _ops().lstmf_fwd(x.contiguous(), W, b, U, int(act), bool(save))
        return hs, (FTape(tape, x.shape[0], x.shape[1]) if save else None)
    zx = linear(x, W, b, 0)
    hs, gates, cs = lstm_seq_fwd(zx, U, act, save)
    return hs, ((gates, cs) if save else None)


class OuterAdjoint:

    def __init__(self, d: torch.Tensor, w: torch.Tensor, shape=None):
        self.d, self.w = d, w
        self.shape = tuple(shape) if shape is not None else (d.shape[0], w.shape[0])

    def reshape(self, *shape):
        shape = tuple(shape[0]) if len(shape) == 1 and not isinstance(shape[0], int) else tuple(shape)
        return OuterAdjoint(self.d, self.w, shape)

    def materialize(self) -> torch.Tensor:
        return linear_dgrad(self.d, self.w).reshape(self.shape)


def outer_adjoint_ok(dz: torch.Tensor) -> bool:
    return dz.dtype in (torch.bfloat16, torch.float32) and _nat(dz) and not _native.fallback_allowed()


def _mat(a):
    return a.materialize() if isinstance(a, OuterAdjoint) else a


def lstm_layer_bwd(dH, tape, U, act: int, W=None, need_dz: bool = True):
    if isinstance(tape, FTape):
        if isinstance(dH, OuterAdjoint) and dH.d.dtype == torch.float32:
            dZ = _ops().lstmf_bwd(None, tape.t, U, int(act), tape.B, tape.T, dH.d.contiguous(),
                                  dH.w.reshape(-1).contiguous())
        else:
            dH = _mat(dH)
            dZ = _ops().lstmf_bwd(None if dH is None else dH.contiguous(), tape.t, U, int(act), tape.B, tape.T)
        return dZ if W is None else (dZ, linear_dgrad(dZ, W))
    if isinstance(tape, torch.Tensor):
        Wk = W if _lstm2_dx_fused(W) else None
        nd = bool(need_dz or Wk is None)
        if isinstance(dH, OuterAdjoint):
            dZ, dX = _ops().lstm2_bwd(None, tape, U, int(act), Wk, nd, dH.d.contiguous(), dH.w.reshape(-1).contiguous())
        else:
            dZ, dX = _ops().lstm2_bwd(dH.contiguous(), tape, U, int(act), Wk, nd)
        if W is not None and Wk is None:
            dX = linear_dgrad(dZ, W)
        if W is not None and not need_dz:
            dZ = None
        return dZ if W is None else (dZ, dX)
    dH = _mat(dH)
    gates, cs = tape
    dZ = lstm_seq_bwd(dH, gates, cs, U, act)
    return dZ if W is None else (dZ, linear_dgrad(dZ, W))


def lstm_layer_bwd_keep(dH, tape, U, act: int, W=None):
    if isinstance(tape, FTape):
        if not _ops().lstmf_ahd_supported():
            return None
        ah = torch.empty((tape.B, tape.T, U.shape[0]), dtype=torch.float32, device=tape.t.device)
        if isinstance(dH, OuterAdjoint) and dH.d.dtype == torch.float32:
            dZ = _ops().lstmf_bwd(None, tape.t, U, int(act), tape.B, tape.T, dH.d.contiguous(),
                                  dH.w.reshape(-1).contiguous(), ah)
        else:
            dH = _mat(dH)
            dZ = _ops().lstmf_bwd(None if dH is None else dH.contiguous(), tape.t, U, int(act), tape.B, tape.T, None,
                                  None, ah)
        return dZ, (None if W is None else linear_dgrad(dZ, W)), ah
    if isinstance(tape, torch.Tensor) or _nat(tape[0]):
        return None
    gates, cs = tape
    dZ, ah = R.lstm_seq_bwd_ahd(_mat(dH), gates, cs, U.to(gates.dtype), act)
    return dZ, (None if W is None else linear_dgrad(dZ, W)), ah


def lstm_layer_tbwd1(dH, a_hd, tape, ttape, U, act: int, W=None):
    if isinstance(tape, FTape):
        if isinstance(dH, OuterAdjoint) and dH.d.dtype == torch.float32:
            dZ = _ops().lstmf_tbwd1(None, a_hd, tape.t, ttape.t, U, int(act), tape.B, tape.T, dH.d.contiguous(),
                                    dH.w.reshape(-1).contiguous())
        else:
            dH = _mat(dH)
            dZ = _ops().lstmf_tbwd1(None if dH is None else dH.contiguous(), a_hd, tape.t, ttape.t, U, int(act), tape.B,
                                    tape.T)
    else:
        gates, cs = tape
        zds, cds = ttape
        dZ = R.lstm_seq_tbwd_ahd(_mat(dH), a_hd, gates, cs, zds, cds, U.to(gates.dtype), act)
    return dZ if W is None else (dZ, linear_dgrad(dZ, W))


def lstm_layer_tfwd(xd, W, tape, U, act: int):
    if isinstance(tape, FTape):
        hds, ttape = _ops().lstmf_tfwd(xd.contiguous(), W, U, tape.t, int(act))
        return hds, FTape(ttape, tape.B, tape.T)
    if isinstance(tape, torch.Tensor):
        hds, ttape = _ops().lstm2_tfwd(xd.contiguous(), W, U, tape, int(act))
        return hds, ttape
    gates, cs = tape
    dzx = linear(xd, W, None, 0)
    hds, zds, cds = lstm_seq_tfwd(dzx, gates, cs, U, act)
    return hds, (zds, cds)


def lstm_wgrad_(x, hs, dZ, gW, gU, gb, xd=None, hds=None, dZd=None, impl: int = 0) -> None:
    f32 = (dZ.dtype == torch.float32 and x.shape[-1] in (32, 35, 36, 100) and hs.shape[-1] == 100
           and dZ.shape[-1] == 400)
    if (dZ.dtype == torch.bfloat16 or f32) and _nat(dZ):
        _ops().lstm_wgrad_(x.contiguous(), hs.contiguous(), dZ.contiguous(), gW, gU, gb,
                           None if xd is None else xd.contiguous(), None if hds is None else hds.contiguous(),
                           None if dZd is None else dZd.contiguous(), int(impl))
        return
    T = hs.shape[1]
    linear_wgrad_(x, dZ, gW, gb)
    linear_wgrad_(hs, dZ, gU, None, shift_T=T)
    if xd is not None:
        linear_wgrad_(xd, dZd, gW, None)
        linear_wgrad_(hds, dZd, gU, None, shift_T=T)


def lstm_layer_tbwd(dH, dHd, tape, ttape, U, act: int, W=None, need_dxd: bool = True):
    if isinstance(tape, FTape):
        heads = [a for a in (dH, dHd) if isinstance(a, OuterAdjoint)]
        if heads and all(a is None or (isinstance(a, OuterAdjoint) and a.w is heads[0].w and a.d.dtype == torch.float32)
                         for a in (dH, dHd)):
            dZ, dZd = _ops().lstmf_tbwd(None, None, tape.t, ttape.t, U, int(act), tape.B, tape.T,
                                        None if dH is None else dH.d.contiguous(),
                                        None if dHd is None else dHd.d.contiguous(), heads[0].w.reshape(-1).contiguous())
        else:
            dH, dHd = _mat(dH), _mat(dHd)
            dZ, dZd = _ops().lstmf_tbwd(None if dH is None else dH.contiguous(), None if dHd is None else dHd.contiguous(),
                                        tape.t, ttape.t, U, int(act), tape.B, tape.T)
        return (dZ, dZd) if W is None else (dZ, dZd, linear_dgrad(dZ, W), linear_dgrad(dZd, W) if need_dxd else None)
    if isinstance(tape, torch.Tensor):
        heads = [a for a in (dH, dHd) if isinstance(a, OuterAdjoint)]
        Wk = W if _lstm2_dx_fused(W) else None
        if heads and all(a is None or (isinstance(a, OuterAdjoint) and a.w is heads[0].w)
                                       for a in (dH, dHd)):
            w = heads[0].w.reshape(-1).contiguous()
            dZ, dZd, dX, dXd = _ops().lstm2_tbwd(None, None, tape, ttape, U, int(act), Wk,
                                                 None if dH is None else dH.d.contiguous(),
                                                 None if dHd is None else dHd.d.contiguous(), w)
        else:
            dH, dHd = _mat(dH), _mat(dHd)
            dZ, dZd, dX, dXd = _ops().lstm2_tbwd(None if dH is None else dH.contiguous(), dHd.contiguous(), tape,
                                                 ttape, U, int(act), Wk)
        if W is not None and Wk is None:
            dX, dXd = linear_dgrad(dZ, W), linear_dgrad(dZd, W) if need_dxd else None
        return (dZ, dZd) if W is None else (dZ, dZd, dX, dXd)
    dH, dHd = _mat(dH), _mat(dHd)
    gates, cs = tape
    zds, cds = ttape
    if dH is None:
        dH = torch.zeros_like(dHd)
    dZ, dZd = lstm_seq_tbwd(dH, dHd, gates, cs, zds, cds, U, act)
    return (dZ, dZd) if W is None else (dZ, dZd, linear_dgrad(dZ, W), linear_dgrad(dZd, W) if need_dxd else None)
```

Measured before the change: 1.646 million seq/s.

## Store LSTM BPTT hidden adjoint in cell-order slab layout and enable bwds2 path

Adds a per-row-block "cell order" slab layout for the saved hidden-state adjoint (aH), matching how each wave and lane owns cells. The backward and tangent-backward kernels can then write and read aH with lane-contiguous addresses instead of strided row-major (B,T,H) tiles. The faster bwds2 kernel variant, previously skipped whenever aH had to be kept, now also stores aH in this layout. The layout is on by default through an environment flag, and the tangent-backward kernel reads it in the same order. The cost is extra template instantiations and an opaque buffer that only these kernels understand.

```diff
diff --git a/do-you-really-need-to-pay-2-20-hedge-fund-strategy-replication-via-machine-learning_amd/csrc/bindings.cpp b/do-you-really-need-to-pay-2-20-hedge-fund-strategy-replication-via-machine-learning_amd/csrc/bindings.cpp
--- a/do-you-really-need-to-pay-2-20-hedge-fund-strategy-replication-via-machine-learning_amd/csrc/bindings.cpp
+++ b/do-you-really-need-to-pay-2-20-hedge-fund-strategy-replication-via-machine-learning_amd/csrc/bindings.cpp
@@ -338,9 +338,10 @@
 }
 
 bool lstmf_ahd_supported() { return hfrep::lstmf_ahd_supported(); }
+int64_t lstmf_ah_elems(int64_t B, int64_t Tn) { return (int64_t)hfrep::lstmf_ah_elems((int)B, (int)Tn); }
 
 Tensor lstmf_bwd(optional<Tensor> dH, Tensor tape, Tensor U, int64_t act, int64_t B, int64_t Tn, optional<Tensor> hd,
-                 optional<Tensor> hw, optional<Tensor> ah_out) {
+                 optional<Tensor> hw, optional<Tensor> ah_out, int64_t ah_layout) {
   CHECK_F32(tape);
   const int H = U.size(0);
   check_lstm_U(U, H);
@@ -349,10 +350,13 @@
   TORCH_CHECK(hd.has_value() == hw.has_value() && !(hd.has_value() && dH.has_value()),
               "lstmf_bwd: dH or the head factors (hd, hw)");
   check_head(hd, hw, tape, B, Tn * H);
+  TORCH_CHECK(ah_layout == 0 || ah_layout == 1, "lstmf_bwd: ah_layout 0 (row-major) or 1 (cell order)");
   if (ah_out.has_value()) {
     CHECK_F32(*ah_out);
-    TORCH_CHECK(ah_out->numel() == B * Tn * H && ah_out->is_contiguous() && ah_out->device() == tape.device(),
-                "lstmf_bwd: ah_out must be a contiguous (B, T, H) fp32 tensor on the tape's device");
+    const int64_t n = ah_layout == 1 ? (int64_t)hfrep::lstmf_ah_elems(B, Tn) : B * Tn * H;
+    TORCH_CHECK(ah_out->numel() == n && ah_out->is_contiguous() && ah_out->device() == tape.device(),
+                "lstmf_bwd: ah_out must be a contiguous fp32 tensor on the tape's device, (B, T, H) or lstmf_ah_elems "
+                "floats by ah_layout");
     TORCH_CHECK(hfrep::lstmf_ahd_supported(), "lstmf_bwd: ah_out needs the split-recurrent BPTT (lstmf_ahd_supported)");
   }
   GUARD(tape);
@@ -368,19 +372,22 @@
   const bool ok = hfrep::launch_lstmf_bwd(dhp, tape.data_ptr<float>(), U.data_ptr<float>(), dZ.data_ptr<float>(), B, Tn,
                                           H, (int)act, cur_stream(tape), head ? hd->data_ptr<float>() : nullptr,
                                           head ? hw->data_ptr<float>() : nullptr,
-                                          ah_out.has_value() ? ah_out->data_ptr<float>() : nullptr);
+                                          ah_out.has_value() ? ah_out->data_ptr<float>() : nullptr, ah_layout == 1);
   TORCH_CHECK(ok, "lstmf_bwd: unsupported H / act");
   return dZ;
 }
 
 Tensor lstmf_tbwd1(optional<Tensor> dH, Tensor aH, Tensor tape, Tensor ttape, Tensor U, int64_t act, int64_t B,
-                   int64_t Tn, optional<Tensor> hd, optional<Tensor> hw) {
+                   int64_t Tn, optional<Tensor> hd, optional<Tensor> hw, int64_t ah_layout) {
   CHECK_F32(tape); CHECK_F32(ttape); CHECK_F32(aH);
   const int H = U.size(0);
   check_lstm_U(U, H);
   TORCH_CHECK(tape.numel() == (int64_t)hfrep::lstmf_tape_elems(B, Tn) && ttape.numel() == tape.numel(), "tape size");
-  TORCH_CHECK(aH.numel() == B * Tn * H && aH.is_contiguous() && aH.device() == tape.device(),
-              "lstmf_tbwd1: aH must be a contiguous (B, T, H) fp32 tensor on the tape's device");
+  TORCH_CHECK(ah_layout == 0 || ah_layout == 1, "lstmf_tbwd1: ah_layout 0 (row-major) or 1 (cell order)");
+  TORCH_CHECK(aH.numel() == (ah_layout == 1 ? (int64_t)hfrep::lstmf_ah_elems(B, Tn) : B * Tn * H) &&
+                  aH.is_contiguous() && aH.device() == tape.device(),
+              "lstmf_tbwd1: aH must be a contiguous fp32 tensor on the tape's device, (B, T, H) or lstmf_ah_elems "
+              "floats by ah_layout");
   if (dH.has_value()) {
     CHECK_F32(*dH);
     TORCH_CHECK(dH->numel() == B * Tn * H && dH->is_contiguous() && dH->device() == tape.device(),
@@ -396,7 +403,7 @@
                                             tape.data_ptr<float>(), ttape.data_ptr<float>(), U.data_ptr<float>(),
                                             dZ.data_ptr<float>(), B, Tn, H, (int)act, cur_stream(tape),
                                             head && hd.has_value() ? hd->data_ptr<float>() : nullptr,
-                                            head ? hw->data_ptr<float>() : nullptr);
+                                            head ? hw->data_ptr<float>() : nullptr, ah_layout == 1);
   TORCH_CHECK(ok, "lstmf_tbwd1: unsupported H / act");
   return dZ;
 }
@@ -1103,10 +1110,11 @@
   m.def("linear_head_cs(Tensor x, Tensor W, Tensor? b, int split, float wa, float wb, Tensor(a!) gW, Tensor(b!)? gb) -> Tensor");
   m.def("linear_head_cs_supported(int K) -> bool", &linear_head_cs_supported);
   m.def("lstmf_bwd(Tensor? dH, Tensor tape, Tensor U, int act, int B, int T, Tensor? hd=None, Tensor? hw=None, "
-        "Tensor(a!)? ah_out=None) -> Tensor");
+        "Tensor(a!)? ah_out=None, int ah_layout=0) -> Tensor");
   m.def("lstmf_ahd_supported() -> bool", &lstmf_ahd_supported);
+  m.def("lstmf_ah_elems(int B, int T) -> int", &lstmf_ah_elems);
   m.def("lstmf_tbwd1(Tensor? dH, Tensor aH, Tensor tape, Tensor ttape, Tensor U, int act, int B, int T, Tensor? hd=None, "
-        "Tensor? hw=None) -> Tensor");
+        "Tensor? hw=None, int ah_layout=0) -> Tensor");
   m.def("lstmf_tbwd(Tensor? dH, Tensor? dHd, Tensor tape, Tensor ttape, Tensor U, int act, int B, int T, Tensor? hd=None, "
         "Tensor? hdd=None, Tensor? hw=None) -> (Tensor, Tensor)");
   m.def("lstmf_tfwd(Tensor xd, Tensor W, Tensor U, Tensor tape, int act) -> (Tensor, Tensor)");
diff --git a/do-you-really-need-to-pay-2-20-hedge-fund-strategy-replication-via-machine-learning_amd/csrc/kernels.h b/do-you-really-need-to-pay-2-20-hedge-fund-strategy-replication-via-machine-learning_amd/csrc/kernels.h
--- a/do-you-really-need-to-pay-2-20-hedge-fund-strategy-replication-via-machine-learning_amd/csrc/kernels.h
+++ b/do-you-really-need-to-pay-2-20-hedge-fund-strategy-replication-via-machine-learning_amd/csrc/kernels.h
@@ -32,17 +32,19 @@
 
 bool lstmf_supported(int H, int K, int act);
 size_t lstmf_tape_elems(int B, int Tn);
+size_t lstmf_ah_elems(int B, int Tn);
 bool launch_lstmf_fwd(const float* x, const float* W, const float* b, const float* U, float* hs, float* tape, int B,
                       int Tn, int K, int H, int act, hipStream_t s);
 bool launch_lstmf_tfwd(const float* xd, const float* W, const float* U, const float* tape, float* hds, float* ttape,
                        int B, int Tn, int K, int H, int act, hipStream_t s);
 bool launch_lstmf_bwd(const float* dH, const float* tape, const float* U, float* dZ, int B, int Tn, int H, int act,
-                      hipStream_t s, const float* hd = nullptr, const float* hw = nullptr, float* aH = nullptr);
+                      hipStream_t s, const float* hd = nullptr, const float* hw = nullptr, float* aH = nullptr,
+                      bool ah_slab = false);
 bool lstmf_head_supported();
 bool lstmf_ahd_supported();
 bool launch_lstmf_tbwd1(const float* dH, const float* aH, const float* tape, const float* ttape, const float* U, float* dZ,
                         int B, int Tn, int H, int act, hipStream_t s, const float* hd = nullptr,
-                        const float* hw = nullptr);
+                        const float* hw = nullptr, bool ah_slab = false);
 bool launch_lstmf_tbwd(const float* dH, const float* dHd, const float* tape, const float* ttape, const float* U, float* dZ,
                        float* dZd, int B, int Tn, int H, int act, hipStream_t s, const float* hd = nullptr,
                        const float* hdd = nullptr, const float* hw = nullptr);
diff --git a/do-you-really-need-to-pay-2-20-hedge-fund-strategy-replication-via-machine-learning_amd/csrc/lstm_f32.hip b/do-you-really-need-to-pay-2-20-hedge-fund-strategy-replication-via-machine-learning_amd/csrc/lstm_f32.hip
--- a/do-you-really-need-to-pay-2-20-hedge-fund-strategy-replication-via-machine-learning_amd/csrc/lstm_f32.hip
+++ b/do-you-really-need-to-pay-2-20-hedge-fund-strategy-replication-via-machine-learning_amd/csrc/lstm_f32.hip
@@ -104,6 +104,15 @@
 __device__ __forceinline__ int ftape_lane(int w, int lane) { return (w * FT_MN * FT_SLOT) * 4 + lane * 16; }
 __device__ __forceinline__ int ftape_cell(int w, int lane) { return (w * FT_MN * FT_SLOT + 256 + lane) * 4; }
 __device__ __forceinline__ constexpr int ftape_slot(int m, int n) { return (m * FNT + n) * FT_SLOT * 4; }
+
+constexpr int AH_STEP = 4 * FT_MN * 64;
+template <int LEAD = 0>
+__device__ __forceinline__ rsrc_t ahs_rsrc(const float* ah, int rb, int nrb, int Tn) {
+  rb = __builtin_amdgcn_readfirstlane(rb);
+  const bool on = ah && rb < nrb;
+  return make_rsrc(ah + (on ? (size_t)rb * Tn * AH_STEP : 0) - (on ? LEAD : 0), on ? (Tn * AH_STEP + LEAD) * 4 : 0);
+}
+__device__ __forceinline__ int ahs_cell(int t, int w, int m, int n) { return ((t * 4 + w) * FT_MN + m * FNT + n) * 256; }
 
 }
 
@@ -673,7 +682,7 @@
   }
 }
 
-template <int ACT, bool HEAD = false>
+template <int ACT, bool HEAD = false, bool AHS = false>
 __global__ void __launch_bounds__(512, 1)
 lstmf_tbwd1_kernel(const float* __restrict__ dH, const float* __restrict__ aH, const float* __restrict__ tape,
                    const float* __restrict__ ttape, const float* __restrict__ U, float* __restrict__ dZ, int B, int Tn,
@@ -714,7 +723,8 @@
     const int tl = ftape_lane(w, lane), tcl = ftape_cell(w, lane);
     for (int rb = blockIdx.x; rb < nrb; rb += gridDim.x) {
       const int row0 = rb * 32;
-      const rsrc_t rdh = ftile_rsrc(dH, row0, B, Tn, FH), rah = ftile_rsrc(aH, row0, B, Tn, FH);
+      const rsrc_t rdh = ftile_rsrc(dH, row0, B, Tn, FH);
+      const rsrc_t rah = AHS ? ahs_rsrc(aH, rb, nrb, Tn) : ftile_rsrc(aH, row0, B, Tn, FH);
       const rsrc_t rt = ftape_rsrc(tape, rb, nrb, Tn), rtt = ftape_rsrc(ttape, rb, nrb, Tn);
       int vp1[2];
 #pragma unroll
@@ -731,7 +741,8 @@
         const bool tok = on && unit_ok(w, n);
         tan_step_load<HEAD>(tg[n], tz[n], tcp[n], tcdp[n], tdh[n], rt, rtt, rdh, rhw, tl, tcl, vp1[m], hvo, hdv[m], m, n, tt,
                             tok);
-        tah[n] = ld1(rah, tok ? vp1[m] : kOOB, tt * FH * 4 + 16 * n);
+        if constexpr (AHS) tah[n] = ld1(rah, tok ? 4 * lane : kOOB, ahs_cell(tt, w, m, n));
+        else tah[n] = ld1(rah, tok ? vp1[m] : kOOB, tt * FH * 4 + 16 * n);
       };
       auto load_half = [&](auto M_, int tt, bool on) {
 #pragma unroll
@@ -1527,7 +1538,7 @@
 constexpr int BS_LZ = 432;
 constexpr int BS_PL = 32 * BS_LZ * 2;
 
-template <int ACT, bool HEAD = false, bool AHD = false>
+template <int ACT, bool HEAD = false, bool AHD = false, bool AHS = false>
 __global__ void __launch_bounds__(256, 1)
 lstmf_bwds_kernel(const float* __restrict__ dH, const float* __restrict__ tape, const float* __restrict__ U,
                   float* __restrict__ dZ, int B, int Tn, const float* __restrict__ hd, const float* __restrict__ hw,
@@ -1576,7 +1587,7 @@
     const int row0 = rb * 32;
     const rsrc_t rdh = ftile_rsrc(dH, row0, B, Tn, FH), rt = ftape_rsrc(tape, rb, nrb, Tn);
     const rsrc_t rz = ftile_rsrc(dZ, row0, B, Tn, FG);
-    const rsrc_t rah = ftile_rsrc(AHD ? aH : nullptr, row0, B, Tn, FH);
+    const rsrc_t rah = AHS ? ahs_rsrc(AHD ? aH : nullptr, rb, nrb, Tn) : ftile_rsrc(AHD ? aH : nullptr, row0, B, Tn, FH);
     const int nr = min(32, B - row0);
     int vp1[2];
 #pragma unroll
@@ -1625,7 +1636,8 @@
                                max(tp - 1, 0) * FT_STEP * 4 + ftape_slot(0, n), tp * FH * 4 + 16 * n, tok && t > 0,
                                tp > 0, hdv[0], rhw, hvo);
       }
-      if constexpr (AHD) st1(dht, rah, tok ? vp1[m] : kOOB, t * FH * 4 + 16 * n);
+      if constexpr (AHD && AHS) st1(dht, rah, tok ? 4 * lane : kOOB, ahs_cell(t, w, m, n));
+      else if constexpr (AHD) st1(dht, rah, tok ? vp1[m] : kOOB, t * FH * 4 + 16 * n);
     };
     auto phase = [&](auto MA_, int t) {
       constexpr int MA = decltype(MA_)::value;
@@ -1712,11 +1724,11 @@
 #ifndef HFREP_BWDS2_NAF
 #define HFREP_BWDS2_NAF 1
 #endif
-template <int ACT, bool HEAD, int NG, bool TILE, bool ST>
+template <int ACT, bool HEAD, bool AHD, int NG, bool TILE, bool ST>
 __device__ __forceinline__ void bwds2_run(const float* __restrict__ dH, const float* __restrict__ tape,
                                           const float* __restrict__ U, float* __restrict__ dZ, int B, int Tn,
-                                          const float* __restrict__ hd, const float* __restrict__ hw, float* fsm,
-                                          int v) {
+                                          const float* __restrict__ hd, const float* __restrict__ hw,
+                                          float* __restrict__ aH, float* fsm, int v) {
   float* zt = fsm;
   float* ht = zt + 32 * BZ_LR;
   float* trash = ht + 32 * BH_LR;
@@ -1757,10 +1769,14 @@
   int tsl[NG];
 #pragma unroll
   for (int k = 0; k < NG; ++k) tsl[k] = ftape_lane((g0 + k) / FNT, 0) + ftape_slot(0, (g0 + k) % FNT);
+  int asl[NG];
+#pragma unroll
+  for (int k = 0; k < NG; ++k) asl[k] = ahs_cell(0, (g0 + k) / FNT, 0, (g0 + k) % FNT);
   for (int rb = blockIdx.x; rb < nrb; rb += gridDim.x) {
     const int row0 = rb * 32;
     const rsrc_t rdh = ftile_rsrc(dH, row0, B, Tn, FH), rt = ftape_rsrc(tape, rb, nrb, Tn);
     const rsrc_t rz = ftile_rsrc(dZ, row0, B, Tn, FG);
+    const rsrc_t rah = ahs_rsrc<256>(AHD ? aH : nullptr, rb, nrb, Tn);
     const int nr = min(32, B - row0);
     int vp1[2];
 #pragma unroll
@@ -1790,7 +1806,8 @@
     auto cell = [&](auto M_, int k, float hrec, int t) {
       constexpr int m = decltype(M_)::value;
       f32x4 z4;
-      bptt_cell<ACT>(z4, dc[m][k], tg[k], tc[m][k], tcp[k], tdh[k], hrec, true, zt + zw + 16 * m * BZ_LR + 4 * k, trash);
+      const float dht = bptt_cell<ACT>(z4, dc[m][k], tg[k], tc[m][k], tcp[k], tdh[k], hrec, true,
+                                       zt + zw + 16 * m * BZ_LR + 4 * k, trash);
       uint32_t p[3][2];
       split3(z4, p);
       planes_store(p, zp + zpw + 16 * m * BS_LZ * 2 + 32 * k, BS_PL);
@@ -1804,6 +1821,7 @@
         bwdf_tape_load_u<HEAD>(tg[k], tcp[k], tdh[k], rt, rdh, tl, tcl, vp1[0], tp * FT_STEP * 4 + sl,
                                max(tp - 1, 0) * FT_STEP * 4 + sl, tp * FH * 4 + 16 * k, t > 0, tp > 0, hdv[0], rhw, hvo);
       }
+      if constexpr (AHD) st1(dht, rah, tcl, t * AH_STEP * 4 + ahs_cell(0, 0, m, 0) + asl[k]);
     };
     auto phase = [&](auto MA_, int t) {
       constexpr int MA = decltype(MA_)::value;
@@ -1866,14 +1884,15 @@
   }
 }
 
-template <int ACT, bool HEAD = false>
+template <int ACT, bool HEAD = false, bool AHD = false>
 __global__ void __launch_bounds__(512, 1)
 lstmf_bwds2_kernel(const float* __restrict__ dH, const float* __restrict__ tape, const float* __restrict__ U,
-                   float* __restrict__ dZ, int B, int Tn, const float* __restrict__ hd, const float* __restrict__ hw) {
+                   float* __restrict__ dZ, int B, int Tn, const float* __restrict__ hd, const float* __restrict__ hw,
+                   float* __restrict__ aH) {
   extern __shared__ __attribute__((aligned(16))) float fsm[];
   const int v = __builtin_amdgcn_readfirstlane(threadIdx.x >> 6);
-  if (v < 7) bwds2_run<ACT, HEAD, 3, true, false>(dH, tape, U, dZ, B, Tn, hd, hw, fsm, v);
-  else bwds2_run<ACT, HEAD, 4, false, true>(dH, tape, U, dZ, B, Tn, hd, hw, fsm, v);
+  if (v < 7) bwds2_run<ACT, HEAD, AHD, 3, true, false>(dH, tape, U, dZ, B, Tn, hd, hw, aH, fsm, v);
+  else bwds2_run<ACT, HEAD, AHD, 4, false, true>(dH, tape, U, dZ, B, Tn, hd, hw, aH, fsm, v);
 }
 
 namespace {
@@ -1994,18 +2013,23 @@
 }
 template <int ACT>
 void bwdf_launch(const float* dH, const float* tape, const float* U, float* dZ, int B, int Tn, hipStream_t s,
-                 const float* hd, const float* hw, float* aH) {
+                 const float* hd, const float* hw, float* aH, bool slab) {
   const int ver = bwdf_impl().load(std::memory_order_relaxed);
   const int nrb = (B + 31) / 32, cus = device_cu_count();
   const size_t sm = (size_t)(32 * BZ_LR + 32 * BH_LR + 4 * BZ_KQ) * 4;
-  if (ver == 4 && !aH) {
+  if (ver == 4 && (!aH || slab)) {
     auto go = [&](auto k) {
       allow_lds(reinterpret_cast<const void*>(k));
       hipLaunchKernelGGL(k, dim3(nrb < cus ? nrb : cus), dim3(512), sm + 16 + 3 * BS_PL, s, dH, tape, U, dZ, B, Tn, hd,
-                         hw);
+                         hw, aH);
     };
-    if (hd) go(lstmf_bwds2_kernel<ACT, true>);
-    else go(lstmf_bwds2_kernel<ACT, false>);
+    if (aH) {
+      if (hd) go(lstmf_bwds2_kernel<ACT, true, true>);
+      else go(lstmf_bwds2_kernel<ACT, false, true>);
+    } else {
+      if (hd) go(lstmf_bwds2_kernel<ACT, true>);
+      else go(lstmf_bwds2_kernel<ACT, false>);
+    }
     return;
   }
   if (ver != 2) {
@@ -2014,7 +2038,10 @@
       hipLaunchKernelGGL(k, dim3(nrb < cus ? nrb : cus), dim3(256), sm + 16 + 3 * BS_PL, s, dH, tape, U, dZ, B, Tn, hd,
                          hw, aH);
     };
-    if (aH) {
+    if (aH && slab) {
+      if (hd) go(lstmf_bwds_kernel<ACT, true, true, true>);
+      else go(lstmf_bwds_kernel<ACT, false, true, true>);
+    } else if (aH) {
       if (hd) go(lstmf_bwds_kernel<ACT, true, true>);
       else go(lstmf_bwds_kernel<ACT, false, true>);
     } else {
@@ -2034,12 +2061,12 @@
 bool lstmf_head_supported() { return bwdf_impl().load(std::memory_order_relaxed) != 2; }
 bool lstmf_ahd_supported() { return bwdf_impl().load(std::memory_order_relaxed) != 2; }
 bool launch_lstmf_bwd(const float* dH, const float* tape, const float* U, float* dZ, int B, int Tn, int H, int act,
-                      hipStream_t s, const float* hd, const float* hw, float* aH) {
+                      hipStream_t s, const float* hd, const float* hw, float* aH, bool ah_slab) {
   if (H != FH || B <= 0 || Tn <= 0) return false;
   switch (act) {
-    case ACT_LINEAR: bwdf_launch<ACT_LINEAR>(dH, tape, U, dZ, B, Tn, s, hd, hw, aH); return true;
-    case ACT_SIGMOID: bwdf_launch<ACT_SIGMOID>(dH, tape, U, dZ, B, Tn, s, hd, hw, aH); return true;
-    case ACT_TANH: bwdf_launch<ACT_TANH>(dH, tape, U, dZ, B, Tn, s, hd, hw, aH); return true;
+    case ACT_LINEAR: bwdf_launch<ACT_LINEAR>(dH, tape, U, dZ, B, Tn, s, hd, hw, aH, ah_slab); return true;
+    case ACT_SIGMOID: bwdf_launch<ACT_SIGMOID>(dH, tape, U, dZ, B, Tn, s, hd, hw, aH, ah_slab); return true;
+    case ACT_TANH: bwdf_launch<ACT_TANH>(dH, tape, U, dZ, B, Tn, s, hd, hw, aH, ah_slab); return true;
     default: return false;
   }
 }
@@ -2071,7 +2098,7 @@
 }
 template <int ACT>
 void tbwd1f_launch(const float* dH, const float* aH, const float* tape, const float* ttape, const float* U, float* dZ,
-                   int B, int Tn, hipStream_t s, const float* hd, const float* hw) {
+                   int B, int Tn, hipStream_t s, const float* hd, const float* hw, bool slab) {
   const int cus = device_cu_count();
   const size_t sm = (size_t)(32 * BZ_LR + 32 * BH_LR + 4 * BZ_KQ) * 4;
   const int nrb = (B + 31) / 32;
@@ -2079,19 +2106,25 @@
     allow_lds(reinterpret_cast<const void*>(k));
     hipLaunchKernelGGL(k, dim3(nrb < cus ? nrb : cus), dim3(512), sm, s, dH, aH, tape, ttape, U, dZ, B, Tn, hd, hw);
   };
-  if (hw) go(lstmf_tbwd1_kernel<ACT, true>);
-  else go(lstmf_tbwd1_kernel<ACT, false>);
+  if (slab) {
+    if (hw) go(lstmf_tbwd1_kernel<ACT, true, true>);
+    else go(lstmf_tbwd1_kernel<ACT, false, true>);
+  } else {
+    if (hw) go(lstmf_tbwd1_kernel<ACT, true>);
+    else go(lstmf_tbwd1_kernel<ACT, false>);
+  }
 }
 bool launch_lstmf_tbwd1(const float* dH, const float* aH, const float* tape, const float* ttape, const float* U, float* dZ,
-                        int B, int Tn, int H, int act, hipStream_t s, const float* hd, const float* hw) {
+                        int B, int Tn, int H, int act, hipStream_t s, const float* hd, const float* hw, bool ah_slab) {
   if (H != FH || B <= 0 || Tn <= 0 || !aH) return false;
   switch (act) {
-    case ACT_LINEAR: tbwd1f_launch<ACT_LINEAR>(dH, aH, tape, ttape, U, dZ, B, Tn, s, hd, hw); return true;
-    case ACT_SIGMOID: tbwd1f_launch<ACT_SIGMOID>(dH, aH, tape, ttape, U, dZ, B, Tn, s, hd, hw); return true;
-    case ACT_TANH: tbwd1f_launch<ACT_TANH>(dH, aH, tape, ttape, U, dZ, B, Tn, s, hd, hw); return true;
+    case ACT_LINEAR: tbwd1f_launch<ACT_LINEAR>(dH, aH, tape, ttape, U, dZ, B, Tn, s, hd, hw, ah_slab); return true;
+    case ACT_SIGMOID: tbwd1f_launch<ACT_SIGMOID>(dH, aH, tape, ttape, U, dZ, B, Tn, s, hd, hw, ah_slab); return true;
+    case ACT_TANH: tbwd1f_launch<ACT_TANH>(dH, aH, tape, ttape, U, dZ, B, Tn, s, hd, hw, ah_slab); return true;
     default: return false;
   }
 }
 size_t lstmf_tape_elems(int B, int Tn) { return (size_t)((B + 31) / 32) * Tn * FT_STEP; }
-
-}
+size_t lstmf_ah_elems(int B, int Tn) { return (size_t)((B + 31) / 32) * Tn * AH_STEP; }
+
+}
diff --git a/do-you-really-need-to-pay-2-20-hedge-fund-strategy-replication-via-machine-learning_amd/models/layers.py b/do-you-really-need-to-pay-2-20-hedge-fund-strategy-replication-via-machine-learning_amd/models/layers.py
--- a/do-you-really-need-to-pay-2-20-hedge-fund-strategy-replication-via-machine-learning_amd/models/layers.py
+++ b/do-you-really-need-to-pay-2-20-hedge-fund-strategy-replication-via-machine-learning_amd/models/layers.py
@@ -172,7 +172,8 @@
         U = self.p("recurrent_kernel")
         dx = None
         if keep is not None:
-            got = Fn.lstm_layer_bwd_keep(dy, ctx["tape"], U, self.act_code, W=self.p("kernel") if need_dx else None)
+            got = Fn.lstm_layer_bwd_keep(dy, ctx["tape"], U, self.act_code, W=self.p("kernel") if need_dx else None,
+                                         cell_order=True)
             if got is not None:
                 dZ, dx, keep["ahd"] = got
                 keep["dZ"] = dZ
diff --git a/do-you-really-need-to-pay-2-20-hedge-fund-strategy-replication-via-machine-learning_amd/ops/functional.py b/do-you-really-need-to-pay-2-20-hedge-fund-strategy-replication-via-machine-learning_amd/ops/functional.py
--- a/do-you-really-need-to-pay-2-20-hedge-fund-strategy-replication-via-machine-learning_amd/ops/functional.py
+++ b/do-you-really-need-to-pay-2-20-hedge-fund-strategy-replication-via-machine-learning_amd/ops/functional.py
@@ -1,6 +1,7 @@
 from __future__ import annotations
 
 import contextlib
+import os
 
 import torch
 
@@ -385,19 +386,36 @@
     return dZ if W is None else (dZ, linear_dgrad(dZ, W))
 
 
-def lstm_layer_bwd_keep(dH, tape, U, act: int, W=None):
+class AHSlab:
+
+    __slots__ = ("t", "B", "T")
+
+    def __init__(self, t: torch.Tensor, B: int, T: int):
+        self.t, self.B, self.T = t, int(B), int(T)
+
+
+def ah_cell_order_enabled() -> bool:
+    return os.environ.get("HFREP_AH_CELL_ORDER", "1") != "0" and hasattr(_ops(), "lstmf_ah_elems")
+
+
+def lstm_layer_bwd_keep(dH, tape, U, act: int, W=None, cell_order: bool = False):
     if isinstance(tape, FTape):
         if not _ops().lstmf_ahd_supported():
             return None
-        ah = torch.empty((tape.B, tape.T, U.shape[0]), dtype=torch.float32, device=tape.t.device)
+        slab = bool(cell_order) and ah_cell_order_enabled()
+        if slab:
+            ah = torch.empty((int(_ops().lstmf_ah_elems(tape.B, tape.T)),), dtype=torch.float32, device=tape.t.device)
+        else:
+            ah = torch.empty((tape.B, tape.T, U.shape[0]), dtype=torch.float32, device=tape.t.device)
+        lay = (1,) if slab else ()
         if isinstance(dH, OuterAdjoint) and dH.d.dtype == torch.float32:
             dZ = _ops().lstmf_bwd(None, tape.t, U, int(act), tape.B, tape.T, dH.d.contiguous(),
-                                  dH.w.reshape(-1).contiguous(), ah)
+                                  dH.w.reshape(-1).contiguous(), ah, *lay)
         else:
             dH = _mat(dH)
             dZ = _ops().lstmf_bwd(None if dH is None else dH.contiguous(), tape.t, U, int(act), tape.B, tape.T, None,
-                                  None, ah)
-        return dZ, (None if W is None else linear_dgrad(dZ, W)), ah
+                                  None, ah, *lay)
+        return dZ, (None if W is None else linear_dgrad(dZ, W)), (AHSlab(ah, tape.B, tape.T) if slab else ah)
     if isinstance(tape, torch.Tensor) or _nat(tape[0]):
         return None
     gates, cs = tape
@@ -407,13 +425,16 @@
 
 def lstm_layer_tbwd1(dH, a_hd, tape, ttape, U, act: int, W=None):
     if isinstance(tape, FTape):
+        lay = ()
+        if isinstance(a_hd, AHSlab):
+            a_hd, lay = a_hd.t, (1,)
         if isinstance(dH, OuterAdjoint) and dH.d.dtype == torch.float32:
             dZ = _ops().lstmf_tbwd1(None, a_hd, tape.t, ttape.t, U, int(act), tape.B, tape.T, dH.d.contiguous(),
-                                    dH.w.reshape(-1).contiguous())
+                                    dH.w.reshape(-1).contiguous(), *lay)
         else:
             dH = _mat(dH)
             dZ = _ops().lstmf_tbwd1(None if dH is None else dH.contiguous(), a_hd, tape.t, ttape.t, U, int(act), tape.B,
-                                    tape.T)
+                                    tape.T, None, None, *lay)
     else:
         gates, cs = tape
         zds, cds = ttape
```

Result: no change. 1.661 million seq/s, median of 6 (+0.9%).
